# JVBSouza/descriptools

Measured on AMD Instinct MI355X. Metric: Mcells/s full descriptor chain, higher is better.
Workload: dtype f32; 1 GPU; 16384x16384 synthetic tilted-integer-fBm DEM per GPU, full chain (d8, flowacc, river mask, flowhand/HAND with fused GFI + ln(hl/H), fused slope+TI+MTI, downslope), device-resident; global_dem=16384x16384, river_threshold_cells=524288

## Files before the change

### descriptools_amd/csrc/dt_capi.hip

```cpp
#include <cmath>
#include <stdarg.h>
#include <stdlib.h>

#include <sys/mman.h>
#include <atomic>
#include <chrono>
#include <mutex>
#include <system_error>
#include <thread>
#include <utility>
#include <vector>

#include "dt_common.h"
#include "dt_kernels.h"

static thread_local char g_err[512] = "";
void dt_set_error(const char *fmt, ...) {
  va_list ap;
  va_start(ap, fmt);
  vsnprintf(g_err, sizeof(g_err), fmt, ap);
  va_end(ap);
}
extern "C" const char *dt_last_error(void) { return g_err; }
extern "C" const char *dt_version(void) { return "descriptools_hip 0.1 (gfx950)"; }
// ... 941 lines not shown
}
extern "C" int dt_dev_downslope_queue(dt_ctx *c, const float *dem, const uint8_t *fdr, int64_t H, int64_t W, double px,
                                      double dz, int raw, float *out, void *qwork, int64_t qbytes) {
  return dev_downslope_phase(c, 1, dem, fdr, H, W, px, dz, raw, out, qwork, qbytes, nullptr, 0);
}
extern "C" int dt_dev_downslope_queued(dt_ctx *c, const void *qwork, int64_t *count) {
  DT_CTX(c);
  DT_REQUIRE(qwork && count, "NULL pointer");
  uint32_t n = 0;
  DT_HIP(hipMemcpyAsync(&n, qwork, sizeof(n), hipMemcpyDeviceToHost, c->stream));
  DT_HIP(hipStreamSynchronize(c->stream));
  *count = (int64_t)n;
  return DT_OK;
}
extern "C" int dt_dev_downslope_finish(dt_ctx *c, const float *dem, const uint8_t *fdr, int64_t H, int64_t W, double px,
                                       double dz, int raw, float *out, void *qwork, int64_t qbytes, void *twork,
                                       int64_t tbytes) {
  return dev_downslope_phase(c, 2, dem, fdr, H, W, px, dz, raw, out, qwork, qbytes, twork, tbytes);
}

extern "C" int dt_dev_confusion_multi(dt_ctx *c, const double *desc, const int8_t *flood, int64_t N,
                                      double nodata_value, const double *th_host, int nth, int under,
                                      int64_t *counts4_dev) {
  DT_DEV(d, c);
  DT_REQUIRE(th_host && counts4_dev, "NULL thresholds / counts");
  DT_REQUIRE((desc && flood) || N == 0, "NULL raster");
  return d.done(dt_launch_confusion(c->stream, desc, flood, N, nodata_value, th_host, nth, under,
                                    (unsigned long long *)counts4_dev));
}

extern "C" int dt_dev_unique_extremes_f32(dt_ctx *c, const float *x, int64_t N, float *out3_dev) {
  DT_DEV(d, c);
  DT_REQUIRE(x && out3_dev && N >= 0, "bad arguments");
  uint32_t *work = (uint32_t *)d.scratch(64, 256);
  DT_TRY(d.rc);
  return d.done(dt_launch_unique_extremes(c->stream, x, N, work, out3_dev));
}

extern "C" int dt_dev_minmax_scale_f32(dt_ctx *c, const float *x, int64_t N, float mn, float mx, float nodata,
                                       double *desc) {
  DT_DEV(d, c);
  DT_REQUIRE((x && desc) || N == 0, "NULL raster");
  return d.done(dt_launch_minmax_scale(c->stream, x, N, mn, mx, nodata, desc));
}

extern "C" int dt_dev_minmax_scale_f32_f64(dt_ctx *c, const float *x, int64_t N, double mn, double mx, double nodata,
                                           double *desc) {
  DT_DEV(d, c);
  DT_REQUIRE((x && desc) || N == 0, "NULL raster");
  return d.done(dt_launch_minmax_scale_f32f64(c->stream, x, N, mn, mx, nodata, desc));
}

extern "C" int dt_dev_classify(dt_ctx *c, const double *desc, int8_t *flood, int64_t N, double nodata_value,
                               double threshold, int under, int remap_flood, uint8_t *binary, int32_t *klass,
                               int64_t *counts4_dev) {
  DT_DEV(d, c);
  DT_REQUIRE(counts4_dev != nullptr, "counts4 is NULL");
  DT_REQUIRE((desc && flood) || N == 0, "NULL raster");
  return d.done(dt_launch_classify_f64(c->stream, desc, nullptr, flood, N, nodata_value, threshold, under, remap_flood,
                                       binary, klass, (unsigned long long *)counts4_dev));
}

extern "C" int dt_dev_membench_copy(dt_ctx *c, const float *a, float *b, int64_t N, int blocks) {
  DT_DEV(d, c);
  DT_REQUIRE(a && b && N >= 0 && blocks != 0, "bad arguments");
  return d.done(dt_launch_membench_copy(c->stream, a, b, N, blocks));
}

extern "C" int dt_dev_membench_mix(dt_ctx *c, const float *r0, const float *r1, float *w0, float *w1, float *w2,
                                   int64_t N, int n_reads, int n_writes, int nontemporal) {
  DT_DEV(d, c);
  DT_REQUIRE((n_reads < 1 || r0) && (n_reads < 2 || r1) && w0 && (n_writes < 2 || w1) && (n_writes < 3 || w2),
             "NULL stream");
  return d.done(dt_launch_membench_mix(c->stream, r0, r1, w0, w1, w2, N, n_reads, n_writes, nontemporal));
}

extern "C" int dt_dev_membench_mix_timed(dt_ctx *c, const float *r0, const float *r1, float *w0, float *w1, float *w2,
                                         int64_t N, int n_reads, int n_writes, int nontemporal, int reps, double *ms) {
  DT_CTX(c);
  DT_REQUIRE(ms && reps >= 1, "bad arguments");
  DT_TRY(dt_dev_membench_mix(c, r0, r1, w0, w1, w2, N, n_reads, n_writes, nontemporal));
  hipEvent_t e0 = nullptr, e1 = nullptr;
  DT_HIP(hipEventCreate(&e0));
  const hipError_t created = hipEventCreate(&e1);
  if (created != hipSuccess) {
    (void)hipEventDestroy(e0);
    DT_HIP(created);
  }
  int rc = DT_OK;
  float t = 0.0f;
  if (hipEventRecord(e0, c->stream) != hipSuccess) rc = DT_EHIP;
  for (int r = 0; r < reps && rc == DT_OK; r++)
    rc = dt_dev_membench_mix(c, r0, r1, w0, w1, w2, N, n_reads, n_writes, nontemporal);
  if (rc == DT_OK && (hipEventRecord(e1, c->stream) != hipSuccess || hipEventSynchronize(e1) != hipSuccess ||
                      hipEventElapsedTime(&t, e0, e1) != hipSuccess)) {
    dt_set_error("event timing failed: %s", hipGetErrorString(hipGetLastError()));
    rc = DT_EHIP;
  }
  (void)hipEventDestroy(e0);
  (void)hipEventDestroy(e1);
  if (rc == DT_OK) *ms = (double)t / reps;
  return rc;
}
extern "C" int dt_dev_mem_info(dt_ctx *c, int64_t *free_bytes, int64_t *total_bytes) {
  DT_CTX(c);
  size_t f = 0, t = 0;
  DT_HIP(hipMemGetInfo(&f, &t));
  if (free_bytes) *free_bytes = (int64_t)f;
  if (total_bytes) *total_bytes = (int64_t)t;
  return DT_OK;
}

extern "C" int dt_dev_i32_to_i64(dt_ctx *c, const int32_t *src, int64_t N, int64_t *dst) {
  DT_DEV(d, c);
  return d.done(dt_launch_i32_to_i64(c->stream, src, N, dst));
}
extern "C" int dt_dev_i64_to_i32(dt_ctx *c, const int64_t *src, int64_t N, int32_t *dst) {
  DT_DEV(d, c);
  return d.done(dt_launch_i64_to_i32(c->stream, src, N, dst));
}

extern "C" int64_t dt_perim_cells(int64_t H, int64_t W) { return dt_perim_count((int)H, (int)W); }

extern "C" int dt_dev_slope_d8_w(dt_ctx *c, const dt_window *win, const float *dem, double px, float *slope,
                                 uint8_t *fdr, float *slope_rad) {
  DT_DEV(d, c, win);
  DT_REQUIRE(dem && (slope || fdr || slope_rad), "NULL raster");
  DT_TRY(dt_side_reserve(c, &c->aux, &c->aux_bytes, dt_stencil_aux_bytes(d.w.H, d.w.W)));
  return d.done(dt_launch_stencil(c->stream, d.w, dem, px, slope, fdr, slope_rad, nullptr, 0, 0.0, nullptr, nullptr,
                                  c->aux));
}

static int dev_slope_twi_w(dt_ctx *c, const dt_window *win, const float *dem, const void *acc, int acc64, double px,
                           double n_top, float *slope, float *slope_rad, float *ti, float *mti) {
  DT_DEV(d, c, win);
  DT_REQUIRE(dem && acc && ti && mti, "NULL raster");
  DT_TRY(dt_side_reserve(c, &c->aux, &c->aux_bytes, dt_stencil_aux_bytes(d.w.H, d.w.W)));
  return d.done(dt_launch_stencil(c->stream, d.w, dem, px, slope, nullptr, slope_rad, acc, acc64, n_top, ti, mti,
                                  c->aux));
}
extern "C" int dt_dev_slope_twi_w(dt_ctx *c, const dt_window *win, const float *dem, const int32_t *acc32,
                                  double px, double n_top, float *slope, float *slope_rad, float *ti,
                                  float *mti) {
  return dev_slope_twi_w(c, win, dem, acc32, 0, px, n_top, slope, slope_rad, ti, mti);
}
extern "C" int dt_dev_slope_twi_w_a64(dt_ctx *c, const dt_window *win, const float *dem, const int64_t *acc64,
                                      double px, double n_top, float *slope, float *slope_rad, float *ti,
                                      float *mti) {
  return dev_slope_twi_w(c, win, dem, acc64, 1, px, n_top, slope, slope_rad, ti, mti);
}

extern "C" int64_t dt_downslope_lift_workspace_w(const dt_window *win) {
  DtWin w;
  if (dt_convert_window(win, &w) != DT_OK) return -1;
  return (int64_t)dt_downslope_lift_bytes_w(w);
}
enum DsForm { DS_PLAIN, DS_LIFT, DS_EMIT };
static int dev_downslope_w(dt_ctx *c, DsForm form, const dt_window *win, const float *dem, const uint8_t *fdr, double px,
                           double dz, int raw, float *out, int32_t *n_unresolved_dev, void *work, int64_t work_bytes,
                           void *walkers, int64_t walkers_bytes) {
  DT_DEV(d, c, win);
  DT_REQUIRE(dem && fdr && out, "NULL raster");
  if (form == DS_LIFT)
    DT_REQUIRE(work != nullptr && work_bytes >= (int64_t)dt_downslope_lift_bytes_w(d.w),
               "downslope workspace missing or too small");
  if (form == DS_EMIT) {
    DT_REQUIRE(work == nullptr || work_bytes >= (int64_t)dt_downslope_lift_bytes_w(d.w), "downslope workspace too small");
    DT_REQUIRE(walkers != nullptr && walkers_bytes >= 256 + 48, "walker buffer missing or too small");
  }
  if (n_unresolved_dev) DT_HIP(hipMemsetAsync(n_unresolved_dev, 0, sizeof(int32_t), c->stream));
  const DtDsLift L = work ? dt_downslope_lift_layout(d.w, work) : DtDsLift{};
  return d.done(dt_launch_downslope(c->stream, d.w, dem, fdr, px, dz, raw, out, (int *)n_unresolved_dev, L.qcount,
                                    L.tab[0], 0, walkers, (size_t)walkers_bytes));
}
extern "C" int dt_dev_downslope_w(dt_ctx *c, const dt_window *win, const float *dem, const uint8_t *fdr,
                                  double px, double dz, int raw, float *out, int32_t *n_unresolved_dev) {
  return dev_downslope_w(c, DS_PLAIN, win, dem, fdr, px, dz, raw, out, n_unresolved_dev, nullptr, 0, nullptr, 0);
}
extern "C" int dt_dev_downslope_lift_w(dt_ctx *c, const dt_window *win, const float *dem, const uint8_t *fdr,
                                       double px, double dz, int raw, float *out, int32_t *n_unresolved_dev,
                                       void *work, int64_t work_bytes) {
  return dev_downslope_w(c, DS_LIFT, win, dem, fdr, px, dz, raw, out, n_unresolved_dev, work, work_bytes, nullptr, 0);
}
extern "C" int dt_dev_downslope_emit_w(dt_ctx *c, const dt_window *win, const float *dem, const uint8_t *fdr,
                                       double px, double dz, int raw, float *out, int32_t *n_unresolved_dev,
                                       void *work, int64_t work_bytes, void *walkers, int64_t walkers_bytes) {
  return dev_downslope_w(c, DS_EMIT, win, dem, fdr, px, dz, raw, out, n_unresolved_dev, work, work_bytes, walkers,
                         walkers_bytes);
}

extern "C" int dt_dev_downslope_walk_w(dt_ctx *c, const dt_window *win, const float *dem, const uint8_t *fdr, double px,
                                       double dz, int64_t n, void *rec, void *work, int64_t work_bytes) {
  DT_DEV(d, c, win);
  DT_REQUIRE(n >= 0, "negative count");
  DT_REQUIRE(n == 0 || (dem && fdr && rec), "NULL pointer");
  DT_REQUIRE(work == nullptr || work_bytes >= (int64_t)dt_downslope_lift_bytes_w(d.w), "downslope workspace too small");
  return d.done(dt_launch_ds_walk(c->stream, d.w, dem, fdr, px, dz, n, rec, work));
}
extern "C" int dt_dev_downslope_walk_route_w(dt_ctx *c, const dt_window *win, const float *dem, const uint8_t *fdr,
                                             double px, double dz, int64_t n, void *rec, void *work, int64_t work_bytes,
                                             float *out, const int32_t *row_starts, int32_t ty,
                                             const int32_t *col_starts, int32_t tx, void *send, int32_t *counts,
                                             int32_t *scratch) {
  DT_DEV(d, c, win);
  DT_REQUIRE(n >= 0, "negative count");
  DT_REQUIRE(ty >= 1 && tx >= 1 && row_starts && col_starts && counts, "layout / counts missing");
  DT_REQUIRE(n == 0 || (dem && fdr && rec && out && send && scratch), "NULL pointer");
  DT_REQUIRE(work == nullptr || work_bytes >= (int64_t)dt_downslope_lift_bytes_w(d.w), "downslope workspace too small");
  DT_TRY(dt_launch_ds_walk(c->stream, d.w, dem, fdr, px, dz, n, rec, work, out));
  return d.done(dt_launch_ds_route(c->stream, n, rec, row_starts, ty, col_starts, tx, send, counts, scratch));
}
template <typename T, typename Launch>
static int dev_downslope_walk_seed_w(dt_ctx *c, const dt_window *win, const T *dem, int64_t n, const int32_t *ys,
                                     const int32_t *xs, void *rec, Launch launch) {
  DT_DEV(d, c, win);
  DT_REQUIRE(n >= 0, "negative count");
  DT_REQUIRE(n == 0 || (dem && ys && xs && rec), "NULL pointer");
  return d.done(launch(c->stream, d.w, dem, n, ys, xs, rec));
}
extern "C" int dt_dev_downslope_walk_seed_w(dt_ctx *c, const dt_window *win, const float *dem, int64_t n,
                                            const int32_t *ys, const int32_t *xs, void *rec) {
  return dev_downslope_walk_seed_w(c, win, dem, n, ys, xs, rec, dt_launch_ds_walk_seed);
}

extern "C" int dt_dev_flowacc_local_w(dt_ctx *c, const dt_window *win, const uint8_t *fdr, int32_t *acc32,
                                      int64_t *A_perim, int32_t *xr_perim, uint8_t *code_perim) {
  DT_DEV(d, c, win);
  DT_REQUIRE(fdr && A_perim && xr_perim && code_perim, "NULL pointer");
  const size_t need = dt_flowacc_tiled_scratch(d.w.H, d.w.W);
  void *scr, *scr2;
  d.scratch(need, dt_flowhand_tiled_scratch(d.w.H, d.w.W), &scr, &scr2);
  DT_TRY(d.rc);
  DT_TRY(dt_launch_fa_local(c->stream, d.w, fdr, scr, need, acc32, 1));
  DT_TRY(d.done(dt_launch_fa_summary(c->stream, d.w, scr, A_perim, xr_perim, code_perim)));
  dt_scratch_claim(c, DT_OWNER_FLOWACC, d.w.H, d.w.W, scr, scr2);
  return DT_OK;
}

static int dev_flowacc_finish_w(dt_ctx *c, const dt_window *win, const uint8_t *fdr, const float *dem,
                                const uint64_t *ext_perim, int64_t threshold, void *acc, int acc64, int8_t *river) {
  DT_DEV(d, c, win);
  DT_REQUIRE(fdr && acc, "NULL raster");
  const DtScratchClaim *k;
  DT_TRY(dt_scratch_claimed(c, DT_OWNER_FLOWACC, &d.w, false,
                            "dt_dev_flowacc_finish_w without a matching dt_dev_flowacc_local_w on this context (another "
                            "call has used the context's scratch in between)", &k));
  return d.done(dt_launch_fa_finish(c->stream, d.w, fdr, dem, k->ptr, (const unsigned long long *)ext_perim, threshold,
                                    acc, acc64, river, c->status));
}
extern "C" int dt_dev_flowacc_finish_w(dt_ctx *c, const dt_window *win, const uint8_t *fdr, const float *dem,
                                       const uint64_t *ext_perim, int64_t threshold, int32_t *acc32,
                                       int8_t *river) {
  return dev_flowacc_finish_w(c, win, fdr, dem, ext_perim, threshold, acc32, 0, river);
}
extern "C" int dt_dev_flowacc_finish_w_a64(dt_ctx *c, const dt_window *win, const uint8_t *fdr, const float *dem,
                                           const uint64_t *ext_perim, int64_t threshold, int64_t *acc64,
                                           int8_t *river) {
  return dev_flowacc_finish_w(c, win, fdr, dem, ext_perim, threshold, acc64, 1, river);
}

static int dev_flowacc_finish_fh_local_w(dt_ctx *c, const dt_window *win, const uint8_t *fdr, const float *dem,
                                         const uint64_t *ext_perim, int64_t threshold, void *acc, int acc64,
                                         int8_t *river, uint8_t *kind, int32_t *ref, int32_t *nc, int32_t *nd,
                                         float *zr, int64_t *ar) {
  DT_DEV(d, c, win);
  DT_REQUIRE(fdr && acc && river && kind && ref && nc && nd && zr && ar, "NULL pointer");
  const DtScratchClaim *k;
  DT_TRY(dt_scratch_claimed(c, DT_OWNER_FLOWACC, &d.w, true,
                            "dt_dev_flowacc_finish_flowhand_local_w without a matching dt_dev_flowacc_local_w on this "
                            "context (another call has used the context's scratch in between)", &k));
  char *fh = k->ptr2;
  DT_TRY(dt_launch_fa_finish_fh_local(c->stream, d.w, fdr, dem, k->ptr, fh, dt_flowhand_tiled_scratch(d.w.H, d.w.W),
                                      (const unsigned long long *)ext_perim, threshold, acc, acc64, river, c->status));
  DT_TRY(d.done(dt_launch_fh_summary(c->stream, d.w, fh, dem, acc, acc64, kind, ref, nc, nd, zr, (long long *)ar)));
  dt_scratch_claim(c, DT_OWNER_HAND, d.w.H, d.w.W, fh);
  return DT_OK;
}
extern "C" int dt_dev_flowacc_finish_flowhand_local_w(dt_ctx *c, const dt_window *win, const uint8_t *fdr,
                                                      const float *dem, const uint64_t *ext_perim, int64_t threshold,
                                                      int32_t *acc32, int8_t *river, uint8_t *kind, int32_t *ref,
                                                      int32_t *nc, int32_t *nd, float *zr, int64_t *ar) {
  return dev_flowacc_finish_fh_local_w(c, win, fdr, dem, ext_perim, threshold, acc32, 0, river, kind, ref, nc, nd, zr, ar);
}
extern "C" int dt_dev_flowacc_finish_flowhand_local_w_a64(dt_ctx *c, const dt_window *win, const uint8_t *fdr,
                                                          const float *dem, const uint64_t *ext_perim,
                                                          int64_t threshold, int64_t *acc64, int8_t *river,
                                                          uint8_t *kind, int32_t *ref, int32_t *nc, int32_t *nd,
                                                          float *zr, int64_t *ar) {
  return dev_flowacc_finish_fh_local_w(c, win, fdr, dem, ext_perim, threshold, acc64, 1, river, kind, ref, nc, nd, zr, ar);
}

static int dev_flowacc_river_flowhand_local(dt_ctx *c, const uint8_t *fdr, const float *dem, const uint8_t *nod4,
                                           int64_t H, int64_t W, int64_t threshold, int32_t *acc32, int8_t *river,
                                           const DtTwiEpilogue *twi = nullptr) {
  DT_DEV(d, c, H, W);
  DT_REQUIRE((fdr && acc32 && river) || H * W == 0, "NULL raster");
  DT_REQUIRE(!twi || H * W == 0 || dt_twi_epilogue_ok(d.w, acc32, river, twi),
             "this raster does not take the TI / MTI epilogue (dt_slope_from_d8_ok): use dt_dev_slope_twi");
  const size_t need = dt_flowacc_tiled_scratch(H, W), need2 = dt_flowhand_tiled_scratch(H, W);
  void *scr, *scr2;
  d.scratch(need, need2, &scr, &scr2);
  DT_TRY(d.rc);
  DT_TRY(dt_launch_fa_local(c->stream, d.w, fdr, scr, need, acc32, 0));
  DT_TRY(d.done(dt_launch_fa_finish_fh_local(c->stream, d.w, fdr, dem, scr, scr2, need2, nullptr, threshold, acc32, 0,
                                             river, c->status, nod4, dt_nodata4_ld(W), twi)));
  dt_scratch_claim(c, DT_OWNER_HAND, H, W, scr2);
  return DT_OK;
}
extern "C" int dt_dev_flowacc_river_flowhand_local(dt_ctx *c, const uint8_t *fdr, const float *dem, int64_t H, int64_t W,
                                                   int64_t threshold, int32_t *acc32, int8_t *river) {
  return dev_flowacc_river_flowhand_local(c, fdr, dem, nullptr, H, W, threshold, acc32, river);
}
extern "C" int dt_dev_flowacc_river_flowhand_local_m(dt_ctx *c, const uint8_t *fdr, const float *dem,
                                                     const uint8_t *nodata4, int64_t H, int64_t W, int64_t threshold,
                                                     int32_t *acc32, int8_t *river) {
  DT_REQUIRE((dem && nodata4) || H * W == 0, "dem and the nodata mask are both required");
  return dev_flowacc_river_flowhand_local(c, fdr, dem, nodata4, H, W, threshold, acc32, river);
}
extern "C" int dt_dev_flowacc_river_flowhand_local_ms(dt_ctx *c, const uint8_t *fdr, const float *dem,
                                                      const uint8_t *nodata4, int64_t H, int64_t W, int64_t threshold,
                                                      int32_t *acc32, int8_t *river, double px, double n_top,
                                                      const float *slope, float *ti, float *mti, void *marks) {
  DT_REQUIRE((dem && nodata4 && slope && ti && mti && marks) || H * W == 0, "NULL raster");
  const DtTwiEpilogue twi{slope, ti, mti, px, n_top, marks};
  return dev_flowacc_river_flowhand_local(c, fdr, dem, nodata4, H, W, threshold, acc32, river, &twi);
}
extern "C" int dt_slope_from_d8_ok(int64_t H, int64_t W) {
  return H > 0 && W > 0 && W % 64 == 0;
}
extern "C" int64_t dt_slope_marks_bytes(int64_t H, int64_t W) {
  return (H < 0 || W < 0) ? -1 : (int64_t)dt_stencil_aux_bytes(H, W);
}
extern "C" int dt_dev_slope_twi_fix(dt_ctx *c, const float *dem, const int32_t *acc32, int64_t H, int64_t W, double px,
                                    double n_top, float *slope, float *ti, float *mti, const void *marks) {
  DT_DEV(d, c, H, W);
  DT_REQUIRE((dem && acc32 && slope && ti && mti && marks) || H * W == 0, "NULL raster");
  return d.done(dt_launch_slope_twi_fix(c->stream, d.w, dem, px, slope, acc32, n_top, ti, mti, (void *)marks));
}
extern "C" int64_t dt_nodata_mask_bytes(int64_t H, int64_t W) {
  return (H < 0 || W < 0) ? -1 : (int64_t)dt_nodata4_bytes(H, W);
}
extern "C" int dt_dev_slope_d8_m(dt_ctx *c, const float *dem, int64_t H, int64_t W, double px, uint8_t *fdr,
                                 uint8_t *nodata4) {
  DT_DEV(d, c, H, W);
  DT_REQUIRE((dem && fdr && nodata4) || H * W == 0, "NULL raster");
  DT_TRY(dt_side_reserve(c, &c->aux, &c->aux_bytes, dt_stencil_aux_bytes(H, W)));
  return d.done(dt_launch_stencil(c->stream, d.w, dem, px, nullptr, fdr, nullptr, nullptr, 0, 0.0, nullptr, nullptr,
                                  c->aux, nodata4, dt_nodata4_ld(W)));
}
extern "C" int dt_dev_slope_d8_ms(dt_ctx *c, const float *dem, int64_t H, int64_t W, double px, uint8_t *fdr,
                                  uint8_t *nodata4, float *slope, void *marks) {
  DT_DEV(d, c, H, W);
  DT_REQUIRE((dem && fdr && nodata4 && (marks || !slope)) || H * W == 0, "NULL raster");
  DT_TRY(dt_side_reserve(c, &c->aux, &c->aux_bytes, dt_stencil_aux_bytes(H, W)));
  return d.done(dt_launch_d8_slope(c->stream, d.w, dem, px, fdr, slope, c->aux, nodata4, dt_nodata4_ld(W), marks));
}
extern "C" int dt_dev_slope_d8_f64(dt_ctx *c, const double *dem, int64_t H, int64_t W, double px, uint8_t *fdr,
                                   float *proxy) {
  DT_DEV(d, c, H, W);
  DT_REQUIRE(dem || H * W == 0, "NULL raster");
  return d.done(dt_launch_d8_f64(c->stream, dem, H, W, px, fdr, nullptr, proxy));
}
extern "C" int dt_dev_slope_twi_f64(dt_ctx *c, const double *dem, const int32_t *acc32, int64_t H, int64_t W,
                                    double px, double n_top, float *slope, float *slope_rad, float *ti, float *mti) {
  DT_DEV(d, c, H, W);
  DT_REQUIRE((dem && acc32 && ti && mti) || H * W == 0, "NULL raster");
  return d.done(dt_launch_slope_twi_f64(c->stream, dem, acc32, H, W, px, n_top, slope, slope_rad, ti, mti));
}
extern "C" int dt_dev_downslope_f64(dt_ctx *c, const double *dem, const uint8_t *fdr, int64_t H, int64_t W, double px,
                                    double dz, int raw, float *out) {
  DT_DEV(d, c, H, W);
  DT_REQUIRE((dem && fdr && out) || H * W == 0, "NULL raster");
  return d.done(dt_launch_downslope_win_f64(c->stream, dem, fdr, H, W, px, dz, raw, out));
}
extern "C" int dt_dev_hand_gfi_f64(dt_ctx *c, const double *dem, const int32_t *idx32, const int32_t *acc32, int64_t H,
                                   int64_t W, double px, double n_gfi, double b, double *hand, float *gfi,
                                   float *lnhlh) {
  DT_DEV(d, c, H, W);
  DT_REQUIRE((dem && idx32 && acc32 && hand) || H * W == 0, "NULL raster");
  return d.done(dt_launch_hand_gfi_f64(c->stream, dem, idx32, acc32, H * W, n_gfi, b, px, hand, gfi, lnhlh));
}

static int dev_flowhand_local_w(dt_ctx *c, const dt_window *win, const float *dem, const uint8_t *fdr,
                                const int8_t *river, const void *acc, int acc64, uint8_t *kind, int32_t *ref,
                                int32_t *nc, int32_t *nd, float *zr, int64_t *ar) {
  DT_DEV(d, c, win);
  DT_REQUIRE(fdr && river && kind && ref && nc && nd && zr && ar, "NULL pointer");
  const size_t need = dt_flowhand_tiled_scratch(d.w.H, d.w.W);
  void *scr = d.scratch(need);
  DT_TRY(d.rc);
  DT_TRY(dt_launch_fh_local(c->stream, d.w, fdr, river, scr, need));
  DT_TRY(d.done(dt_launch_fh_summary(c->stream, d.w, scr, dem, acc, acc64, kind, ref, nc, nd, zr, (long long *)ar)));
  dt_scratch_claim(c, DT_OWNER_HAND, d.w.H, d.w.W, scr);
  return DT_OK;
}
extern "C" int dt_dev_flowhand_local_w(dt_ctx *c, const dt_window *win, const float *dem, const uint8_t *fdr,
                                       const int8_t *river, const int32_t *acc32, uint8_t *kind, int32_t *ref,
                                       int32_t *nc, int32_t *nd, float *zr, int64_t *ar) {
  return dev_flowhand_local_w(c, win, dem, fdr, river, acc32, 0, kind, ref, nc, nd, zr, ar);
}
extern "C" int dt_dev_flowhand_local_w_a64(dt_ctx *c, const dt_window *win, const float *dem, const uint8_t *fdr,
                                           const int8_t *river, const int64_t *acc64, uint8_t *kind, int32_t *ref,
                                           int32_t *nc, int32_t *nd, float *zr, int64_t *ar) {
  return dev_flowhand_local_w(c, win, dem, fdr, river, acc64, 1, kind, ref, nc, nd, zr, ar);
}

static int dev_flowhand_finish_w(dt_ctx *c, const dt_window *win, const float *dem, const uint8_t *fdr,
                                 const int8_t *river, const void *acc, int acc64, double px, double n_gfi, double b,
                                 const uint8_t *res_ok, const int32_t *res_nc, const int32_t *res_nd,
                                 const int64_t *rem_gidx, const float *rem_zr, const int64_t *rem_ar, float *fdist,
                                 int32_t *idx32, int64_t *idx64, float *hand, void *a_river, float *gfi,
                                 float *lnhlh, bool fused) {
  DT_DEV(d, c, win);
  DT_REQUIRE(fdr && river, "NULL raster");
  DT_REQUIRE(!hand || dem, "hand needs dem");
  DT_REQUIRE(!a_river || acc, "a_river needs the accumulation raster");
  DT_REQUIRE(!fused || (dem && acc && gfi && lnhlh), "NULL raster");
  DT_REQUIRE(!res_ok || (res_nc && res_nd && rem_gidx && rem_zr && rem_ar), "incomplete rank-exit results");
  const DtScratchClaim *k;
  DT_TRY(dt_scratch_claimed(c, DT_OWNER_HAND, &d.w, false,
                            "flowhand finish without a matching dt_dev_flowhand_local_w on this context (another call "
                            "has used the context's scratch in between)", &k));
  return d.done(dt_launch_fh_finish(c->stream, d.w, dem, fdr, river, acc, acc64, px, k->ptr, res_ok, res_nc, res_nd,
                                    (const long long *)rem_gidx, rem_zr, (const long long *)rem_ar, fdist, idx32,
                                    (long long *)idx64, hand, a_river, fused ? gfi : nullptr, fused ? lnhlh : nullptr,
                                    n_gfi, b, px));
}
extern "C" int dt_dev_flowhand_finish_w(dt_ctx *c, const dt_window *win, const float *dem, const uint8_t *fdr,
                                        const int8_t *river, const int32_t *acc32, double px,
                                        const uint8_t *res_ok, const int32_t *res_nc, const int32_t *res_nd,
                                        const int64_t *rem_gidx, const float *rem_zr, const int64_t *rem_ar,
                                        float *fdist, int32_t *idx32, int64_t *idx64, float *hand,
                                        int32_t *a_river) {
  return dev_flowhand_finish_w(c, win, dem, fdr, river, acc32, 0, px, 0.0, 1.0, res_ok, res_nc, res_nd, rem_gidx, rem_zr,
                               rem_ar, fdist, idx32, idx64, hand, a_river, nullptr, nullptr, false);
}
extern "C" int dt_dev_flowhand_finish_w_a64(dt_ctx *c, const dt_window *win, const float *dem, const uint8_t *fdr,
                                            const int8_t *river, const int64_t *acc64, double px,
                                            const uint8_t *res_ok, const int32_t *res_nc, const int32_t *res_nd,
                                            const int64_t *rem_gidx, const float *rem_zr, const int64_t *rem_ar,
                                            float *fdist, int32_t *idx32, int64_t *idx64, float *hand,
                                            int64_t *a_river64) {
  return dev_flowhand_finish_w(c, win, dem, fdr, river, acc64, 1, px, 0.0, 1.0, res_ok, res_nc, res_nd, rem_gidx, rem_zr,
                               rem_ar, fdist, idx32, idx64, hand, a_river64, nullptr, nullptr, false);
}
extern "C" int dt_dev_flowhand_gfi_finish_w(dt_ctx *c, const dt_window *win, const float *dem, const uint8_t *fdr,
                                            const int8_t *river, const int32_t *acc32, double px, double n_gfi,
                                            double b, const uint8_t *res_ok, const int32_t *res_nc,
                                            const int32_t *res_nd, const int64_t *rem_gidx, const float *rem_zr,
                                            const int64_t *rem_ar, float *fdist, int32_t *idx32, int64_t *idx64,
                                            float *hand, int32_t *a_river, float *gfi, float *lnhlh) {
  return dev_flowhand_finish_w(c, win, dem, fdr, river, acc32, 0, px, n_gfi, b, res_ok, res_nc, res_nd, rem_gidx, rem_zr,
                               rem_ar, fdist, idx32, idx64, hand, a_river, gfi, lnhlh, true);
}
extern "C" int dt_dev_flowhand_gfi_finish_w_a64(dt_ctx *c, const dt_window *win, const float *dem,
                                                const uint8_t *fdr, const int8_t *river, const int64_t *acc64,
                                                double px, double n_gfi, double b, const uint8_t *res_ok,
                                                const int32_t *res_nc, const int32_t *res_nd,
                                                const int64_t *rem_gidx, const float *rem_zr, const int64_t *rem_ar,
                                                float *fdist, int32_t *idx32, int64_t *idx64, float *hand,
                                                int64_t *a_river64, float *gfi, float *lnhlh) {
  return dev_flowhand_finish_w(c, win, dem, fdr, river, acc64, 1, px, n_gfi, b, res_ok, res_nc, res_nd, rem_gidx, rem_zr,
                               rem_ar, fdist, idx32, idx64, hand, a_river64, gfi, lnhlh, true);
}

static int dt_scratch2_reserve(dt_ctx *c, size_t bytes) {
  return dt_side_reserve(c, &c->scratch2, &c->scratch2_bytes, bytes);
}

extern "C" int dt_dev_rank_solve_flowacc(dt_ctx *c, int ty, int tx, const int64_t *heights, const int64_t *widths,
                                         int64_t Pmax, const void *rows_dev, int64_t rowbytes,
                                         const int64_t *field_offsets3, int rank, int64_t P_rank,
                                         uint64_t *ext_out_dev) {
  DT_DEV(d, c);
  DT_REQUIRE(heights && widths && rows_dev && field_offsets3 && ext_out_dev, "NULL pointer");
  DT_REQUIRE(rank >= 0 && rank < ty * tx && P_rank >= 0 && P_rank <= Pmax, "bad rank / ring size");
  DT_TRY(dt_scratch2_reserve(c, dt_rank_solve_scratch(ty * tx, Pmax)));
  return d.done(dt_launch_rank_solve_flowacc(c->stream, ty, tx, heights, widths, Pmax, rows_dev, rowbytes,
                                             field_offsets3, rank, P_rank, c->scratch2,
                                             (unsigned long long *)ext_out_dev));
}

extern "C" int dt_dev_rank_solve_flowhand(dt_ctx *c, int ty, int tx, const int64_t *heights, const int64_t *widths,
                                          int64_t Pmax, const void *rows_dev, int64_t rowbytes,
                                          const int64_t *field_offsets7, int rank, int64_t P_rank,
                                          uint8_t *res_ok, int32_t *res_nc, int32_t *res_nd, int64_t *rem_gidx,
                                          float *rem_zr, int64_t *rem_ar) {
  DT_DEV(d, c);
  DT_REQUIRE(heights && widths && rows_dev && field_offsets7 && res_ok && res_nc && res_nd && rem_gidx && rem_zr &&
                 rem_ar, "NULL pointer");
  DT_REQUIRE(rank >= 0 && rank < ty * tx && P_rank >= 0 && P_rank <= Pmax, "bad rank / ring size");
  DT_TRY(dt_scratch2_reserve(c, dt_rank_solve_scratch(ty * tx, Pmax)));
  return d.done(dt_launch_rank_solve_flowhand(c->stream, ty, tx, heights, widths, Pmax, rows_dev, rowbytes,
                                              field_offsets7, rank, P_rank, c->scratch2, res_ok, res_nc, res_nd,
                                              (long long *)rem_gidx, rem_zr, (long long *)rem_ar));
}

extern "C" int dt_dev_slope_d8_f64_w(dt_ctx *c, const dt_window *win, const double *dem, double px, uint8_t *fdr,
                                     float *proxy) {
  DT_DEV(d, c, win);
  DT_REQUIRE(dem && (fdr || proxy), "NULL raster");
  return d.done(dt_launch_d8_f64_w(c->stream, d.w, dem, px, fdr, proxy));
}
static int dev_slope_twi_f64_w(dt_ctx *c, const dt_window *win, const double *dem, const void *acc, int acc64,
                               double px, double n_top, float *slope, float *slope_rad, float *ti, float *mti) {
  DT_DEV(d, c, win);
  DT_REQUIRE(dem && acc && ti && mti, "NULL raster");
  return d.done(dt_launch_slope_twi_f64_w(c->stream, d.w, dem, acc, acc64, px, n_top, slope, slope_rad, ti, mti));
}
extern "C" int dt_dev_slope_twi_f64_w(dt_ctx *c, const dt_window *win, const double *dem, const int32_t *acc32,
                                      double px, double n_top, float *slope, float *slope_rad, float *ti, float *mti) {
  return dev_slope_twi_f64_w(c, win, dem, acc32, 0, px, n_top, slope, slope_rad, ti, mti);
}
extern "C" int dt_dev_slope_twi_f64_w_a64(dt_ctx *c, const dt_window *win, const double *dem, const int64_t *acc64,
                                          double px, double n_top, float *slope, float *slope_rad, float *ti,
                                          float *mti) {
  return dev_slope_twi_f64_w(c, win, dem, acc64, 1, px, n_top, slope, slope_rad, ti, mti);
}
extern "C" int dt_dev_downslope_f64_w(dt_ctx *c, const dt_window *win, const double *dem, const uint8_t *fdr,
                                      double px, double dz, int raw, float *out, int32_t *n_unresolved_dev) {
  DT_DEV(d, c, win);
  DT_REQUIRE(dem && fdr && out, "NULL raster");
  if (n_unresolved_dev) DT_HIP(hipMemsetAsync(n_unresolved_dev, 0, sizeof(int32_t), c->stream));
  return d.done(dt_launch_downslope_win_f64_w(c->stream, d.w, dem, fdr, px, dz, raw, out, (int *)n_unresolved_dev));
}
extern "C" int dt_dev_downslope_walk_seed_f64_w(dt_ctx *c, const dt_window *win, const double *dem, int64_t n,
                                                const int32_t *ys, const int32_t *xs, void *rec) {
  return dev_downslope_walk_seed_w(c, win, dem, n, ys, xs, rec, dt_launch_ds_walk_seed_f64);
}
extern "C" int dt_dev_downslope_walk_route_f64_w(dt_ctx *c, const dt_window *win, const double *dem,
                                                 const uint8_t *fdr, double px, double dz, int64_t n, void *rec,
                                                 float *out, const int32_t *row_starts, int32_t ty,
                                                 const int32_t *col_starts, int32_t tx, void *send, int32_t *counts,
                                                 int32_t *scratch) {
  DT_DEV(d, c, win);
  DT_REQUIRE(n >= 0, "negative count");
  DT_REQUIRE(ty >= 1 && tx >= 1 && row_starts && col_starts && counts, "layout / counts missing");
  DT_REQUIRE(n == 0 || (dem && fdr && rec && out && send && scratch), "NULL pointer");
  DT_TRY(dt_launch_ds_walk_f64(c->stream, d.w, dem, fdr, px, dz, n, rec, out));
  return d.done(dt_launch_ds_route(c->stream, n, rec, row_starts, ty, col_starts, tx, send, counts, scratch));
}
extern "C" int dt_dev_flowhand_zr64_w(dt_ctx *c, const dt_window *win, const double *dem, int64_t n,
                                      const uint8_t *kind, const int32_t *ref, double *zr64) {
  DT_DEV(d, c, win);
  DT_REQUIRE(n >= 0 && n <= dt_perim_count(d.w.H, d.w.W), "bad ring size");
  DT_REQUIRE(n == 0 || (dem && kind && ref && zr64), "NULL pointer");
  return d.done(dt_launch_fh_zr64_w(c->stream, d.w, dem, n, kind, ref, zr64));
}
extern "C" int dt_dev_rank_solve_flowhand_f64(dt_ctx *c, int ty, int tx, const int64_t *heights, const int64_t *widths,
                                              int64_t Pmax, const void *rows_dev, int64_t rowbytes,
                                              const int64_t *field_offsets8, int rank, int64_t P_rank,
                                              uint8_t *res_ok, int32_t *res_nc, int32_t *res_nd, int64_t *rem_gidx,
                                              float *rem_zr, int64_t *rem_ar, double *rem_zr64) {
  DT_DEV(d, c);
  DT_REQUIRE(heights && widths && rows_dev && field_offsets8 && res_ok && res_nc && res_nd && rem_gidx && rem_zr &&
                 rem_ar && rem_zr64, "NULL pointer");
  DT_REQUIRE(rank >= 0 && rank < ty * tx && P_rank >= 0 && P_rank <= Pmax, "bad rank / ring size");
  DT_REQUIRE(field_offsets8[7] % 8 == 0 && rowbytes % 8 == 0, "the float64 field must be 8-byte aligned");
  DT_TRY(dt_scratch2_reserve(c, dt_rank_solve_scratch(ty * tx, Pmax)));
  return d.done(dt_launch_rank_solve_flowhand_f64(c->stream, ty, tx, heights, widths, Pmax, rows_dev, rowbytes,
                                                  field_offsets8, rank, P_rank, c->scratch2, res_ok, res_nc, res_nd,
                                                  (long long *)rem_gidx, rem_zr, (long long *)rem_ar, rem_zr64));
}
extern "C" int64_t dt_hand_f64_table_bytes(int64_t n_remote) {
  return n_remote < 0 ? -1 : dt_hand_f64_table_slots(n_remote) * 16;
}
static int dev_hand_gfi_f64_w(dt_ctx *c, const dt_window *win, const double *dem, const int32_t *idx32,
                              const int64_t *idx64, const void *acc, const void *a_river, int acc64, int64_t n_remote,
                              const uint8_t *res_ok, const int64_t *rem_gidx, const double *rem_zr64, void *table,
                              int64_t table_bytes, double px, double n_gfi, double b, double *hand, float *gfi,
                              float *lnhlh) {
  DT_DEV(d, c, win);
  DT_REQUIRE(dem && (idx32 || idx64) && acc && a_river && hand, "NULL raster");
  DT_REQUIRE(n_remote >= 0 && (n_remote == 0 || !res_ok || (rem_gidx && rem_zr64)), "incomplete rank-exit results");
  DT_REQUIRE(table && table_bytes >= dt_hand_f64_table_bytes(n_remote), "river-height table missing or too small");
  return d.done(dt_launch_hand_gfi_f64_w(c->stream, d.w, dem, idx64 ? nullptr : idx32, idx64, acc, a_river, acc64,
                                         n_remote, res_ok, rem_gidx, rem_zr64, table, n_gfi, b, px, hand, gfi, lnhlh));
}
extern "C" int dt_dev_hand_gfi_f64_w(dt_ctx *c, const dt_window *win, const double *dem, const int32_t *idx32,
                                     const int64_t *idx64, const int32_t *acc32, const int32_t *a_river32,
                                     int64_t n_remote, const uint8_t *res_ok, const int64_t *rem_gidx,
                                     const double *rem_zr64, void *table, int64_t table_bytes, double px,
                                     double n_gfi, double b, double *hand, float *gfi, float *lnhlh) {
  return dev_hand_gfi_f64_w(c, win, dem, idx32, idx64, acc32, a_river32, 0, n_remote, res_ok, rem_gidx, rem_zr64,
                            table, table_bytes, px, n_gfi, b, hand, gfi, lnhlh);
}
extern "C" int dt_dev_hand_gfi_f64_w_a64(dt_ctx *c, const dt_window *win, const double *dem, const int32_t *idx32,
                                         const int64_t *idx64, const int64_t *acc64, const int64_t *a_river64,
                                         int64_t n_remote, const uint8_t *res_ok, const int64_t *rem_gidx,
                                         const double *rem_zr64, void *table, int64_t table_bytes, double px,
                                         double n_gfi, double b, double *hand, float *gfi, float *lnhlh) {
  return dev_hand_gfi_f64_w(c, win, dem, idx32, idx64, acc64, a_river64, 1, n_remote, res_ok, rem_gidx, rem_zr64,
                            table, table_bytes, px, n_gfi, b, hand, gfi, lnhlh);
}

static dt_ctx *g_host_ctx = nullptr;
static std::mutex g_host_mu;

static int host_ctx(dt_ctx **out) {
  if (!g_host_ctx) {
    int dev = 0;
    if (hipGetDevice(&dev) != hipSuccess) dev = 0;
    DT_TRY(dt_ctx_create(dev, nullptr, &g_host_ctx));
  }
  *out = g_host_ctx;
  return hipSetDevice(g_host_ctx->device) == hipSuccess ? DT_OK : DT_EHIP;
}

struct HostBlock {
  void *p;
  size_t bytes;
  bool busy;
};
static std::vector<HostBlock> g_blocks;
static void host_blocks_drop_idle(size_t keep_bytes) {
  for (;;) {
    size_t idle = 0;
    int big = -1;
    for (size_t i = 0; i < g_blocks.size(); i++)
      if (!g_blocks[i].busy) {
        idle += g_blocks[i].bytes;
        if (big < 0 || g_blocks[i].bytes > g_blocks[(size_t)big].bytes) big = (int)i;
      }
    if (idle <= keep_bytes || big < 0) return;
    (void)hipFree(g_blocks[(size_t)big].p);
    g_blocks.erase(g_blocks.begin() + big);
  }
}
static void *host_block_take(size_t bytes) {
  int best = -1;
  for (size_t i = 0; i < g_blocks.size(); i++)
    if (!g_blocks[i].busy && g_blocks[i].bytes >= bytes && g_blocks[i].bytes <= bytes + bytes / 4 + 4096 &&
        (best < 0 || g_blocks[i].bytes < g_blocks[(size_t)best].bytes))
      best = (int)i;
  if (best >= 0) {
    g_blocks[(size_t)best].busy = true;
    return g_blocks[(size_t)best].p;
  }
  void *p = nullptr;
  if (hipMalloc(&p, bytes) != hipSuccess) {
    host_blocks_drop_idle(0);
    (void)hipGetLastError();
    if (hipMalloc(&p, bytes) != hipSuccess) return nullptr;
  }
  g_blocks.push_back(HostBlock{p, bytes, true});
  return p;
}
static size_t host_cache_budget() {
  static long long mb = -1;
  if (mb < 0) {
    const char *e = getenv("DT_HOST_CACHE_MB");
    mb = e ? atoll(e) : 4096;
    if (mb < 0) mb = 0;
  }
  return (size_t)mb << 20;
}
static void host_block_release(void *p) {
  for (auto &b : g_blocks)
    if (b.p == p) b.busy = false;
  host_blocks_drop_idle(host_cache_budget());
}
struct HostCall {
  std::lock_guard<std::mutex> lk{g_host_mu};
  dt_ctx *c = nullptr;
  int rc = host_ctx(&c);
  ~HostCall() {
    if (!synced && c) (void)hipStreamSynchronize(c->stream);
    for (void *p : blocks) host_block_release(p);
  }
  void *workspace(size_t bytes) {
    void *p = host_block_take(bytes ? bytes : 16);
    if (p) blocks.push_back(p);
    return p;
  }
  template <typename T>
  T *scratch(size_t count) {
    T *d = rc == DT_OK ? (T *)workspace(count * sizeof(T)) : nullptr;
    if (!d && rc == DT_OK) {
      dt_set_error("hipMalloc of %zu bytes failed", count ? count * sizeof(T) : 16);
      rc = DT_ENOMEM;
    }
    return d;
  }
  template <typename T>
  T *in(const T *src, size_t count) {
    T *d = src ? scratch<T>(count) : nullptr;
    if (d) copy(d, src, count * sizeof(T), hipMemcpyHostToDevice);
    return d;
  }
  template <typename T>
  T *out(T *dst, size_t count) {
    T *d = dst ? scratch<T>(count) : nullptr;
    if (d) downloads.push_back({dst, d, count * sizeof(T)});
    return d;
  }
  template <typename T>
  int download(T *dst, const T *src, size_t count) {
    copy(dst, src, count * sizeof(T), hipMemcpyDeviceToHost);
    return rc;
  }
  int finish() {
    for (const Copy &d : downloads) copy(d.dst, d.src, d.bytes, hipMemcpyDeviceToHost);
    if (rc != DT_OK) return rc;
    synced = true;
    return dt_ctx_sync(c);
  }

 private:
  struct Copy {
    void *dst;
    const void *src;
    size_t bytes;
  };
  std::vector<void *> blocks;
  std::vector<Copy> downloads;
  bool synced = false;
  void copy(void *dst, const void *src, size_t bytes, hipMemcpyKind kind) {
    if (rc != DT_OK || bytes == 0) return;
    const hipError_t e = hipMemcpyAsync(dst, src, bytes, kind, c->stream);
    if (e != hipSuccess) {
      dt_set_error("hipMemcpyAsync of %zu bytes failed: %s", bytes, hipGetErrorString(e));
      rc = e == hipErrorOutOfMemory ? DT_ENOMEM : DT_EHIP;
    }
  }
};
extern "C" int dt_host_trim(void) {
  std::lock_guard<std::mutex> lk(g_host_mu);
  if (g_host_ctx) DT_HIP(hipStreamSynchronize(g_host_ctx->stream));
  for (size_t i = 0; i < g_blocks.size();) {
// ... 908 lines not shown
```

### descriptools_amd/csrc/dt_common.h

```cpp
#pragma once
#include <hip/hip_runtime.h>
#include <stdint.h>
#include <stdio.h>
#include <string.h>

#include "../../include/descriptools_hip.h"

#define DT_NODATA (-100.0f)

void dt_set_error(const char *fmt, ...);

#define DT_HIP(call)                                                                   \
  do {                                                                                 \
    hipError_t e__ = (call);                                                           \
    if (e__ != hipSuccess) {                                                           \
      dt_set_error("%s failed: %s (%s:%d)", #call, hipGetErrorString(e__), __FILE__,   \
                   __LINE__);                                                          \
      return e__ == hipErrorOutOfMemory ? DT_ENOMEM : DT_EHIP;                         \
    }                                                                                  \
  } while (0)

#define DT_REQUIRE(cond, msg)                      \
  do {                                             \
    if (!(cond)) {                                 \
      dt_set_error("invalid argument: %s", msg);   \
      return DT_EINVAL;                            \
    }                                              \
  } while (0)

#define DT_TRY(expr)          \
  do {                        \
    int rc__ = (expr);        \
    if (rc__ != DT_OK) return rc__; \
  } while (0)

enum {
  DT_DBG_TWI_FLAG_ALL = 0,
  DT_DBG_RETIRED_FIRST = 1, DT_DBG_RETIRED_LAST = 7,
  DT_DBG_HY_COLOUR_MIN = 8,
  DT_DBG_FA_SCATTER = 9,
  DT_DBG_RC_SLOTS = 10,
  DT_DBG_DINF_STACK = 11,
  DT_DBG_COUNT = 12
};
int dt_debug_get(int key);

enum DtScratchOwner { DT_OWNER_NONE = 0, DT_OWNER_FLOWACC, DT_OWNER_HAND, DT_OWNER_DINF, DT_OWNER_MFD };
struct DtScratchClaim {
  DtScratchOwner owner;
  int64_t h, w;
  char *ptr;
  char *ptr2;
  const void *in[2];
  int frac_bits;
};
struct dt_ctx {
  int device;
  hipStream_t stream;
  bool own_stream;
  char *scratch;
  size_t scratch_bytes;
  size_t scratch_used;
  DtScratchClaim claim;
  char *scratch2;
  size_t scratch2_bytes;
  hipEvent_t ev;
  int *status;
  char *aux;
  size_t aux_bytes;
  uint64_t ws_gen;
};

int dt_scratch_reset(dt_ctx *ctx, size_t total_bytes);
void *dt_scratch_take(dt_ctx *ctx, size_t bytes);
static inline size_t dt_align256(size_t b) { return (b + 255) & ~(size_t)255; }

struct DtCarver {
  char *base;
  size_t off = 0;
  explicit DtCarver(void *p) : base((char *)p) {}
  void *raw(size_t nbytes) {
    char *q = base ? base + off : nullptr;
    off += dt_align256(nbytes);
    return q;
  }
  template <typename T> T *take(size_t count) { return (T *)raw(count * sizeof(T)); }
  size_t bytes() const { return off; }
};
static inline int dt_doubling_rounds(int64_t N) {
  int r = 0;
  while (r < 62 && (1ll << r) < N) r++;
  return r + 1;
}
static inline unsigned dt_capped_grid(int64_t n, int64_t cap) {
  const int64_t want = (n + 255) / 256;
  return (unsigned)(want < cap ? want : cap);
}

__device__ __forceinline__ uint32_t dt_block_scan_256(uint32_t v, uint32_t *s_w, uint32_t *total) {
  const int lane = (int)(threadIdx.x & 63u), wv = (int)(threadIdx.x >> 6);
  uint32_t x = v;
#pragma unroll
  for (int o = 1; o < 64; o <<= 1) {
    const uint32_t t = (uint32_t)__shfl_up((int)x, o);
    if (lane >= o) x += t;
  }
  if (lane == 63) s_w[wv] = x;
  __syncthreads();
  uint32_t before = 0, all = 0;
#pragma unroll
  for (int k = 0; k < 4; k++) {
    const uint32_t t = s_w[k];
    before += k < wv ? t : 0u;
    all += t;
  }
  __syncthreads();
  *total = all;
  return before + x - v;
}

__device__ __forceinline__ bool dt_d8_valid(uint32_t code) {
  return code != 0u && (code & (code - 1u)) == 0u;
}
#define DT_PK8(a, b, c, d, e, f, g, h)                                                 \
  ((uint32_t)((a) + 1) | (uint32_t)((b) + 1) << 2 | (uint32_t)((c) + 1) << 4 |          \
   (uint32_t)((d) + 1) << 6 | (uint32_t)((e) + 1) << 8 | (uint32_t)((f) + 1) << 10 |    \
   (uint32_t)((g) + 1) << 12 | (uint32_t)((h) + 1) << 14)
#define DT_DX_PACK DT_PK8(1, 1, 0, -1, -1, -1, 0, 1)
#define DT_DY_PACK DT_PK8(0, 1, 1, 1, 0, -1, -1, -1)
__device__ __forceinline__ void dt_nb_delta(int i, int &dy, int &dx) {
  dx = (int)((DT_DX_PACK >> (2 * i)) & 3u) - 1;
  dy = (int)((DT_DY_PACK >> (2 * i)) & 3u) - 1;
}
__device__ __forceinline__ uint32_t dt_nb_back_code(int i) { return 1u << ((i + 4) & 7); }
__device__ __forceinline__ void dt_d8_delta(uint32_t code, int &dy, int &dx) {
  dt_nb_delta(__ffs((int)code) - 1, dy, dx);
}

struct DtWin {
  int H, W;
  long long ld;
  int gy0, gx0, Hg, Wg;
  int halo;
};
static inline DtWin dt_full_window(int64_t H, int64_t W) {
  DtWin w;
  w.H = (int)H; w.W = (int)W; w.ld = W; w.gy0 = 0; w.gx0 = 0; w.Hg = (int)H; w.Wg = (int)W; w.halo = 0;
  return w;
}
__host__ __device__ __forceinline__ bool dt_in_core(const DtWin &w, int y, int x) {
  return y >= 0 && y < w.H && x >= 0 && x < w.W;
}
__host__ __device__ __forceinline__ bool dt_readable(const DtWin &w, int y, int x) {
  int gy = w.gy0 + y, gx = w.gx0 + x;
  return gy >= 0 && gy < w.Hg && gx >= 0 && gx < w.Wg && y >= -w.halo && y < w.H + w.halo && x >= -w.halo &&
         x < w.W + w.halo;
}
__host__ __device__ __forceinline__ bool dt_has_code(const DtWin &w, int y, int x) {
  if (!dt_readable(w, y, x)) return false;
  const int gy = w.gy0 + y, gx = w.gx0 + x;
  return (y > -w.halo || gy == 0) && (y < w.H + w.halo - 1 || gy == w.Hg - 1) && (x > -w.halo || gx == 0) &&
         (x < w.W + w.halo - 1 || gx == w.Wg - 1);
}
__host__ __device__ __forceinline__ bool dt_in_global(const DtWin &w, int y, int x) {
  int gy = w.gy0 + y, gx = w.gx0 + x;
  return gy >= 0 && gy < w.Hg && gx >= 0 && gx < w.Wg;
}
__host__ __device__ __forceinline__ long long dt_perim_count(int H, int W) {
  if (H <= 0 || W <= 0) return 0;
  if (H == 1) return W;
  if (W == 1) return H;
  return 2ll * W + 2ll * (H - 2);
}
__host__ __device__ __forceinline__ long long dt_perim_index(int H, int W, int y, int x) {
  if (H == 1) return x;
  if (W == 1) return y;
  if (y == 0) return x;
  if (y == H - 1) return (long long)W + x;
  if (x == 0) return 2ll * W + (y - 1);
  if (x == W - 1) return 2ll * W + (H - 2) + (y - 1);
  return -1;
}
__host__ __device__ __forceinline__ void dt_perim_cell(int H, int W, long long i, int &y, int &x) {
  if (H == 1) { y = 0; x = (int)i; return; }
  if (W == 1) { y = (int)i; x = 0; return; }
  if (i < W) { y = 0; x = (int)i; }
  else if (i < 2ll * W) { y = H - 1; x = (int)(i - W); }
  else if (i < 2ll * W + (H - 2)) { y = (int)(i - 2ll * W) + 1; x = 0; }
  else { y = (int)(i - 2ll * W - (H - 2)) + 1; x = W - 1; }
}
```

### descriptools_amd/csrc/dt_fa3fh1_kernel.inc

```
#if FA3_TWI
__global__ __launch_bounds__(256, 6) void k_fa3fh1_twi(const uint8_t *__restrict__ fdr, const float *__restrict__ dem,
#else
template <int ND>
__global__ __launch_bounds__(256, 6) void k_fa3fh1(const uint8_t *__restrict__ fdr, const float *__restrict__ dem,
#endif
                                                  const uint8_t *__restrict__ nod4, int ldm, DtWin w, int tiles_x,
                                                  const unsigned long long *__restrict__ rec,
                                                  const unsigned long long *__restrict__ state,
                                                  const unsigned long long *__restrict__ ext,
                                                  const uint16_t *__restrict__ loc16, int32_t *__restrict__ acc32,
                                                  int32_t river_thr, int8_t *__restrict__ river,
                                                  int *__restrict__ status, uint32_t nnodes,
                                                  unsigned long long *__restrict__ nodes,
                                                  unsigned long long *__restrict__ cache,
#if FA3_TWI
                                                  uint8_t *__restrict__ cache_wide, TwiOut tw) {
  constexpr int ND = 2;
#else
                                                  uint8_t *__restrict__ cache_wide) {
#endif
#define P3(c) ((uint32_t)(c) + (((uint32_t)(c) >> 6) << 2))
#define NT3 (TH * (TW + 4))
  __shared__ __attribute__((aligned(16))) unsigned char smem[NT3 * 6];
  __shared__ unsigned long long s_in;
  __shared__ int s_ovf;
  uint32_t *s_delta = reinterpret_cast<uint32_t *>(smem);
  uint16_t *s_nxt = reinterpret_cast<uint16_t *>(smem + NT3 * 4);
  const int tile = dt_tile_of_block((int)blockIdx.x, (int)gridDim.x);
  const int ty = tile / tiles_x, tx = tile - ty * tiles_x;
  const int y0 = ty * TH, x0 = tx * TW;
  const uint4 v_fdr = dt_tile_fetch16(fdr, w, y0, x0);
  uint32_t c2[8] = {0u, 0u, 0u, 0u, 0u, 0u, 0u, 0u};
  if (rec) fa_nbr_codes(fdr, w, y0, x0, threadIdx.x, c2);
  unsigned long long e = 0ull;
  if (threadIdx.x < PS && ext) e = ext[(size_t)tile * PS + threadIdx.x];
  constexpr int VPT = NT / 4 / 256;
  uint2 l4[VPT];
  float4 z4[VPT];
#if FA3_TWI
  fa_v4f s4[VPT];
#endif
#pragma unroll
  for (int u = 0; u < VPT; u++) {
    int c = 4 * (threadIdx.x + 256 * u);
    int y = y0 + c / TW;
    l4[u] = *reinterpret_cast<const uint2 *>(loc16 + (size_t)tile * NT + c);
    z4[u] = make_float4(0.f, 0.f, 0.f, 0.f);
#if FA3_TWI
    s4[u] = (fa_v4f){0.f, 0.f, 0.f, 0.f};
    if (y < w.H)
      s4[u] = __builtin_nontemporal_load(reinterpret_cast<const fa_v4f *>(tw.slope + (long long)y * w.ld + x0 + c % TW));
#endif
    if (ND == 1 && y < w.H) z4[u] = *reinterpret_cast<const float4 *>(dem + (long long)y * w.ld + x0 + c % TW);
    if (ND == 2 && y < w.H) {
      const uint32_t m = (uint32_t)reinterpret_cast<const uint16_t *>(nod4)[(long long)(y >> 2) * ldm + ((x0 + c % TW) >> 2)] >>
                         (4 * (y & 3));
      z4[u] = make_float4((m & 1u) ? DT_NODATA : 0.f, (m & 2u) ? DT_NODATA : 0.f, (m & 4u) ? DT_NODATA : 0.f,
                          (m & 8u) ? DT_NODATA : 0.f);
    }
  }
  {
    const int ly = (int)threadIdx.x >> 2, lxb = ((int)threadIdx.x & 3) * 16;
    const uint32_t cv[4] = {v_fdr.x, v_fdr.y, v_fdr.z, v_fdr.w};
    const bool interior = dt_tile_interior(w, y0, x0);
    const int pbase = ly * (TW + 4) + lxb;
#pragma unroll
    for (int q = 0; q < 4; q++) {
      uint32_t nn[4];
#pragma unroll
      for (int k = 0; k < 4; k++) {
        const uint32_t code = (cv[q] >> (8 * k)) & 0xFFu;
        const int lx = lxb + 4 * q + k;
        const uint32_t n = interior ? dt_tile_next_interior(code, ly, lx) : dt_tile_next(code, ly, lx, y0, x0, w);
        nn[k] = n < NT ? P3(n) : n;
      }
      *reinterpret_cast<uint2 *>(&s_nxt[pbase + 4 * q]) = make_uint2(nn[0] | (nn[1] << 16), nn[2] | (nn[3] << 16));
      *reinterpret_cast<uint4 *>(&s_delta[pbase + 4 * q]) = make_uint4(0, 0, 0, 0);
    }
  }
  if (rec) e = fa_inflow(fa_gather(c2, y0, x0, threadIdx.x, tiles_x, rec, state), e);
  if (threadIdx.x == 0) s_ovf = 0;
  if (__syncthreads_or(!(e & FA_CYCLE) && FA_VALUE(e) >= (1ull << 22))) {
    if (threadIdx.x == 0) s_in = 0ull;
    __syncthreads();
    if (e != 0ull && !(e & FA_CYCLE)) atomicAdd(&s_in, FA_VALUE(e));
    __syncthreads();
    if (threadIdx.x == 0 && s_in >= (1ull << 31) - (unsigned long long)NT && status) atomicOr(status, DT_STATUS_ACC_OVERFLOW);
  }
  if (e != 0ull) {
    int ly, lx;
    dt_cell_of_slot(threadIdx.x, ly, lx);
    uint32_t c = P3(ly * TW + lx);
    if (e & FA_CYCLE) {
      for (int it = 0; it < NT && c < NT3; it++) {
        atomicOr(&s_delta[c], 0x80000000u);
        c = s_nxt[c];
      }
    } else {
      const uint32_t add = (uint32_t)e;
      for (int it = 0; it < NT && c < NT3; it++) {
        atomicAdd(&s_delta[c], add);
        c = s_nxt[c];
      }
    }
  }
  __syncthreads();
  auto finish = [&](uint32_t l16, uint32_t d, float z) -> int32_t {
    int32_t v = l16 == 0xFFFFu ? -100 : (int32_t)l16;
    if (v != -100) v += (int32_t)(d & 0x7FFFFFFFu);
    if (d & 0x80000000u) v = -100;
    if (ND != 0 && z <= DT_NODATA) v = -100;
    return v;
  };
  uint32_t riv4[VPT];
#pragma unroll
  for (int u = 0; u < VPT; u++) {
    int c = 4 * (threadIdx.x + 256 * u);
    int y = y0 + c / TW;
    riv4[u] = 0u;
    if (y >= w.H) continue;
    long long o = (long long)y * w.ld + x0 + c % TW;
    uint4 d = *reinterpret_cast<const uint4 *>(&s_delta[P3(c)]);
    int4 v = make_int4(finish(l4[u].x & 0xFFFFu, d.x, z4[u].x), finish(l4[u].x >> 16, d.y, z4[u].y),
                       finish(l4[u].y & 0xFFFFu, d.z, z4[u].z), finish(l4[u].y >> 16, d.w, z4[u].w));
    *reinterpret_cast<int4 *>(acc32 + o) = v;
    riv4[u] = (v.x > river_thr ? 1u : 0u) | (v.y > river_thr ? 0x100u : 0u) | (v.z > river_thr ? 0x10000u : 0u) |
              (v.w > river_thr ? 0x1000000u : 0u);
    *reinterpret_cast<uint32_t *>(river + o) = riv4[u];
#if FA3_TWI
    {
      const int32_t fv[4] = {v.x, v.y, v.z, v.w};
      const double nlnpx2 = tw.n_top * tw.lnpx2;
      fa_v4f tio, mtio;
      uint32_t rej = 0u;
#pragma unroll
      for (int k = 0; k < 4; k++) {
        const float q = dt_pct_to_tan(s4[u][k]);
        const bool tnod = fv[k] <= -100;
        float tv, mv;
        rej |= ((sd_twi_fast(fv[k], q, tw.n_top, tw.lnpx2, nlnpx2, tv, mv) && !tnod) ? 1u : 0u) << k;
        tio[k] = tnod ? DT_NODATA : tv;
        mtio[k] = tnod ? DT_NODATA : mv;
      }
      __builtin_nontemporal_store(tio, reinterpret_cast<fa_v4f *>(tw.ti + o));
      __builtin_nontemporal_store(mtio, reinterpret_cast<fa_v4f *>(tw.mti + o));
      if (rej) {
        const int x = x0 + c % TW;
        const int stile = (y >> 4) * tw.stiles_x + (x >> 8);
        const size_t lane = (size_t)stile * 256 + (size_t)(((y & 15) >> 2) * 64 + ((x & 255) >> 2));
        atomicOr(&tw.lane_mask[lane >> 1], rej << (16 * (int)(lane & 1) + 4 * (y & 3)));
        tw.tile_mark[stile] = (uint8_t)1;
      }
    }
#endif
  }
  __syncthreads();
#undef P3
#undef NT3
  uint32_t *s_w = reinterpret_cast<uint32_t *>(smem);
  uint8_t *s_fdr = smem + NT * 4;
  uint8_t *s_kind = smem + NT * 5;
  uint32_t *s_lut = reinterpret_cast<uint32_t *>(smem + NT * 6);
  s_lut[threadIdx.x] = fh_lut_entry(threadIdx.x);
  dt_tile_put16(s_fdr, v_fdr);
  __syncthreads();
  fh_tile1n_body(s_fdr, s_w, s_kind, &s_ovf, s_lut, riv4, w, tile, tiles_x, y0, x0, nnodes, nodes, cache, cache_wide);
}
```

### descriptools_amd/csrc/dt_kernels.h

```cpp
#pragma once
#include "dt_common.h"

int dt_launch_synth_dem(hipStream_t s, uint32_t seed, int O, int64_t Hg, int64_t y0, int64_t x0,
                        int64_t h, int64_t w, int nodata_pct, float *out);
int dt_launch_stencil(hipStream_t s, const DtWin &w, const float *dem, double px, float *slope,
                      uint8_t *fdr, float *slope_rad, const void *acc, int acc64, double n_top, float *ti,
                      float *mti, void *aux = nullptr, uint8_t *nod4 = nullptr, int ldm = 0);
static inline int dt_nodata4_ld(int64_t W) { return (int)((((W + 3) / 4) + 7) & ~(int64_t)7); }
static inline size_t dt_nodata4_bytes(int64_t H, int64_t W) { return (size_t)((H + 3) / 4) * (size_t)dt_nodata4_ld(W) * 2; }
struct DtStencilAux {
  uint8_t *mark;
  uint16_t *lmask;
  size_t bytes;
};
static inline DtStencilAux dt_stencil_aux_layout(int64_t ntiles, void *aux) {
  DtStencilAux a;
  DtCarver c(aux);
  a.mark = c.take<uint8_t>((size_t)ntiles);
  a.lmask = c.take<uint16_t>((size_t)ntiles * 256);
  a.bytes = c.bytes();
  return a;
}
size_t dt_stencil_aux_bytes(int64_t H, int64_t W);
int dt_launch_d8_slope(hipStream_t s, const DtWin &w, const float *dem, double px, uint8_t *fdr, float *slope,
                       void *aux, uint8_t *nod4, int ldm, void *smarks);
int dt_launch_slope_twi_fix(hipStream_t s, const DtWin &w, const float *dem, double px, float *slope,
                            const int32_t *acc, double n_top, float *ti, float *mti, void *smarks);
int dt_launch_flowacc(hipStream_t s, const uint8_t *fdr, const float *dem, int64_t H, int64_t W,
                      unsigned long long *state, int32_t *acc32);
int dt_launch_river_mask(hipStream_t s, const int32_t *acc32, int64_t n, int64_t thr, int8_t *river);
int dt_launch_flowhand(hipStream_t s, const float *dem, const uint8_t *fdr, const int8_t *river,
                       const int32_t *acc32, int64_t H, int64_t W, double px,
                       unsigned long long *state, float *fdist, int32_t *idx32, float *hand,
                       int32_t *a_river);
int dt_launch_twi(hipStream_t s, const int32_t *acc32, const float *srad, int64_t n, double px,
                  double n_top, float *ti, float *mti);
int dt_launch_twi_i64(hipStream_t s, const int64_t *fac, const float *srad, int64_t n, double px,
                      double n_top, float *ti, float *mti);
int dt_launch_gfi(hipStream_t s, const float *hand, const int32_t *area, int64_t n, double expo,
                  double b, double size, float *out, int own_cell);
int dt_launch_gfi_i64(hipStream_t s, const float *hand, const int64_t *area, int64_t n, double expo,
                      double b, double size, float *out, int own_cell);
int dt_launch_river_acc_i64(hipStream_t s, const int64_t *fac, const int64_t *idx, int64_t n,
                            int64_t *out);
struct DtDsLift {
  uint32_t *qcount;
  uint4 *qentries;
  uint32_t qcapacity;
  uint2 *tab[3];
  uint8_t *dom;
  size_t queue_bytes, tables_bytes, bytes;
};
DtDsLift dt_downslope_lift_layout(const DtWin &w, void *work);
size_t dt_downslope_lift_bytes(int64_t H, int64_t W);
size_t dt_downslope_queue_bytes(int64_t H, int64_t W);
size_t dt_downslope_tables_bytes(int64_t H, int64_t W);
uint32_t dt_downslope_lift_min(int64_t H, int64_t W);
size_t dt_downslope_tables_bytes_w(const DtWin &w);
size_t dt_downslope_lift_bytes_w(const DtWin &w);
int dt_launch_downslope(hipStream_t s, const DtWin &w, const float *dem, const uint8_t *fdr, double px,
                        double dz, int raw, float *out, int *n_unresolved, void *qwork = nullptr,
                        void *twork = nullptr, int phase = 0, void *walkers = nullptr, size_t walkers_bytes = 0);
int dt_launch_ds_walk(hipStream_t s, const DtWin &w, const float *dem, const uint8_t *fdr, double px, double dz,
                      int64_t n, void *rec, void *work, float *out = nullptr);
int dt_launch_ds_route(hipStream_t s, int64_t n, const void *rec, const int32_t *row_starts, int ty,
                       const int32_t *col_starts, int tx, void *send, int32_t *counts, int32_t *scratch);
int dt_launch_ds_walk_seed(hipStream_t s, const DtWin &w, const float *dem, int64_t n, const int32_t *ys,
                           const int32_t *xs, void *rec);
int dt_launch_downslope_v1(hipStream_t s, const float *dem, const uint8_t *fdr, int64_t H, int64_t W,
                           double px, double dz, int raw, float *out);
int dt_launch_hand_i64(hipStream_t s, const float *dem, const int64_t *idx, int64_t n, float *hand);
int dt_launch_slope_f64(hipStream_t s, const double *dem, int64_t H, int64_t W, double px, float *slope);
int dt_launch_hand_f64(hipStream_t s, const double *dem, const int64_t *idx, int64_t n, double *hand);
int dt_launch_downslope_f64(hipStream_t s, const double *dem, const uint8_t *fdr, int64_t H, int64_t W, double px,
                            double dz, int raw, float *out);
int dt_launch_gfi_f64h(hipStream_t s, const double *hand, const int64_t *fac, const int64_t *idx, int64_t n,
                       double expo, double b, double size, int own_area, float *out);
int dt_launch_d8_f64(hipStream_t s, const double *dem, int64_t H, int64_t W, double px, uint8_t *fdr, float *slope,
                     float *proxy);
int dt_launch_slope_twi_f64(hipStream_t s, const double *dem, const int32_t *acc32, int64_t H, int64_t W, double px,
                            double n_top, float *slope, float *slope_rad, float *ti, float *mti);
int dt_launch_downslope_win_f64(hipStream_t s, const double *dem, const uint8_t *fdr, int64_t H, int64_t W, double px,
                                double dz, int raw, float *out);
int dt_launch_hand_gfi_f64(hipStream_t s, const double *dem, const int32_t *idx32, const int32_t *acc32, int64_t n,
                           double expo, double b, double size, double *hand, float *gfi, float *lnhlh);
int dt_launch_d8_f64_w(hipStream_t s, const DtWin &w, const double *dem, double px, uint8_t *fdr, float *proxy);
int dt_launch_slope_twi_f64_w(hipStream_t s, const DtWin &w, const double *dem, const void *acc, int acc64, double px,
                              double n_top, float *slope, float *slope_rad, float *ti, float *mti);
int dt_launch_downslope_win_f64_w(hipStream_t s, const DtWin &w, const double *dem, const uint8_t *fdr, double px,
                                  double dz, int raw, float *out, int *n_unresolved);
int dt_launch_fh_zr64_w(hipStream_t s, const DtWin &w, const double *dem, int64_t n, const uint8_t *kind,
                        const int32_t *ref, double *zr64);
int64_t dt_hand_f64_table_slots(int64_t n_remote);
int dt_launch_hand_gfi_f64_w(hipStream_t s, const DtWin &w, const double *dem, const int32_t *idx32,
                             const int64_t *idx64, const void *fac, const void *a_river, int acc64, int64_t n_remote,
                             const uint8_t *res_ok, const int64_t *rem_gidx, const double *rem_zr64, void *table,
                             double expo, double b, double size, double *hand, float *gfi, float *lnhlh);
int dt_launch_ds_walk_f64(hipStream_t s, const DtWin &w, const double *dem, const uint8_t *fdr, double px, double dz,
                          int64_t n, void *rec, float *out);
int dt_launch_ds_walk_seed_f64(hipStream_t s, const DtWin &w, const double *dem, int64_t n, const int32_t *ys,
                               const int32_t *xs, void *rec);
int dt_launch_confusion(hipStream_t s, const double *desc, const int8_t *flood, int64_t n,
                        double nodata, const double *th_host, int nth, int under,
                        unsigned long long *counts4);
int dt_launch_i32_to_i64(hipStream_t s, const int32_t *a, int64_t n, int64_t *b);
int dt_launch_i64_to_i32(hipStream_t s, const int64_t *a, int64_t n, int32_t *b);

size_t dt_flowacc_tiled_scratch(int64_t H, int64_t W);
int dt_launch_fa_local(hipStream_t s, const DtWin &w, const uint8_t *fdr, void *scratch, size_t scratch_bytes,
                       int32_t *acc32, int rank_level);
int dt_launch_fa_summary(hipStream_t s, const DtWin &w, void *scratch, int64_t *A, int32_t *xr, uint8_t *code);
int dt_launch_fa_finish(hipStream_t s, const DtWin &w, const uint8_t *fdr, const float *dem, void *scratch,
                        const unsigned long long *ext_perim, int64_t river_thr, void *acc, int acc64,
                        int8_t *river, int *status = nullptr);
size_t dt_flowacc_weighted_scratch(int64_t H, int64_t W);
int dt_launch_flowacc_weighted(hipStream_t s, const DtWin &w, const uint8_t *fdr, const float *dem, const double *wt,
                               int frac_bits, void *scratch, size_t scratch_bytes, double *acc, int *status);
size_t dt_flowhand_tiled_scratch(int64_t H, int64_t W);
struct DtTwiEpilogue {
  const float *slope;
  float *ti, *mti;
  double px, n_top;
  void *marks;
};
int dt_launch_fa_finish_fh_local(hipStream_t s, const DtWin &w, const uint8_t *fdr, const float *dem, void *fa_scratch,
                                 void *fh_scratch, size_t fh_bytes, const unsigned long long *ext_perim,
                                 int64_t river_thr, void *acc, int acc64, int8_t *river, int *status,
                                 const uint8_t *nod4 = nullptr, int ldm = 0, const DtTwiEpilogue *twi = nullptr);
bool dt_twi_epilogue_ok(const DtWin &w, const void *acc, const int8_t *river, const DtTwiEpilogue *twi);
int dt_launch_fh_local(hipStream_t s, const DtWin &w, const uint8_t *fdr, const int8_t *river, void *scratch,
                       size_t scratch_bytes);
int dt_launch_fh_summary(hipStream_t s, const DtWin &w, void *scratch, const float *dem, const void *acc, int acc64,
                         uint8_t *kind, int32_t *ref, int32_t *nc, int32_t *nd, float *zr, long long *ar);
int dt_launch_fh_finish(hipStream_t s, const DtWin &w, const float *dem, const uint8_t *fdr,
                        const int8_t *river, const void *acc, int acc64, double px, void *scratch,
                        const uint8_t *res_ok, const int32_t *res_nc, const int32_t *res_nd,
                        const long long *rem_gidx, const float *rem_zr, const long long *rem_ar, float *fdist,
                        int32_t *idx32, long long *idx64, float *hand, void *a_river, float *gfi = nullptr,
                        float *lnhlh = nullptr, double n_gfi = 0.0, double b_gfi = 1.0, double size = 1.0);
int dt_launch_gfi_both(hipStream_t s, const float *hand, const void *a_river, const void *fac, int acc64,
                       int64_t n, double expo, double b, double size, float *gfi, float *lnhlh);
int dt_launch_unique_extremes(hipStream_t s, const float *x, int64_t n, uint32_t *work4, float *out3);
int dt_launch_minmax_scale(hipStream_t s, const float *x, int64_t n, float mn, float mx, float nodata,
                           double *out);
int dt_launch_minmax_scale_f32f64(hipStream_t s, const float *x, int64_t n, double mn, double mx, double nodata,
                                  double *out);
int dt_launch_minmax_scale_den_f32(hipStream_t s, const float *x, int64_t n, float mn, float den, float nodata,
                                   float *out);
int dt_launch_minmax_scale_den_f64(hipStream_t s, const double *x, int64_t n, double mn, double den, double nodata,
                                   double *out);
int dt_launch_minmax_scale_f16(hipStream_t s, const void *x, int64_t n, float mn, float den, float nodata, void *out);
int dt_launch_classify_f64(hipStream_t s, const double *desc, const int32_t *bin_in, int8_t *flood, int64_t n,
                           double nodata, double th, int under, int remap, uint8_t *binary, int32_t *klass,
                           unsigned long long *counts4);
int dt_launch_classify_f32(hipStream_t s, const float *desc, const int32_t *bin_in, int8_t *flood, int64_t n,
                           float nodata, float th, int under, int remap, uint8_t *binary, int32_t *klass,
                           unsigned long long *counts4);
int dt_launch_membench_copy(hipStream_t s, const float *a, float *b, int64_t n, int blocks);
int dt_launch_membench_mix(hipStream_t s, const float *r0, const float *r1, float *w0, float *w1, float *w2, int64_t n,
                           int nr, int nw, int nt);
size_t dt_rank_solve_scratch(int nranks, int64_t Pmax);
int dt_launch_rank_solve_flowacc(hipStream_t s, int ty, int tx, const int64_t *heights, const int64_t *widths,
                                 int64_t Pmax, const void *rows, int64_t rowbytes, const int64_t *offs, int rank,
                                 int64_t P_rank, void *scratch, unsigned long long *ext_out);
int dt_launch_rank_solve_flowhand(hipStream_t s, int ty, int tx, const int64_t *heights, const int64_t *widths,
                                  int64_t Pmax, const void *rows, int64_t rowbytes, const int64_t *offs, int rank,
                                  int64_t P_rank, void *scratch, uint8_t *res_ok, int32_t *res_nc,
                                  int32_t *res_nd, long long *gidx, float *zr, long long *ar);
int dt_launch_rank_solve_flowhand_f64(hipStream_t s, int ty, int tx, const int64_t *heights, const int64_t *widths,
                                      int64_t Pmax, const void *rows, int64_t rowbytes, const int64_t *offs8, int rank,
                                      int64_t P_rank, void *scratch, uint8_t *res_ok, int32_t *res_nc,
                                      int32_t *res_nd, long long *gidx, float *zr, long long *ar, double *zr64);

size_t dt_hydro_scratch(int64_t H, int64_t W);
int dt_launch_condition(hipStream_t s, const float *dem, int64_t H, int64_t W, double px, float *filled, uint8_t *fdr,
                        void *scratch, int *unresolved_host, int *rounds_host);
int dt_launch_condition_stage(hipStream_t s, const DtWin &w, int stage, int rounds, const float *dem, float *filled,
                              uint8_t *fdr, uint32_t *dist, int *flag_dev, uint8_t *nsame = nullptr);
int dt_launch_condition_async(hipStream_t s, const float *dem, int64_t H, int64_t W, double px, float *filled,
                              uint8_t *fdr, void *scratch, int rounds, int *status);
int dt_launch_condition_f64(hipStream_t s, const double *dem, int64_t H, int64_t W, double px, double *filled,
                            uint8_t *fdr, void *scratch, int *unresolved_host, int *rounds_host);
int dt_launch_condition_async_f64(hipStream_t s, const double *dem, int64_t H, int64_t W, double px, double *filled,
                                  uint8_t *fdr, void *scratch, int rounds, int *status);

int dt_flow_impl();

size_t dt_stream_order_scratch(int64_t H, int64_t W);
#define DT_SCAN_CPT 8
#define DT_SCAN_CHUNK (256 * DT_SCAN_CPT)
static inline int64_t dt_scan_blocks(int64_t n) { return (n + DT_SCAN_CHUNK - 1) / DT_SCAN_CHUNK; }
struct DtCountScan {
  int64_t nblk, ng;
  uint32_t *bcount, *gsum;
  int64_t *offsets, *goff, *meta;
};
DtCountScan dt_count_scan_carve(DtCarver &c, int64_t n, int64_t *meta);
int dt_launch_count_scan(hipStream_t s, const DtCountScan &cs, int64_t nblk);
int dt_launch_stream_order(hipStream_t s, const uint8_t *fdr, const int8_t *river, int64_t H, int64_t W, void *scratch,
                           size_t scratch_bytes, int8_t *strahler, int64_t *shreve, int64_t *link, int64_t *m_host);

size_t dt_drainage_scratch(int64_t H, int64_t W);
size_t dt_upslope_length_scratch(int64_t H, int64_t W);
int dt_launch_drainage(hipStream_t s, const uint8_t *fdr, const float *dem, const int64_t *pour, int64_t H, int64_t W,
                       double px, void *scratch, size_t scratch_bytes, int64_t *target, double *length,
                       int64_t *label);
int dt_launch_upslope_length(hipStream_t s, const uint8_t *fdr, const float *dem, int64_t H, int64_t W, double px,
                             void *scratch, size_t scratch_bytes, double *length);

size_t dt_reach_catchments_scratch(int64_t N, int own_reach);
int dt_launch_reach_catchments(hipStream_t s, const int64_t *link, const void *idx, int idx_bytes, int64_t N,
                               void *scratch, size_t scratch_bytes, int32_t *reach, int32_t *catch_, int64_t *heads,
                               int64_t cap, int64_t *n_reaches_dev);
int dt_launch_reach_channels(hipStream_t s, const uint8_t *fdr, const int32_t *reach, int64_t H, int64_t W, int64_t R,
                             int64_t *end, int64_t *down, int64_t *n_cells, int64_t *n_card, int64_t *n_diag);
size_t dt_reach_tables_scratch(int K);
int dt_launch_reach_tables(hipStream_t s, const int32_t *catch_, const void *hand, int hand_bytes, const float *slope,
                           int64_t H, int64_t W, const double *stages_host, int K, int64_t R, int frac_bits,
                           void *scratch, size_t scratch_bytes, int64_t *cells, int64_t *Hq, int64_t *Bq, int *status,
                           int slots);
int dt_launch_inundate(hipStream_t s, const int32_t *catch_, const void *hand, int hand_bytes, const double *stage,
                       int64_t N, int64_t R, float *depth);

int dt_launch_dinf_direction(hipStream_t s, const float *dem, const uint8_t *fdr, int64_t H, int64_t W, double px,
                             float *angle, float *slope);
#define DI_STACK 8
size_t dt_dinf_accumulate_scratch(int64_t H, int64_t W);
int dt_launch_dinf_accumulate(hipStream_t s, const float *angle, const double *wt, int64_t H, int64_t W, int frac_bits,
                              int start, int rounds, int finish, int stack_cap, void *scratch, size_t scratch_bytes,
                              double *out, int *status);
const uint32_t *dt_dinf_accumulate_ctl(void *scratch, int64_t H, int64_t W);

#define DT_DINF_DIST_BATCH_MAX 64
size_t dt_dinf_distance_scratch(int64_t H, int64_t W);
int dt_launch_dinf_distance(hipStream_t s, const float *angle, const int8_t *river, const float *dem, int64_t H,
                            int64_t W, double px, int stat, int check_edges, int visit_limit, int start, int rounds,
                            int finish, void *scratch, size_t scratch_bytes, double *h, double *v, double *sf,
                            int *status);
const uint32_t *dt_dinf_distance_ctl(void *scratch, int64_t H, int64_t W);

int dt_launch_mfd_shares(hipStream_t s, const float *dem, const uint8_t *fdr, int64_t H, int64_t W, double exponent,
                         int contour, uint16_t *shares);
size_t dt_mfd_accumulate_scratch(int64_t H, int64_t W);
int dt_launch_mfd_accumulate(hipStream_t s, const uint16_t *shares, const double *wt, int64_t H, int64_t W,
                             int frac_bits, int start, int rounds, int finish, int stack_cap, void *scratch,
                             size_t scratch_bytes, double *out, int *status);
const uint32_t *dt_mfd_accumulate_ctl(void *scratch, int64_t H, int64_t W);

#define DT_TERRAIN_OUTPUTS 8
#define DT_TERRAIN_RADIUS_MAX 32
int dt_launch_terrain(hipStream_t s, const float *dem, int64_t H, int64_t W, double px, int radius, double sx,
                      double sy, double sz, float *const out[DT_TERRAIN_OUTPUTS]);

#define DT_HORIZON_RADIUS_MAX 64
int dt_launch_horizon(hipStream_t s, const float *dem, int64_t H, int64_t W, double px, int radius, int skip,
                      double flat_tan, uint8_t *landform, uint16_t *pattern, float *positive, float *negative,
                      float *sky_view);

size_t dt_proximity_scratch(int64_t H, int64_t W);
int dt_launch_proximity(hipStream_t s, const int8_t *river, const float *nod, int64_t H, int64_t W, double px,
                        void *scratch, size_t scratch_bytes, float *distance, int64_t *indices);

size_t dt_regions_scratch(int64_t H, int64_t W);
size_t dt_inundate_connected_scratch(int64_t H, int64_t W);
int dt_launch_regions(hipStream_t s, const uint8_t *mask, const uint8_t *seeds, int64_t H, int64_t W, int connectivity,
                      int64_t min_cells, void *scratch, size_t scratch_bytes, int64_t *label, int64_t *size,
                      uint8_t *keep);
int dt_launch_inundate_connected(hipStream_t s, const int32_t *catch_, const void *hand, int hand_bytes,
                                 const double *stage, const int8_t *river, int64_t H, int64_t W, int64_t R,
                                 int connectivity, void *scratch, size_t scratch_bytes, float *depth);
```

### descriptools_amd/csrc/dt_tiles.hip

```cpp
#include "dt_common.h"
#include "dt_kernels.h"
#include "dt_math.h"

#define TW 64
#define TH 64
#define NT (TW * TH)
#define PS (2 * TW + 2 * (TH - 2))
#define CPT (NT / 256)

#define NX_SINK 0xFFFFu
#define NX_EXIT 0xFFFEu
#define NX_REXIT 0xFFFDu
#define X_NONE 0xFFFFu

__device__ __forceinline__ int dt_slot_of(int ly, int lx) {
  if (ly == 0) return lx;
  if (ly == TH - 1) return TW + lx;
  if (lx == 0) return 2 * TW + (ly - 1);
  if (lx == TW - 1) return 2 * TW + (TH - 2) + (ly - 1);
  return -1;
}
__device__ __forceinline__ void dt_cell_of_slot(int s, int &ly, int &lx) {
  if (s < TW) { ly = 0; lx = s; }
  else if (s < 2 * TW) { ly = TH - 1; lx = s - TW; }
// ... 900 lines not shown
#pragma unroll
    for (int o = 32; o > 0; o >>= 1) s += __shfl_xor(s, o);
    const uint32_t km = (uint32_t)__popcll(__ballot(mine));
    if (lane == lead) {
      led = true;
      k = km;
      S = (unsigned long long)s;
      rp = rec[pl];
      pp = parent[pl];
      old = atomicAdd(&state[pl], S - ((unsigned long long)km << FA2_SH));
    }
    todo = todo && !mine;
  }
  if (!led || (old >> FA2_SH) != (unsigned long long)k) return;
  unsigned long long T = FAW_W(rp) + (old & FA2_MASK) + S;
  p = pp;
  for (int64_t it = 0; it < nnodes && p != FA_NONE; it++) {
    rp = rec[p];
    pp = parent[p];
    old = atomicAdd(&state[p], T - (1ull << FA2_SH));
    if ((old >> FA2_SH) != 1ull) break;
    T = FAW_W(rp) + (old & FA2_MASK) + T;
    p = pp;
  }
}

#define P3(c) ((uint32_t)(c) + (((uint32_t)(c) >> 6) << 2))
#define NT3 (TH * (TW + 4))
template <bool HAS_DEM>
__global__ __launch_bounds__(256, 3) void k_faw_tile3(const uint8_t *__restrict__ fdr, const float *__restrict__ dem,
                                                     DtWin w, int tiles_x, const unsigned long long *__restrict__ rec,
                                                     const unsigned long long *__restrict__ state,
                                                     const unsigned long long *__restrict__ loc, int sbits,
                                                     double *__restrict__ acc) {
  __shared__ uint16_t s_nxt[NT3];
  __shared__ __attribute__((aligned(16))) unsigned long long s_delta[NT3];
  uint8_t *s_fdr = reinterpret_cast<uint8_t *>(s_delta);
  const int tile = dt_tile_of_block((int)blockIdx.x, (int)gridDim.x);
  const int ty = tile / tiles_x, tx = tile - ty * tiles_x;
  const int y0 = ty * TH, x0 = tx * TW;
  const uint4 v_fdr = dt_tile_fetch16(fdr, w, y0, x0);
  uint32_t c2[8];
  fa_nbr_codes(fdr, w, y0, x0, threadIdx.x, c2);
  unsigned long long lv[CPT];
  float zv[CPT];
#pragma unroll
  for (int j = 0; j < CPT; j++) {
    const int c = threadIdx.x + 256 * j;
    const int y = y0 + c / TW, x = x0 + c % TW;
    lv[j] = loc[(size_t)tile * NT + c];
    zv[j] = (HAS_DEM && y < w.H && x < w.W) ? dem[(long long)y * w.ld + x] : 0.0f;
  }
  unsigned long long e = 0ull;
  {
    int ly = 0, lx = 0;
    if (threadIdx.x < PS) dt_cell_of_slot(threadIdx.x, ly, lx);
    unsigned long long pend = 0ull;
#pragma unroll
    for (int k = 0; k < 8; k++)
      if (c2[k] == fa_back(k)) {
        const uint32_t f = dt_node_of(y0 + ly + FA_QDY(k), x0 + lx + FA_QDX(k), tiles_x);
        const unsigned long long st = state[f];
        e += FAW_W(rec[f]) + (st & FA2_MASK);
        pend |= st >> FA2_SH;
      }
    if (pend) e = FAW_CYC;
  }
  dt_tile_put16(s_fdr, v_fdr);
  __syncthreads();
  uint32_t nx[CPT];
#pragma unroll
  for (int j = 0; j < CPT; j++) {
    const int c = threadIdx.x + 256 * j;
    nx[j] = dt_tile_next(s_fdr[c], c / TW, c % TW, y0, x0, w);
  }
  __syncthreads();
#pragma unroll
  for (int j = 0; j < CPT; j++) {
    const int c = threadIdx.x + 256 * j;
    s_nxt[P3(c)] = (uint16_t)(nx[j] < NT ? P3(nx[j]) : nx[j]);
    s_delta[P3(c)] = 0ull;
  }
  __syncthreads();
  if (e != 0ull) {
    int ly, lx;
    dt_cell_of_slot(threadIdx.x, ly, lx);
    uint32_t c = P3(ly * TW + lx);
    if (e & FAW_CYC) {
      for (int it = 0; it < NT && c < NT3; it++) {
        atomicOr(&s_delta[c], FAW_CYC);
        c = s_nxt[c];
      }
    } else {
      for (int it = 0; it < NT && c < NT3; it++) {
        atomicAdd(&s_delta[c], e);
        c = s_nxt[c];
      }
    }
  }
  __syncthreads();
#pragma unroll
  for (int j = 0; j < CPT; j++) {
    const int c = threadIdx.x + 256 * j;
    const int y = y0 + c / TW, x = x0 + c % TW;
    if (y >= w.H || x >= w.W) continue;
    const unsigned long long d = s_delta[P3(c)];
    const bool dead = lv[j] == FAW_LOC_CYC || (d & FAW_CYC) || (HAS_DEM && zv[j] <= DT_NODATA);
    acc[(long long)y * w.ld + x] = dead ? -100.0 : ldexp((double)(lv[j] + d), -sbits);
  }
}
#undef P3
#undef NT3

struct FawScratch {
  unsigned long long *rec, *state, *loc;
  uint32_t *parent;
  int64_t nnodes, ntiles;
  int tiles_x;
  size_t bytes;
};
static FawScratch faw_layout(const DtWin &w, void *scratch) {
  FawScratch f;
  f.tiles_x = (w.W + TW - 1) / TW;
  f.ntiles = (int64_t)f.tiles_x * ((w.H + TH - 1) / TH);
  f.nnodes = f.ntiles * PS;
  DtCarver c(scratch);
  f.rec = c.take<unsigned long long>((size_t)f.nnodes);
  f.state = c.take<unsigned long long>((size_t)f.nnodes);
  f.parent = c.take<uint32_t>((size_t)f.nnodes);
  f.loc = c.take<unsigned long long>((size_t)f.ntiles * NT);
  f.bytes = c.bytes();
  return f;
}
size_t dt_flowacc_weighted_scratch(int64_t H, int64_t W) { return faw_layout(dt_full_window(H, W), nullptr).bytes; }

int dt_launch_flowacc_weighted(hipStream_t s, const DtWin &w, const uint8_t *fdr, const float *dem, const double *wt,
                               int frac_bits, void *scratch, size_t scratch_bytes, double *acc, int *status) {
  if (w.H == 0 || w.W == 0) return DT_OK;
  FawScratch f = faw_layout(w, scratch);
  DT_REQUIRE(scratch_bytes >= f.bytes, "scratch too small");
  DT_REQUIRE(f.nnodes < 0x7FFFFFF0ll, "raster too large for one device tile");
  const unsigned long long qmax = (1ull << 52) / (unsigned long long)((int64_t)w.H * w.W);
  dim3 gt((unsigned)f.ntiles), b(256), gn((unsigned)((f.nnodes + 255) / 256));
  hipLaunchKernelGGL(k_faw_tile1, gt, b, 0, s, fdr, wt, w, f.tiles_x, frac_bits, qmax, f.rec, f.state, f.parent,
                     f.loc, status);
  hipLaunchKernelGGL(k_faw_reduce, gn, b, 0, s, f.rec, f.nnodes, f.parent, f.state);
  if (dem) hipLaunchKernelGGL(k_faw_tile3<true>, gt, b, 0, s, fdr, dem, w, f.tiles_x, f.rec, f.state, f.loc, frac_bits, acc);
  else hipLaunchKernelGGL(k_faw_tile3<false>, gt, b, 0, s, fdr, dem, w, f.tiles_x, f.rec, f.state, f.loc, frac_bits, acc);
  return DT_OK;
}

#define FHT_DEAD 0xFFFFFFFFu
#define FHT_REMOTE 0x80000000u
#define FHT_DONE 0x8000u
#define FHT_CAP 20000u
#define K_RIVER 1u
#define K_DEAD 2u
#define K_EXIT 3u
#define K_REXIT 4u

__device__ __forceinline__ unsigned long long fht_pack(uint32_t ptr, uint32_t nd, uint32_t ncf) {
  return ((unsigned long long)ptr << 32) | ((unsigned long long)nd << 16) | (unsigned long long)ncf;
}

struct FhTile {
  uint8_t *s_fdr;
  uint8_t *s_halo;
  unsigned long long *s_st;
};

__device__ __forceinline__ uint32_t fht_fdr_at(const FhTile &T, int ly, int lx) {
  if (ly >= 0 && ly < TH && lx >= 0 && lx < TW) return T.s_fdr[ly * TW + lx];
  if (ly < 0) return T.s_halo[lx + 1];
  if (ly >= TH) return T.s_halo[(TW + 2) + lx + 1];
  if (lx < 0) return T.s_halo[2 * (TW + 2) + ly];
  return T.s_halo[2 * (TW + 2) + TH + ly];
}

__device__ __forceinline__ void fht_solve_tile(const FhTile &T, const uint8_t *__restrict__ fdr,
                                               const int8_t *__restrict__ river, const DtWin &w, int y0,
                                               int x0) {
  dt_tile_load_fdr(fdr, w, y0, x0, T.s_fdr);
  for (int i = threadIdx.x; i < 2 * (TW + 2) + 2 * TH; i += 256) {
    int y, x;
    if (i < TW + 2) { y = y0 - 1; x = x0 - 1 + i; }
    else if (i < 2 * (TW + 2)) { y = y0 + TH; x = x0 - 1 + (i - (TW + 2)); }
    else if (i < 2 * (TW + 2) + TH) { y = y0 + (i - 2 * (TW + 2)); x = x0 - 1; }
    else { y = y0 + (i - 2 * (TW + 2) - TH); x = x0 + TW; }
    uint8_t v = 0;
    if (dt_readable(w, y, x)) v = fdr[(long long)y * w.ld + x];
    T.s_halo[i] = v;
  }
  uint8_t *s_riv = reinterpret_cast<uint8_t *>(T.s_st);
  dt_tile_load_fdr(reinterpret_cast<const uint8_t *>(river), w, y0, x0, s_riv);
  __syncthreads();
  uint32_t riv = 0;
  for (int j = 0; j < CPT; j++) {
    int c = threadIdx.x + 256 * j;
    if (s_riv[c] == 1) riv |= 1u << j;
  }
  __syncthreads();
  if (dt_tile_interior(w, y0, x0)) {
#pragma unroll
    for (int j = 0; j < CPT; j++) {
      int c = threadIdx.x + 256 * j;
      int ly = c / TW, lx = c % TW;
      uint32_t code = T.s_fdr[c];
      uint32_t ptr = (uint32_t)c | (K_DEAD << 12), lo = FHT_DONE;
      if (code != 0u && ((riv >> j) & 1u)) {
        ptr = (uint32_t)c | (K_RIVER << 12);
      } else if (dt_d8_valid(code)) {
        int dy, dx;
        dt_d8_delta(code, dy, dx);
        uint32_t ny = (uint32_t)(ly + dy), nx = (uint32_t)(lx + dx);
        bool in_tile = ny < (uint32_t)TH && nx < (uint32_t)TW;
        uint32_t tcode = in_tile ? (uint32_t)T.s_fdr[ny * TW + nx] : fht_fdr_at(T, ly + dy, lx + dx);
        if (tcode != 0u) {
          if (in_tile) {
            bool diag = dy != 0 && dx != 0;
            ptr = ny * TW + nx;
            lo = diag ? (1u << 16) : 1u;
          } else {
            ptr = (uint32_t)c | (K_EXIT << 12);
          }
        }
      }
      T.s_st[c] = ((unsigned long long)ptr << 32) | (unsigned long long)lo;
    }
  } else {
    for (int j = 0; j < CPT; j++) {
      int c = threadIdx.x + 256 * j;
      int ly = c / TW, lx = c % TW;
      int y = y0 + ly, x = x0 + lx;
      uint32_t code = T.s_fdr[c];
      unsigned long long s;
      if (y >= w.H || x >= w.W || code == 0u) {
        s = fht_pack((uint32_t)c | (K_DEAD << 12), 0, FHT_DONE);
      } else if ((riv >> j) & 1u) {
        s = fht_pack((uint32_t)c | (K_RIVER << 12), 0, FHT_DONE);
      } else if (!dt_d8_valid(code)) {
        s = fht_pack((uint32_t)c | (K_DEAD << 12), 0, FHT_DONE);
      } else {
        int dy, dx;
        dt_d8_delta(code, dy, dx);
        int ty = y + dy, tx = x + dx;
        if (!dt_in_global(w, ty, tx) || fht_fdr_at(T, ly + dy, lx + dx) == 0u) {
          s = fht_pack((uint32_t)c | (K_DEAD << 12), 0, FHT_DONE);
        } else if (!dt_in_core(w, ty, tx)) {
          s = fht_pack((uint32_t)c | (K_REXIT << 12), 0, FHT_DONE);
        } else if (ly + dy < 0 || ly + dy >= TH || lx + dx < 0 || lx + dx >= TW) {
          s = fht_pack((uint32_t)c | (K_EXIT << 12), 0, FHT_DONE);
        } else {
          bool diag = dy != 0 && dx != 0;
          s = fht_pack((uint32_t)((ly + dy) * TW + lx + dx), diag ? 1u : 0u, diag ? 0u : 1u);
        }
      }
      T.s_st[c] = s;
    }
  }
  __syncthreads();
  ulonglong2 *s_st2 = reinterpret_cast<ulonglong2 *>(T.s_st);
  for (int round = 0; round < 13; round++) {
    int changed = 0;
#pragma unroll
    for (int j = 0; j < CPT / 2; j++) {
      int c2 = threadIdx.x + 256 * j;
      ulonglong2 s = s_st2[c2];
      bool dx = ((uint32_t)s.x & FHT_DONE) != 0u, dy = ((uint32_t)s.y & FHT_DONE) != 0u;
      if (dx && dy) continue;
      if (!dx) {
        unsigned long long t = T.s_st[(uint32_t)(s.x >> 32) & 0xFFFu];
        s.x = (t & 0xFFFFFFFF00000000ull) | (unsigned long long)((uint32_t)s.x + (uint32_t)t);
      }
      if (!dy) {
        unsigned long long t = T.s_st[(uint32_t)(s.y >> 32) & 0xFFFu];
        s.y = (t & 0xFFFFFFFF00000000ull) | (unsigned long long)((uint32_t)s.y + (uint32_t)t);
      }
      s_st2[c2] = s;
      changed |= (((uint32_t)s.x & (uint32_t)s.y & FHT_DONE) == 0u) ? 1 : 0;
    }
    if (!__syncthreads_or(changed)) break;
  }
#pragma unroll
  for (int j = 0; j < CPT; j++) {
    int c = threadIdx.x + 256 * j;
    if (!((uint32_t)T.s_st[c] & FHT_DONE)) T.s_st[c] = fht_pack((uint32_t)c | (K_DEAD << 12), 0, FHT_DONE);
  }
  __syncthreads();
}

__device__ __forceinline__ uint32_t fh_cache_pack(unsigned long long s) {
  uint32_t ptr = (uint32_t)(s >> 32);
  return (ptr & 0x7FFFu) | ((uint32_t)((s >> 16) & 0xFFu) << 15) | ((uint32_t)(s & 0xFFu) << 23);
}
__device__ __forceinline__ unsigned long long fh_cache_unpack(uint32_t v) {
  return fht_pack(v & 0x7FFFu, (v >> 15) & 0xFFu, ((v >> 23) & 0xFFu) | FHT_DONE);
}
__device__ __forceinline__ unsigned long long fh_cache_get(const unsigned long long *__restrict__ cache, bool wide,
                                                            int tile, int c) {
  if (wide) return cache[(size_t)tile * NT + c];
  return fh_cache_unpack(reinterpret_cast<const uint32_t *>(cache + (size_t)tile * NT)[c]);
}

__global__ __launch_bounds__(256) void k_fh_tile1(const uint8_t *__restrict__ fdr,
                                                 const int8_t *__restrict__ river, DtWin w, int tiles_x,
                                                 uint32_t nnodes, unsigned long long *__restrict__ nodes,
                                                 unsigned long long *__restrict__ cache,
                                                 uint8_t *__restrict__ cache_wide, int only_marked, int ntiles) {
  __shared__ __attribute__((aligned(16))) uint8_t s_fdr[NT];
  __shared__ uint8_t s_halo[2 * (TW + 2) + 2 * TH];
  __shared__ __attribute__((aligned(16))) unsigned long long s_st[NT];
  for (int tile = (int)blockIdx.x; tile < ntiles; tile += (int)gridDim.x) {
  if (only_marked && cache_wide[tile] != 2) continue;
  const int ty = tile / tiles_x, tx = tile - ty * tiles_x;
  const int y0 = ty * TH, x0 = tx * TW;
  FhTile T{s_fdr, s_halo, s_st};
  fht_solve_tile(T, fdr, river, w, y0, x0);
  if (threadIdx.x < PS) {
    int ly, lx;
    dt_cell_of_slot(threadIdx.x, ly, lx);
    unsigned long long s = s_st[ly * TW + lx];
    uint32_t ptr = (uint32_t)(s >> 32), nd = (uint32_t)((s >> 16) & 0xFFFFu);
    uint32_t ncf = (uint32_t)(s & 0xFFFFu), nc = ncf & 0x7FFFu;
    uint32_t kind = (ptr >> 12) & 7u, f = ptr & 0xFFFu;
    int fy = (int)f / TW, fx = (int)f % TW;
    unsigned long long o = fht_pack(FHT_DEAD, 0, FHT_DONE);
    if (!(ncf & FHT_DONE)) {
    } else if (kind == K_RIVER) {
      o = fht_pack((uint32_t)((y0 + fy) * w.W + x0 + fx), nd, nc | FHT_DONE);
    } else if (kind == K_EXIT || kind == K_REXIT) {
      int dy, dx;
      dt_d8_delta(s_fdr[f], dy, dx);
      bool diag = dy != 0 && dx != 0;
      uint32_t node = kind == K_EXIT ? dt_node_of(y0 + fy + dy, x0 + fx + dx, tiles_x)
                                     : nnodes + (uint32_t)dt_perim_index(w.H, w.W, y0 + fy, x0 + fx);
      o = fht_pack(node, nd + (diag ? 1u : 0u), nc + (diag ? 0u : 1u));
    }
    nodes[(size_t)tile * PS + threadIdx.x] = o;
  }
  unsigned long long wv[CPT];
  int wide = 0;
#pragma unroll
  for (int j = 0; j < CPT; j++) {
    wv[j] = s_st[threadIdx.x + 256 * j];
    wide |= (((uint32_t)wv[j] & 0x7FFFu) > 255u || ((uint32_t)(wv[j] >> 16) & 0xFFFFu) > 255u) ? 1 : 0;
  }
  wide = __syncthreads_or(wide);
  if (threadIdx.x == 0) cache_wide[tile] = (uint8_t)wide;
  if (wide) {
#pragma unroll
    for (int j = 0; j < CPT; j++) cache[(size_t)tile * NT + threadIdx.x + 256 * j] = wv[j];
  } else {
    uint32_t *c32 = reinterpret_cast<uint32_t *>(cache + (size_t)tile * NT);
#pragma unroll
    for (int j = 0; j < CPT; j++) c32[threadIdx.x + 256 * j] = fh_cache_pack(wv[j]);
  }
  __syncthreads();
  }
}

#define FN_CNT 0x3FFFFu
#define FN_DONE 0x40000u
#define FN_LOW 0x7FFFFu
#define FN_OVF 0x20100u
#define FN_PTR_SH 19
__device__ __forceinline__ uint32_t fh_lut_entry(uint32_t code) {
  if (!dt_d8_valid(code)) return 0u;
  int dy, dx;
  dt_d8_delta(code, dy, dx);
  return ((uint32_t)(dy * TW + dx) << FN_PTR_SH) + ((dy != 0 && dx != 0) ? (1u << 9) : 1u);
}
__device__ __forceinline__ void fh_tile1n_body(uint8_t *s_fdr, uint32_t *s_w, uint8_t *s_kind, int *s_ovf_p,
                                               const uint32_t *s_lut, const uint32_t (&riv4)[NT / 4 / 256],
                                               const DtWin &w, int tile, int tiles_x, int y0, int x0, uint32_t nnodes,
                                               unsigned long long *__restrict__ nodes,
                                               unsigned long long *__restrict__ cache,
                                               uint8_t *__restrict__ cache_wide) {
#define s_ovf (*s_ovf_p)
  const bool interior = dt_tile_interior(w, y0, x0);
  const uint32_t lx0 = (4u * threadIdx.x) & 63u;
#pragma unroll
  for (int u = 0; u < NT / 4 / 256; u++) {
    const int c0 = 4 * (threadIdx.x + 256 * u);
    const uint32_t codes = *reinterpret_cast<const uint32_t *>(&s_fdr[c0]);
    uint32_t wd[4], kinds = 0;
#pragma unroll
    for (int k = 0; k < 4; k++) {
      const int c = c0 + k;
      const uint32_t code = (codes >> (8 * k)) & 0xFFu, cw = (uint32_t)c << FN_PTR_SH;
      const bool is_river = ((riv4[u] >> (8 * k)) & 0xFFu) == 1u;
      uint32_t word = cw | FN_DONE, kind = K_DEAD;
      if (interior) {
        const uint32_t wn = cw + s_lut[code];
        if (code != 0u) {
          if (is_river) {
            kind = K_RIVER;
          } else if (wn & FN_CNT) {
            const bool out = (int32_t)wn < 0 || (((wn >> FN_PTR_SH) & 63u) - (lx0 + (uint32_t)k - 1u)) > 2u;
            if (out) kind = K_EXIT;
            else word = wn;
          }
        }
      } else {
        const int ly = c / TW, lx = c % TW;
        const int y = y0 + ly, x = x0 + lx;
        if (y < w.H && x < w.W && code != 0u) {
          if (is_river) {
            kind = K_RIVER;
          } else if (dt_d8_valid(code)) {
            int dy, dx;
            dt_d8_delta(code, dy, dx);
            uint32_t ny = (uint32_t)(ly + dy), nx = (uint32_t)(lx + dx);
            bool in_tile = ny < (uint32_t)TH && nx < (uint32_t)TW;
            if (dt_in_global(w, y + dy, x + dx)) {
              if (!dt_in_core(w, y + dy, x + dx)) kind = K_REXIT;
              else if (!in_tile) kind = K_EXIT;
              else word = ((ny * TW + nx) << FN_PTR_SH) | ((dy != 0 && dx != 0) ? (1u << 9) : 1u);
            }
          }
        }
      }
      wd[k] = word;
      kinds |= kind << (8 * k);
    }
    *reinterpret_cast<uint4 *>(&s_w[c0]) = make_uint4(wd[0], wd[1], wd[2], wd[3]);
    *reinterpret_cast<uint32_t *>(&s_kind[c0]) = kinds;
  }
  __syncthreads();
  uint2 *s_w2 = reinterpret_cast<uint2 *>(s_w);
  uint2 own[CPT / 2];
#pragma unroll
  for (int j = 0; j < CPT / 2; j++) own[j] = s_w2[threadIdx.x + 256 * j];
  for (int round = 0; round < 13; round++) {
    int changed = 0;
    uint32_t ovf = 0;
#pragma unroll
    for (int j = 0; j < CPT / 2; j++) {
      int c2 = threadIdx.x + 256 * j;
      uint2 v = own[j];
      bool dx = (v.x & FN_DONE) != 0u, dy = (v.y & FN_DONE) != 0u;
      if (dx && dy) continue;
      if (!dx) {
        v.x = s_w[v.x >> FN_PTR_SH] + (v.x & FN_CNT);
        if (!(v.x & (FN_DONE | FN_OVF))) v.x = s_w[v.x >> FN_PTR_SH] + (v.x & FN_CNT);
        ovf |= v.x & FN_OVF;
      }
      if (!dy) {
        v.y = s_w[v.y >> FN_PTR_SH] + (v.y & FN_CNT);
        if (!(v.y & (FN_DONE | FN_OVF))) v.y = s_w[v.y >> FN_PTR_SH] + (v.y & FN_CNT);
        ovf |= v.y & FN_OVF;
      }
      own[j] = v;
      s_w2[c2] = v;
      changed |= ((v.x & v.y & FN_DONE) == 0u) ? 1 : 0;
    }
    if (ovf) s_ovf = 1;
    if (!__syncthreads_or(changed)) break;
    if (s_ovf) break;
  }
  if (s_ovf) {
    if (threadIdx.x == 0) cache_wide[tile] = 2;
    return;
  }
  auto narrow = [&](uint32_t v, uint32_t c) -> uint32_t {
    uint32_t f = v >> FN_PTR_SH, kind = s_kind[f];
    if (!(v & FN_DONE)) { f = c; kind = K_DEAD; v = 0; }
    return f | (kind << 12) | (((v >> 9) & 0xFFu) << 15) | ((v & 0xFFu) << 23);
  };
#pragma unroll
  for (int j = 0; j < CPT / 2; j++) {
    const int c2 = threadIdx.x + 256 * j;
    s_w2[c2] = make_uint2(narrow(own[j].x, 2u * (uint32_t)c2), narrow(own[j].y, 2u * (uint32_t)c2 + 1u));
  }
  if (threadIdx.x == 0) cache_wide[tile] = 0;
  __syncthreads();
  uint32_t *c32 = reinterpret_cast<uint32_t *>(cache + (size_t)tile * NT);
#pragma unroll
  for (int u = 0; u < NT / 4 / 256; u++) {
    int c = 4 * (threadIdx.x + 256 * u);
    *reinterpret_cast<uint4 *>(c32 + c) = *reinterpret_cast<const uint4 *>(&s_w[c]);
  }
  if (threadIdx.x < PS) {
    int ly, lx;
    dt_cell_of_slot(threadIdx.x, ly, lx);
    unsigned long long sw = fh_cache_unpack(s_w[ly * TW + lx]);
    uint32_t ptr = (uint32_t)(sw >> 32), nd = (uint32_t)((sw >> 16) & 0xFFFFu), nc = (uint32_t)sw & 0x7FFFu;
    uint32_t kind = (ptr >> 12) & 7u, f = ptr & 0xFFFu;
    int fy = (int)f / TW, fx = (int)f % TW;
    unsigned long long o = fht_pack(FHT_DEAD, 0, FHT_DONE);
    if (kind == K_RIVER) {
      o = fht_pack((uint32_t)((y0 + fy) * w.W + x0 + fx), nd, nc | FHT_DONE);
    } else if (kind == K_EXIT || kind == K_REXIT) {
      int dy, dx;
      dt_d8_delta(s_fdr[f], dy, dx);
      bool diag = dy != 0 && dx != 0;
      uint32_t node = kind == K_EXIT ? dt_node_of(y0 + fy + dy, x0 + fx + dx, tiles_x)
                                     : nnodes + (uint32_t)dt_perim_index(w.H, w.W, y0 + fy, x0 + fx);
      o = fht_pack(node, nd + (diag ? 1u : 0u), nc + (diag ? 0u : 1u));
    }
    nodes[(size_t)tile * PS + threadIdx.x] = o;
  }
#undef s_ovf
}

__global__ __launch_bounds__(256, 6) void k_fh_tile1n(const uint8_t *__restrict__ fdr,
                                                     const int8_t *__restrict__ river, DtWin w, int tiles_x,
                                                     uint32_t nnodes, unsigned long long *__restrict__ nodes,
                                                     unsigned long long *__restrict__ cache,
                                                     uint8_t *__restrict__ cache_wide) {
  __shared__ __attribute__((aligned(16))) uint8_t s_fdr[NT];
  __shared__ __attribute__((aligned(16))) uint32_t s_w[NT];
  __shared__ __attribute__((aligned(16))) uint8_t s_kind[NT];
  __shared__ uint32_t s_lut[256];
  __shared__ int s_ovf;
  const int tile = dt_tile_of_block((int)blockIdx.x, (int)gridDim.x);
  const int ty = tile / tiles_x, tx = tile - ty * tiles_x;
  const int y0 = ty * TH, x0 = tx * TW;
  const uint4 v_fdr = dt_tile_fetch16(fdr, w, y0, x0);
  const uint4 v_riv = dt_tile_fetch16(reinterpret_cast<const uint8_t *>(river), w, y0, x0);
  dt_tile_put16(s_fdr, v_fdr);
  dt_tile_put16(s_kind, v_riv);
  s_lut[threadIdx.x] = fh_lut_entry(threadIdx.x);
  if (threadIdx.x == 0) s_ovf = 0;
  __syncthreads();
  uint32_t riv4[NT / 4 / 256];
#pragma unroll
  for (int u = 0; u < NT / 4 / 256; u++) riv4[u] = *reinterpret_cast<const uint32_t *>(&s_kind[4 * (threadIdx.x + 256 * u)]);
  fh_tile1n_body(s_fdr, s_w, s_kind, &s_ovf, s_lut, riv4, w, tile, tiles_x, y0, x0, nnodes, nodes, cache, cache_wide);
}


struct TwiOut {
  const float *slope;
  float *ti, *mti;
  double n_top, lnpx2;
  uint8_t *tile_mark;
  uint32_t *lane_mask;
  int stiles_x;
};
typedef float fa_v4f __attribute__((ext_vector_type(4)));
#define FA3_TWI 0
#include "dt_fa3fh1_kernel.inc"
#undef FA3_TWI
#define FA3_TWI 1
#include "dt_fa3fh1_kernel.inc"
#undef FA3_TWI

__global__ __launch_bounds__(256) void k_fh_ghost_init(unsigned long long *__restrict__ nodes, uint32_t nnodes,
                                                      int64_t P) {
  int64_t i = (int64_t)blockIdx.x * 256 + threadIdx.x;
  if (i < P) nodes[nnodes + i] = fht_pack(nnodes + (uint32_t)i, 0, 0);
}

__global__ __launch_bounds__(256) void k_fh_node_jump(unsigned long long *__restrict__ state, int64_t n,
                                                      int *__restrict__ flags, int round, int hops) {
  if (flags && round > 0 && flags[round - 1] == 0) {
    if (blockIdx.x == 0 && threadIdx.x == 0) flags[round] = 0;
    return;
  }
  bool pending = false;
  for (int64_t i = (int64_t)blockIdx.x * 256 + threadIdx.x; i < n; i += (int64_t)gridDim.x * 256) {
    unsigned long long s = __hip_atomic_load(&state[i], __ATOMIC_RELAXED, __HIP_MEMORY_SCOPE_AGENT);
    bool open = false, changed = false;
    for (int h = 0; h < hops; h++) {
      const uint32_t ncf = (uint32_t)(s & 0xFFFFu);
      const uint32_t ptr = (uint32_t)(s >> 32), nd = (uint32_t)((s >> 16) & 0xFFFFu);
      if ((ncf & FHT_DONE) || ptr == (uint32_t)i) break;
      const unsigned long long t = __hip_atomic_load(&state[ptr], __ATOMIC_RELAXED, __HIP_MEMORY_SCOPE_AGENT);
      const uint32_t tptr = (uint32_t)(t >> 32), tnd = (uint32_t)((t >> 16) & 0xFFFFu);
      const uint32_t tncf = (uint32_t)(t & 0xFFFFu);
      const uint32_t nnc = ncf + (tncf & 0x7FFFu), nnd = nd + tnd;
      if (((tncf & FHT_DONE) && tptr == FHT_DEAD) || nnc + nnd > FHT_CAP) s = fht_pack(FHT_DEAD, 0, FHT_DONE);
      else s = fht_pack(tptr, nnd, nnc | (tncf & FHT_DONE));
      changed = true;
      open = !(s & (unsigned long long)FHT_DONE) && tptr != ptr;
      if (!open) break;
    }
    if (changed) __hip_atomic_store(&state[i], s, __ATOMIC_RELAXED, __HIP_MEMORY_SCOPE_AGENT);
    pending = pending || open;
  }
  if (flags && __any(pending) && (threadIdx.x & 63) == 0) flags[round] = 1;
}

template <typename AccT>
__global__ __launch_bounds__(256) void k_fh_rank_summary(DtWin w, int tiles_x, uint32_t nnodes,
                                                        const unsigned long long *__restrict__ nodes,
                                                        const float *__restrict__ dem,
                                                        const AccT *__restrict__ acc32, int64_t P,
                                                        uint8_t *__restrict__ kind, int32_t *__restrict__ ref,
                                                        int32_t *__restrict__ nc, int32_t *__restrict__ nd,
                                                        float *__restrict__ zr, long long *__restrict__ ar) {
  int64_t i = (int64_t)blockIdx.x * 256 + threadIdx.x;
  if (i >= P) return;
  int y, x;
  dt_perim_cell(w.H, w.W, i, y, x);
  const bool has_node = dt_slot_of(y % TH, x % TW) >= 0;
  unsigned long long s = has_node ? nodes[dt_node_of(y, x, tiles_x)] : fht_pack(FHT_DEAD, 0, FHT_DONE);
  uint32_t ptr = (uint32_t)(s >> 32), ncf = (uint32_t)(s & 0xFFFFu);
  uint8_t k = (uint8_t)K_DEAD;
  int32_t r = -1;
  float z = DT_NODATA;
  long long a = 0;
  if (ncf & FHT_DONE) {
    if (ptr != FHT_DEAD) {
      k = (uint8_t)K_RIVER;
      r = (int32_t)ptr;
      long long o = (long long)(ptr / (uint32_t)w.W) * w.ld + (ptr % (uint32_t)w.W);
      if (dem) z = dem[o];
      if (acc32) a = (long long)acc32[o];
    }
  } else if (ptr >= nnodes) {
    k = (uint8_t)K_REXIT;
    r = (int32_t)(ptr - nnodes);
  }
  kind[i] = k;
  ref[i] = r;
  nc[i] = (int32_t)(ncf & 0x7FFFu);
  nd[i] = (int32_t)((s >> 16) & 0xFFFFu);
  zr[i] = z;
  ar[i] = a;
}

__global__ __launch_bounds__(256) void k_fh_ghost_set(unsigned long long *__restrict__ nodes, uint32_t nnodes,
                                                     int64_t P, const uint8_t *__restrict__ res_ok,
                                                     const int32_t *__restrict__ res_nc,
                                                     const int32_t *__restrict__ res_nd) {
  int64_t i = (int64_t)blockIdx.x * 256 + threadIdx.x;
  if (i >= P) return;
  unsigned long long o = fht_pack(FHT_DEAD, 0, FHT_DONE);
  if (res_ok[i]) o = fht_pack(FHT_REMOTE | (uint32_t)i, (uint32_t)res_nd[i], (uint32_t)res_nc[i] | FHT_DONE);
  nodes[nnodes + i] = o;
}

struct FhGfi {
  float *gfi, *lnhlh;
  double expo, c0;
  const DtLogEntry *tab;
};
struct FhRemote {
  const long long *gidx;
  const float *zr;
  const long long *ar;
};
template <typename AccT>
struct FhPay;
template <>
struct FhPay<int32_t> {
  unsigned long long v[PS];
  __device__ __forceinline__ void set(int i, float z, int32_t a) {
    v[i] = ((unsigned long long)(uint32_t)a << 32) | (unsigned long long)__float_as_uint(z);
  }
  __device__ __forceinline__ void get(int i, float &z, int32_t &a) const {
    const unsigned long long p = v[i];
    z = __uint_as_float((uint32_t)p);
    a = (int32_t)(uint32_t)(p >> 32);
  }
};
template <>
struct FhPay<long long> {
  long long av[PS];
  float zv[PS];
  __device__ __forceinline__ void set(int i, float z, long long a) {
    av[i] = a;
    zv[i] = z;
  }
  __device__ __forceinline__ void get(int i, float &z, long long &a) const {
    z = zv[i];
    a = av[i];
  }
};

typedef float fh_v4f __attribute__((ext_vector_type(4)));
typedef int fh_v4i __attribute__((ext_vector_type(4)));
__device__ __forceinline__ void fh_store4(float *p, float a, float b, float c, float d) {
  fh_v4f v = {a, b, c, d};
  __builtin_nontemporal_store(v, reinterpret_cast<fh_v4f *>(p));
}
__device__ __forceinline__ void fh_store4(int32_t *p, int32_t a, int32_t b, int32_t c, int32_t d) {
  fh_v4i v = {a, b, c, d};
  __builtin_nontemporal_store(v, reinterpret_cast<fh_v4i *>(p));
}
typedef long long fh_v2l __attribute__((ext_vector_type(2)));
__device__ __forceinline__ void fh_store4(long long *p, long long a, long long b, long long c, long long d) {
  fh_v2l v0 = {a, b}, v1 = {c, d};
  __builtin_nontemporal_store(v0, reinterpret_cast<fh_v2l *>(p));
  __builtin_nontemporal_store(v1, reinterpret_cast<fh_v2l *>(p + 2));
}

template <bool RANKED, int VH, int MINW, typename AccT>
__global__ __launch_bounds__(256, MINW) void k_fh_tile3(const uint8_t *__restrict__ fdr,
                                                 const float *__restrict__ dem,
                                                 const AccT *__restrict__ acc32, DtWin w, int tiles_x,
                                                 uint32_t nnodes, const unsigned long long *__restrict__ nodes,
                                                 const unsigned long long *__restrict__ cache,
                                                 const uint8_t *__restrict__ cache_wide,
                                                 FhRemote rem, double px, float *__restrict__ fdist,
                                                 int32_t *__restrict__ idx32, long long *__restrict__ idx64,
                                                 float *__restrict__ hand, AccT *__restrict__ a_river,
                                                 FhGfi G) {
  __shared__ unsigned long long s_x[PS];
  __shared__ FhPay<AccT> s_pay;
  __shared__ DtLogEntry s_tab[DT_LOGTAB_N];
  if (G.gfi) dt_math_stage(G.tab, s_tab);
  const int tile = dt_tile_of_block((int)blockIdx.x, (int)gridDim.x);
  const int ty = tile / tiles_x, tx = tile - ty * tiles_x;
  const int y0 = ty * TH, x0 = tx * TW;
  const bool wide = cache_wide[tile] != 0;
  if (threadIdx.x < PS) {
    int ly, lx;
    dt_cell_of_slot(threadIdx.x, ly, lx);
    int f = ly * TW + lx;
    unsigned long long s = fh_cache_get(cache, wide, tile, f);
    uint32_t sp = (uint32_t)(s >> 32);
    unsigned long long o = fht_pack(FHT_DEAD, 0, FHT_DONE);
    float zr = DT_NODATA;
    AccT ar = -100;
    bool ex = sp == ((uint32_t)f | (K_EXIT << 12)), rex = sp == ((uint32_t)f | (K_REXIT << 12));
    if (ex || rex) {
      int dy, dx;
      dt_d8_delta(fdr[(long long)(y0 + ly) * w.ld + x0 + lx], dy, dx);
      size_t node = ex ? (size_t)dt_node_of(y0 + ly + dy, x0 + lx + dx, tiles_x)
                       : (size_t)nnodes + (size_t)dt_perim_index(w.H, w.W, y0 + ly, x0 + lx);
      unsigned long long ns = nodes[node];
      uint32_t nptr = (uint32_t)(ns >> 32), nnd = (uint32_t)((ns >> 16) & 0xFFFFu);
      uint32_t nncf = (uint32_t)(ns & 0xFFFFu);
      if (RANKED && !(nncf & FHT_DONE) && nptr >= nnodes && (size_t)nptr != node) {
        unsigned long long gs = nodes[nptr];
        uint32_t gncf = (uint32_t)(gs & 0xFFFFu);
        nnd += (uint32_t)((gs >> 16) & 0xFFFFu);
        const uint32_t cnt = (nncf & 0x7FFFu) + (gncf & 0x7FFFu);
        nptr = (uint32_t)(gs >> 32);
        if ((gncf & FHT_DONE) && nptr != FHT_DEAD && cnt + nnd <= FHT_CAP) nncf = cnt | FHT_DONE;
        else nptr = FHT_DEAD;
      }
      bool diag = dy != 0 && dx != 0;
      if ((nncf & FHT_DONE) && nptr != FHT_DEAD) {
        o = fht_pack(nptr, nnd + (diag ? 1u : 0u), ((nncf & 0x7FFFu) + (diag ? 0u : 1u)) | FHT_DONE);
        if (RANKED && (nptr & FHT_REMOTE)) {
          zr = rem.zr[nptr & ~FHT_REMOTE];
          ar = (AccT)rem.ar[nptr & ~FHT_REMOTE];
        } else {
          long long ro = (long long)(nptr / (uint32_t)w.W) * w.ld + (nptr % (uint32_t)w.W);
          if (dem) zr = dem[ro];
          if (acc32) ar = acc32[ro];
        }
      }
    }
    s_x[threadIdx.x] = o;
    s_pay.set((int)threadIdx.x, zr, ar);
  }
  const bool vec = x0 + TW <= w.W && (w.ld & 3) == 0 && (!dem || ((uintptr_t)dem & 15) == 0) &&
                   (!fdist || ((uintptr_t)fdist & 15) == 0) && (!idx32 || ((uintptr_t)idx32 & 15) == 0) &&
                   (!idx64 || ((uintptr_t)idx64 & 15) == 0) && (!hand || ((uintptr_t)hand & 15) == 0) &&
                   (!a_river || ((uintptr_t)a_river & 15) == 0) &&
                   (!G.gfi || ((((uintptr_t)G.gfi | (uintptr_t)G.lnhlh | (uintptr_t)acc32) & 15) == 0));
  const double dcard = px, ddiag = px * sqrt(2.0);
  struct CellOut {
    float fd, h;
    int32_t i32;
    AccT ar;
    long long i64;
  };
  auto solve = [&](unsigned long long s, float z) -> CellOut {
    uint32_t ptr = (uint32_t)(s >> 32), nd = (uint32_t)((s >> 16) & 0xFFFFu);
    uint32_t ncf = (uint32_t)(s & 0xFFFFu), nc = ncf & 0x7FFFu;
    uint32_t kind = (ptr >> 12) & 7u, f = ptr & 0xFFFu;
    bool ok = false;
    uint32_t ridx = 0;
    float pz = 0.0f;
    AccT pa = 0;
    if (ncf & FHT_DONE) {
      if (kind == K_RIVER) {
        ok = true;
        ridx = (uint32_t)((y0 + (int)f / TW) * w.W + x0 + (int)f % TW);
        long long ro = (long long)(y0 + (int)f / TW) * w.ld + x0 + (int)f % TW;
        pz = dem ? dem[ro] : DT_NODATA;
        pa = acc32 ? acc32[ro] : (AccT)-100;
      } else if (kind == K_EXIT || kind == K_REXIT) {
        int slot = dt_slot_of((int)f / TW, (int)f % TW);
        unsigned long long xs = s_x[slot];
        uint32_t xptr = (uint32_t)(xs >> 32);
        if (xptr != FHT_DEAD) {
          nc += (uint32_t)(xs & 0x7FFFu);
          nd += (uint32_t)((xs >> 16) & 0xFFFFu);
          ok = nc + nd <= FHT_CAP;
          ridx = xptr;
          s_pay.get(slot, pz, pa);
        }
      }
    }
    const bool remote = RANKED && ok && (ridx & FHT_REMOTE) != 0u;
    CellOut o;
    o.fd = ok ? (float)(dcard * (double)nc + ddiag * (double)nd) : DT_NODATA;
    o.i32 = (ok && !remote) ? (int32_t)ridx : -100;
    o.i64 = -100;
    if (RANKED && ok) {
      o.i64 = remote ? rem.gidx[ridx & ~FHT_REMOTE]
                     : (long long)(w.gy0 + (int)(ridx / (uint32_t)w.W)) * w.Wg + w.gx0 + (int)(ridx % (uint32_t)w.W);
      o.i32 = (int32_t)o.i64;
    }
    o.h = DT_NODATA;
    if (z != DT_NODATA && ok) {
      o.h = z - pz;
      if (o.h < 0.0f && o.h != DT_NODATA) o.h = 0.0f;
    }
    o.ar = ok ? pa : (AccT)-100;
    return o;
  };
  if (vec) {
    constexpr int VPT = NT / 4 / 256;
#pragma unroll 1
    for (int h = 0; h < VPT / VH; h++) {
      uint4 wa[VH], wb[VH];
      float4 z4[VH];
#pragma unroll
      for (int u = 0; u < VH; u++) {
        int c = 4 * (threadIdx.x + 256 * (h * VH + u));
        if (wide) {
          const uint4 *cp = reinterpret_cast<const uint4 *>(cache + (size_t)tile * NT + c);
          wa[u] = cp[0];
          wb[u] = cp[1];
        } else {
          uint4 v = *reinterpret_cast<const uint4 *>(reinterpret_cast<const uint32_t *>(cache + (size_t)tile * NT) + c);
          unsigned long long a = fh_cache_unpack(v.x), b2 = fh_cache_unpack(v.y), c2 = fh_cache_unpack(v.z),
                             d2 = fh_cache_unpack(v.w);
          wa[u] = make_uint4((uint32_t)a, (uint32_t)(a >> 32), (uint32_t)b2, (uint32_t)(b2 >> 32));
          wb[u] = make_uint4((uint32_t)c2, (uint32_t)(c2 >> 32), (uint32_t)d2, (uint32_t)(d2 >> 32));
        }
        int y = y0 + c / TW;
        z4[u] = make_float4(DT_NODATA, DT_NODATA, DT_NODATA, DT_NODATA);
        if (dem && y < w.H) z4[u] = *reinterpret_cast<const float4 *>(dem + (long long)y * w.ld + x0 + c % TW);
      }
      if (h == 0) __syncthreads();
#pragma unroll
      for (int u = 0; u < VH; u++) {
        int c = 4 * (threadIdx.x + 256 * (h * VH + u));
        int y = y0 + c / TW;
        if (y >= w.H) continue;
        long long o = (long long)y * w.ld + x0 + c % TW;
        CellOut r0 = solve(((unsigned long long)wa[u].y << 32) | wa[u].x, z4[u].x);
        CellOut r1 = solve(((unsigned long long)wa[u].w << 32) | wa[u].z, z4[u].y);
        CellOut r2 = solve(((unsigned long long)wb[u].y << 32) | wb[u].x, z4[u].z);
        CellOut r3 = solve(((unsigned long long)wb[u].w << 32) | wb[u].z, z4[u].w);
        if (fdist) fh_store4(fdist + o, r0.fd, r1.fd, r2.fd, r3.fd);
        if (idx32) fh_store4(idx32 + o, r0.i32, r1.i32, r2.i32, r3.i32);
        if (RANKED && idx64) {
          *reinterpret_cast<longlong2 *>(idx64 + o) = make_longlong2(r0.i64, r1.i64);
          *reinterpret_cast<longlong2 *>(idx64 + o + 2) = make_longlong2(r2.i64, r3.i64);
        }
        if (hand) fh_store4(hand + o, r0.h, r1.h, r2.h, r3.h);
        if (a_river) fh_store4(a_river + o, r0.ar, r1.ar, r2.ar, r3.ar);
        if (G.gfi) {
          AccT fx, fy, fz, fw;
          if (sizeof(AccT) == 8) {
            const longlong2 fa = *reinterpret_cast<const longlong2 *>(acc32 + o);
            const longlong2 fb = *reinterpret_cast<const longlong2 *>(acc32 + o + 2);
            fx = (AccT)fa.x; fy = (AccT)fa.y; fz = (AccT)fb.x; fw = (AccT)fb.y;
          } else {
            const int4 f = *reinterpret_cast<const int4 *>(acc32 + o);
            fx = (AccT)f.x; fy = (AccT)f.y; fz = (AccT)f.z; fw = (AccT)f.w;
          }
          float4 g, l;
          dt_gfi_both_cell(r0.h, r0.ar, fx, G.expo, G.c0, s_tab, g.x, l.x);
          __builtin_amdgcn_sched_barrier(0);
          dt_gfi_both_cell(r1.h, r1.ar, fy, G.expo, G.c0, s_tab, g.y, l.y);
          __builtin_amdgcn_sched_barrier(0);
          dt_gfi_both_cell(r2.h, r2.ar, fz, G.expo, G.c0, s_tab, g.z, l.z);
          __builtin_amdgcn_sched_barrier(0);
          dt_gfi_both_cell(r3.h, r3.ar, fw, G.expo, G.c0, s_tab, g.w, l.w);
          fh_store4(G.gfi + o, g.x, g.y, g.z, g.w);
          fh_store4(G.lnhlh + o, l.x, l.y, l.z, l.w);
        }
        __builtin_amdgcn_sched_barrier(0);
      }
    }
    return;
  }
  __syncthreads();
#pragma unroll 1
  for (int j = 0; j < CPT; j++) {
    int c = threadIdx.x + 256 * j;
    int y = y0 + c / TW, x = x0 + c % TW;
    if (y >= w.H || x >= w.W) continue;
    long long o = (long long)y * w.ld + x;
    CellOut r = solve(fh_cache_get(cache, wide, tile, c), dem ? dem[o] : DT_NODATA);
    if (fdist) fdist[o] = r.fd;
    if (idx32) idx32[o] = r.i32;
    if (RANKED && idx64) idx64[o] = r.i64;
    if (hand) hand[o] = r.h;
    if (a_river) a_river[o] = r.ar;
    if (G.gfi) {
      float g, l;
      dt_gfi_both_cell(r.h, r.ar, acc32[o], G.expo, G.c0, s_tab, g, l);
      G.gfi[o] = g;
      G.lnhlh[o] = l;
    }
  }
}

struct FhScratch {
  unsigned long long *nodes, *cache;
  int *flags;
  uint8_t *cache_wide;
  int64_t nnodes, ntiles, P;
  int tiles_x;
  size_t bytes;
};
static FhScratch fh_layout(const DtWin &w, void *scratch) {
  FhScratch f;
  f.tiles_x = (w.W + TW - 1) / TW;
  f.ntiles = (int64_t)f.tiles_x * ((w.H + TH - 1) / TH);
  f.nnodes = f.ntiles * PS;
  f.P = dt_perim_count(w.H, w.W);
  DtCarver c(scratch);
  f.nodes = c.take<unsigned long long>((size_t)f.nnodes + (size_t)f.P);
  f.cache = c.take<unsigned long long>((size_t)f.ntiles * NT);
  f.flags = (int *)c.raw(256);
  f.cache_wide = c.take<uint8_t>((size_t)f.ntiles);
  f.bytes = c.bytes();
  return f;
}
size_t dt_flowhand_tiled_scratch(int64_t H, int64_t W) { return fh_layout(dt_full_window(H, W), nullptr).bytes; }

static int fh_local_tail(hipStream_t s, const DtWin &w, const uint8_t *fdr, const int8_t *river, const FhScratch &f) {
  dim3 gt((unsigned)f.ntiles), b(256);
  hipLaunchKernelGGL(k_fh_tile1, dim3(gt.x < 2048u ? gt.x : 2048u), b, 0, s, fdr, river, w, f.tiles_x,
                     (uint32_t)f.nnodes, f.nodes, f.cache, f.cache_wide, 1, (int)f.ntiles);
  hipLaunchKernelGGL(k_fh_ghost_init, dim3((unsigned)((f.P + 255) / 256)), b, 0, s, f.nodes, (uint32_t)f.nnodes, f.P);
  DT_HIP(hipMemsetAsync(f.flags, 0, 64, s));
  dim3 gj(dt_capped_grid(f.nnodes + f.P, 4096));
  for (int r = 0; r < 8; r++)
    hipLaunchKernelGGL(k_fh_node_jump, gj, b, 0, s, f.nodes, f.nnodes + f.P, f.flags, r, 3);
  return DT_OK;
}

int dt_launch_fh_local(hipStream_t s, const DtWin &w, const uint8_t *fdr, const int8_t *river, void *scratch,
                       size_t scratch_bytes) {
  if (w.H == 0 || w.W == 0) return DT_OK;
  FhScratch f = fh_layout(w, scratch);
  DT_REQUIRE(scratch_bytes >= f.bytes, "scratch too small");
  DT_REQUIRE(f.nnodes + f.P < 0x7FFFFFF0ll, "raster too large for one device tile");
  hipLaunchKernelGGL(k_fh_tile1n, dim3((unsigned)f.ntiles), dim3(256), 0, s, fdr, river, w, f.tiles_x,
                     (uint32_t)f.nnodes, f.nodes, f.cache, f.cache_wide);
  return fh_local_tail(s, w, fdr, river, f);
}

bool dt_twi_epilogue_ok(const DtWin &w, const void *acc, const int8_t *river, const DtTwiEpilogue *twi) {
  return w.W % TW == 0 && (w.ld & 3) == 0 && w.halo == 0 && w.gx0 == 0 &&
         w.gy0 == 0 && w.ld == w.W && ((uintptr_t)acc & 15) == 0 && ((uintptr_t)river & 3) == 0 && twi->marks &&
         twi->slope && twi->ti && twi->mti &&
         (((uintptr_t)twi->slope | (uintptr_t)twi->ti | (uintptr_t)twi->mti | (uintptr_t)twi->marks) & 15) == 0;
}

int dt_launch_fa_finish_fh_local(hipStream_t s, const DtWin &w, const uint8_t *fdr, const float *dem, void *fa_scratch,
                                 void *fh_scratch, size_t fh_bytes, const unsigned long long *ext_perim,
                                 int64_t river_thr, void *acc, int acc64, int8_t *river, int *status,
                                 const uint8_t *nod4, int ldm, const DtTwiEpilogue *twi) {
  if (w.H == 0 || w.W == 0) return DT_OK;
  DT_REQUIRE(river != nullptr, "HAND needs the river mask");
  FaScratch f = fa_layout(w, fa_scratch);
  FhScratch h = fh_layout(w, fh_scratch);
  DT_REQUIRE(fh_bytes >= h.bytes, "scratch too small");
  DT_REQUIRE(h.nnodes + h.P < 0x7FFFFFF0ll, "raster too large for one device tile");
  dim3 gt((unsigned)f.ntiles), b(256), gn((unsigned)((f.nnodes + 255) / 256));
  if (ext_perim) {
    int64_t P = dt_perim_count(w.H, w.W);
    hipLaunchKernelGGL(k_fa_propagate, dim3((unsigned)((P + 255) / 256)), b, 0, s, w, f.tiles_x, f.nnodes, f.nxt,
                       ext_perim, P, f.ext);
  }
  if (dt_debug_get(DT_DBG_FA_SCATTER)) hipLaunchKernelGGL(k_fa_poison, gn, b, 0, s, f.rec, f.nnodes, f.entry_of, f.state, f.ext);
  const bool fused = !acc64 && w.W % TW == 0 && (w.ld & 3) == 0 &&
                     (((uintptr_t)acc | (uintptr_t)dem) & 15) == 0 && ((uintptr_t)river & 3) == 0;
  if (fused) {
    const FaIn in = fa_inputs(f, ext_perim);
    int32_t thr = river_thr > 2147483647ll ? 2147483647 : (river_thr < -2147483647ll ? -2147483647 : (int32_t)river_thr);
    const bool use_mask = nod4 != nullptr && w.halo == 0 && w.gx0 == 0 && w.gy0 == 0;
    if (twi) {
      DT_REQUIRE(dt_twi_epilogue_ok(w, acc, river, twi) && use_mask && !ext_perim,
                 "the TI / MTI epilogue takes a single raster with its nodata mask (dt_twi_epilogue_ok)");
      const int64_t stx = (w.W + 255) / 256, sntiles = stx * ((w.H + 15) / 16);
      const DtStencilAux S = dt_stencil_aux_layout(sntiles, twi->marks);
      TwiOut tw{twi->slope, twi->ti, twi->mti, twi->n_top, log(twi->px * twi->px), S.mark, (uint32_t *)S.lmask, (int)stx};
      hipLaunchKernelGGL(k_fa3fh1_twi, gt, b, 0, s, fdr, dem, nod4, ldm, w, f.tiles_x, in.rec, in.state, in.ext, f.loc16,
                         (int32_t *)acc, thr, river, status, (uint32_t)h.nnodes, h.nodes, h.cache, h.cache_wide, tw);
    } else if (use_mask)
      hipLaunchKernelGGL(k_fa3fh1<2>, gt, b, 0, s, fdr, dem, nod4, ldm, w, f.tiles_x, in.rec, in.state, in.ext, f.loc16, (int32_t *)acc, thr,
                         river, status, (uint32_t)h.nnodes, h.nodes, h.cache, h.cache_wide);
    else if (dem)
      hipLaunchKernelGGL(k_fa3fh1<1>, gt, b, 0, s, fdr, dem, nod4, ldm, w, f.tiles_x, in.rec, in.state, in.ext, f.loc16, (int32_t *)acc, thr,
                         river, status, (uint32_t)h.nnodes, h.nodes, h.cache, h.cache_wide);
    else
      hipLaunchKernelGGL(k_fa3fh1<0>, gt, b, 0, s, fdr, dem, nod4, ldm, w, f.tiles_x, in.rec, in.state, in.ext, f.loc16, (int32_t *)acc, thr,
                         river, status, (uint32_t)h.nnodes, h.nodes, h.cache, h.cache_wide);
  } else {
    DT_REQUIRE(!twi, "the TI / MTI epilogue needs the fused form of the tile passes (dt_twi_epilogue_ok)");
    if (acc64) {
      fa_launch_tile3<long long>(s, gt, w, fdr, dem, f, ext_perim, (long long *)acc, (long long)river_thr, river, status);
    } else {
      int32_t thr = river_thr > 2147483647ll ? 2147483647 : (river_thr < -2147483647ll ? -2147483647 : (int32_t)river_thr);
      fa_launch_tile3<int32_t>(s, gt, w, fdr, dem, f, ext_perim, (int32_t *)acc, thr, river, status);
    }
    hipLaunchKernelGGL(k_fh_tile1n, gt, b, 0, s, fdr, river, w, h.tiles_x, (uint32_t)h.nnodes, h.nodes, h.cache,
                       h.cache_wide);
  }
  return fh_local_tail(s, w, fdr, river, h);
}

int dt_launch_fh_summary(hipStream_t s, const DtWin &w, void *scratch, const float *dem, const void *acc, int acc64,
                         uint8_t *kind, int32_t *ref, int32_t *nc, int32_t *nd, float *zr, long long *ar) {
  FhScratch f = fh_layout(w, scratch);
  if (f.P == 0) return DT_OK;
  dim3 g((unsigned)((f.P + 255) / 256)), b(256);
  if (acc64)
    hipLaunchKernelGGL(k_fh_rank_summary<long long>, g, b, 0, s, w, f.tiles_x, (uint32_t)f.nnodes, f.nodes, dem,
                       (const long long *)acc, f.P, kind, ref, nc, nd, zr, ar);
  else
    hipLaunchKernelGGL(k_fh_rank_summary<int32_t>, g, b, 0, s, w, f.tiles_x, (uint32_t)f.nnodes, f.nodes, dem,
                       (const int32_t *)acc, f.P, kind, ref, nc, nd, zr, ar);
  return DT_OK;
}

int dt_launch_fh_finish(hipStream_t s, const DtWin &w, const float *dem, const uint8_t *fdr,
                        const int8_t *river, const void *acc, int acc64, double px, void *scratch,
                        const uint8_t *res_ok, const int32_t *res_nc, const int32_t *res_nd,
                        const long long *rem_gidx, const float *rem_zr, const long long *rem_ar, float *fdist,
                        int32_t *idx32, long long *idx64, float *hand, void *a_river, float *gfi,
                        float *lnhlh, double n_gfi, double b_gfi, double size) {
  if (w.H == 0 || w.W == 0) return DT_OK;
  FhScratch f = fh_layout(w, scratch);
  dim3 gt((unsigned)f.ntiles), b(256), gn((unsigned)((f.nnodes + f.P + 255) / 256));
  if (res_ok) {
    hipLaunchKernelGGL(k_fh_ghost_set, dim3((unsigned)((f.P + 255) / 256)), b, 0, s, f.nodes, (uint32_t)f.nnodes,
                       f.P, res_ok, res_nc, res_nd);
  }
  FhRemote rem{rem_gidx, rem_zr, rem_ar};
  FhGfi G{nullptr, nullptr, 0.0, 0.0, nullptr};
  if (gfi && lnhlh) {
    DT_REQUIRE(dem && acc, "fused GFI needs dem and the accumulation raster");
    G = FhGfi{gfi, lnhlh, n_gfi, log(b_gfi) + n_gfi * log(size * size), dt_math_device_table(s)};
  }
  (void)river;
  const bool ranked = res_ok || idx64;
#define FH_GO(R, MW, T)                                                                                                \
  hipLaunchKernelGGL((k_fh_tile3<R, 1, MW, T>), gt, b, 0, s, fdr, dem, (const T *)acc, w, f.tiles_x, (uint32_t)f.nnodes, \
                     f.nodes, f.cache, f.cache_wide, rem, px, fdist, idx32, idx64, hand, (T *)a_river, G)
  if (acc64) {
    if (ranked) FH_GO(true, 4, long long);
    else FH_GO(false, 4, long long);
  } else {
    if (ranked) FH_GO(true, 5, int32_t);
    else FH_GO(false, 5, int32_t);
  }
#undef FH_GO
  return DT_OK;
}

#define RK_MAX 64
struct RkLayout {
  int ty, tx, nranks;
  long long Pmax;
  int ys[RK_MAX + 1], xs[RK_MAX + 1];
  int Hg, Wg;
};
__device__ __forceinline__ void rk_rank_geom(const RkLayout &L, int r, int &y0, int &x0, int &H, int &W) {
  int ry = r / L.tx, rx = r - ry * L.tx;
  y0 = L.ys[ry];
  x0 = L.xs[rx];
  H = L.ys[ry + 1] - y0;
  W = L.xs[rx + 1] - x0;
}
__device__ __forceinline__ long long rk_step_target(const RkLayout &L, int r, long long i, uint32_t code) {
  if (!dt_d8_valid(code)) return -1;
  int y0, x0, H, W;
  rk_rank_geom(L, r, y0, x0, H, W);
  if (i >= dt_perim_count(H, W)) return -1;
  int y, x, dy, dx;
  dt_perim_cell(H, W, i, y, x);
  dt_d8_delta(code, dy, dx);
  int ty = y + dy, tx = x + dx;
  if (ty >= 0 && ty < H && tx >= 0 && tx < W) return -1;
  int gy = y0 + ty, gx = x0 + tx;
  if (gy < 0 || gy >= L.Hg || gx < 0 || gx >= L.Wg) return -1;
  int ry = 0, rx = 0;
  while (gy >= L.ys[ry + 1]) ry++;
  while (gx >= L.xs[rx + 1]) rx++;
  int r2 = ry * L.tx + rx, y2, x2, H2, W2;
  rk_rank_geom(L, r2, y2, x2, H2, W2);
  return (long long)r2 * L.Pmax + dt_perim_index(H2, W2, gy - y2, gx - x2);
}

struct RkRows {
  const unsigned char *buf;
  long long rowbytes;
  long long off[8];
};
template <typename T>
__device__ __forceinline__ T rk_get(const RkRows &R, int field, int r, long long i) {
  return reinterpret_cast<const T *>(R.buf + (long long)r * R.rowbytes + R.off[field])[i];
}

__global__ __launch_bounds__(256) void k_rk_fa_link(RkLayout L, RkRows R, int32_t *__restrict__ entry_of,
                                                   int32_t *__restrict__ parent, uint32_t *__restrict__ pending) {
  long long n = (long long)blockIdx.x * 256 + threadIdx.x;
  if (n >= (long long)L.nranks * L.Pmax) return;
  int r = (int)(n / L.Pmax);
  long long i = n - (long long)r * L.Pmax;
  long long e = rk_step_target(L, r, i, rk_get<uint8_t>(R, 2, r, i));
  int32_t par = -1;
  if (e >= 0) {
    int r2 = (int)(e / L.Pmax);
    int32_t xr = rk_get<int32_t>(R, 1, r2, e - (long long)r2 * L.Pmax);
    if (xr >= 0) {
      par = (int32_t)((long long)r2 * L.Pmax + xr);
      atomicAdd(&pending[par], 1u);
    }
  }
  entry_of[n] = (int32_t)e;
  parent[n] = par;
}
__global__ __launch_bounds__(256) void k_rk_fa_sources(long long nn, const int32_t *__restrict__ entry_of,
                                                      const uint32_t *__restrict__ pending,
                                                      uint8_t *__restrict__ is_src) {
  long long n = (long long)blockIdx.x * 256 + threadIdx.x;
  if (n >= nn) return;
  is_src[n] = (entry_of[n] >= 0 && pending[n] == 0u) ? 1 : 0;
}
__global__ __launch_bounds__(256) void k_rk_fa_reduce(RkLayout L, RkRows R, const int32_t *__restrict__ entry_of,
                                                     const int32_t *__restrict__ parent,
                                                     const uint8_t *__restrict__ is_src,
                                                     uint32_t *__restrict__ pending,
                                                     unsigned long long *__restrict__ sum,
                                                     unsigned long long *__restrict__ ext) {
  long long n = (long long)blockIdx.x * 256 + threadIdx.x;
  long long nn = (long long)L.nranks * L.Pmax;
  if (n >= nn) return;
  if (!is_src[n]) return;
  long long q = n;
  int rq = (int)(q / L.Pmax);
  unsigned long long A = (unsigned long long)rk_get<long long>(R, 0, rq, q - (long long)rq * L.Pmax);
  for (long long it = 0; it < nn; it++) {
    atomicAdd(&ext[entry_of[q]], A);
    int32_t p = parent[q];
    if (p < 0) break;
    atomicAdd(&sum[p], A);
    __threadfence();
    if (atomicSub(&pending[p], 1u) != 1u) break;
    __threadfence();
    int rp = (int)(p / L.Pmax);
    A = (unsigned long long)rk_get<long long>(R, 0, rp, p - (long long)rp * L.Pmax) +
        __hip_atomic_load(&sum[p], __ATOMIC_RELAXED, __HIP_MEMORY_SCOPE_AGENT);
    q = p;
  }
}
__global__ __launch_bounds__(256) void k_rk_fa_poison(RkLayout L, const int32_t *__restrict__ entry_of,
                                                     const uint32_t *__restrict__ pending,
                                                     unsigned long long *__restrict__ ext) {
  long long n = (long long)blockIdx.x * 256 + threadIdx.x;
  if (n >= (long long)L.nranks * L.Pmax) return;
  if (entry_of[n] >= 0 && pending[n] != 0u) atomicOr(&ext[entry_of[n]], FA_CYCLE);
}

static int rk_make_layout(int ty, int tx, const int64_t *heights, const int64_t *widths, int64_t Pmax,
                          RkLayout *L) {
  DT_REQUIRE(ty >= 1 && tx >= 1 && ty <= RK_MAX && tx <= RK_MAX, "rank grid too large");
  L->ty = ty;
  L->tx = tx;
  L->nranks = ty * tx;
  L->Pmax = Pmax;
  L->ys[0] = L->xs[0] = 0;
  for (int i = 0; i < ty; i++) L->ys[i + 1] = L->ys[i] + (int)heights[i];
  for (int i = 0; i < tx; i++) L->xs[i + 1] = L->xs[i] + (int)widths[i];
  L->Hg = L->ys[ty];
  L->Wg = L->xs[tx];
  return DT_OK;
}

struct RkScratch {
  unsigned long long *sum, *ext;
  uint32_t *pending;
  int32_t *entry_of, *parent;
  uint8_t *is_src;
  void *pad;
  size_t bytes;
};
static RkScratch rk_scratch_layout(size_t nn, void *scratch) {
  RkScratch ws;
  DtCarver c(scratch);
  ws.sum = c.take<unsigned long long>(nn);
  ws.ext = c.take<unsigned long long>(nn);
  ws.pending = c.take<uint32_t>(nn);
  ws.entry_of = c.take<int32_t>(nn);
  ws.parent = c.take<int32_t>(nn);
  ws.is_src = c.take<uint8_t>(nn);
  ws.pad = c.raw(256);
  ws.bytes = c.bytes();
  return ws;
}
size_t dt_rank_solve_scratch(int nranks, int64_t Pmax) {
  return rk_scratch_layout((size_t)nranks * (size_t)Pmax, nullptr).bytes;
}

int dt_launch_rank_solve_flowacc(hipStream_t s, int ty, int tx, const int64_t *heights, const int64_t *widths,
                                 int64_t Pmax, const void *rows, int64_t rowbytes, const int64_t *offs, int rank,
                                 int64_t P_rank, void *scratch, unsigned long long *ext_out) {
  RkLayout L;
  DT_TRY(rk_make_layout(ty, tx, heights, widths, Pmax, &L));
  RkRows R;
  R.buf = (const unsigned char *)rows;
  R.rowbytes = rowbytes;
  for (int k = 0; k < 8; k++) R.off[k] = k < 3 ? offs[k] : 0;
  size_t nn = (size_t)L.nranks * (size_t)Pmax;
  if (nn == 0) return DT_OK;
  const RkScratch ws = rk_scratch_layout(nn, scratch);
  DT_HIP(hipMemsetAsync(ws.sum, 0, (size_t)((char *)ws.entry_of - (char *)ws.sum), s));
  dim3 g((unsigned)((nn + 255) / 256)), b(256);
  hipLaunchKernelGGL(k_rk_fa_link, g, b, 0, s, L, R, ws.entry_of, ws.parent, ws.pending);
  hipLaunchKernelGGL(k_rk_fa_sources, g, b, 0, s, (long long)nn, ws.entry_of, ws.pending, ws.is_src);
  hipLaunchKernelGGL(k_rk_fa_reduce, g, b, 0, s, L, R, ws.entry_of, ws.parent, ws.is_src, ws.pending, ws.sum, ws.ext);
  hipLaunchKernelGGL(k_rk_fa_poison, g, b, 0, s, L, ws.entry_of, ws.pending, ws.ext);
  DT_HIP(hipMemcpyAsync(ext_out, ws.ext + (size_t)rank * Pmax, (size_t)P_rank * 8, hipMemcpyDeviceToDevice, s));
  return DT_OK;
}

__global__ __launch_bounds__(256) void k_rk_fh_build(RkLayout L, RkRows R, unsigned long long *__restrict__ nodes) {
  long long n = (long long)blockIdx.x * 256 + threadIdx.x;
  if (n >= (long long)L.nranks * L.Pmax) return;
  int r = (int)(n / L.Pmax);
  long long i = n - (long long)r * L.Pmax;
  uint32_t kind = rk_get<uint8_t>(R, 5, r, i);
  unsigned long long o = fht_pack(FHT_DEAD, 0, FHT_DONE);
  if (kind == K_RIVER) {
    o = fht_pack((uint32_t)n, (uint32_t)rk_get<int32_t>(R, 2, r, i), (uint32_t)rk_get<int32_t>(R, 1, r, i) | FHT_DONE);
  } else if (kind == K_REXIT) {
    long long ex = rk_get<int32_t>(R, 0, r, i);
    long long e = rk_step_target(L, r, ex, rk_get<uint8_t>(R, 6, r, ex));
    if (e >= 0) o = fht_pack((uint32_t)e, (uint32_t)rk_get<int32_t>(R, 2, r, i), (uint32_t)rk_get<int32_t>(R, 1, r, i));
  }
  nodes[n] = o;
}
__global__ __launch_bounds__(256) void k_rk_fh_result(RkLayout L, RkRows R, const unsigned long long *__restrict__ nodes,
                                                     int rank, long long P_rank, uint8_t *__restrict__ res_ok,
                                                     int32_t *__restrict__ res_nc, int32_t *__restrict__ res_nd,
                                                     long long *__restrict__ gidx, float *__restrict__ zr,
                                                     long long *__restrict__ ar) {
  long long i = (long long)blockIdx.x * 256 + threadIdx.x;
  if (i >= P_rank) return;
  uint8_t ok = 0;
  int32_t c = 0, d = 0;
  long long g = -100, a = 0;
  float z = DT_NODATA;
  long long e = rk_step_target(L, rank, i, rk_get<uint8_t>(R, 6, rank, i));
  if (e >= 0) {
    unsigned long long wd = nodes[e];
    uint32_t ptr = (uint32_t)(wd >> 32), ncf = (uint32_t)(wd & 0xFFFFu);
    if ((ncf & FHT_DONE) && ptr != FHT_DEAD) {
      ok = 1;
      c = (int32_t)(ncf & 0x7FFFu);
      d = (int32_t)((wd >> 16) & 0xFFFFu);
      int rt = (int)(ptr / (uint32_t)L.Pmax);
      long long it = (long long)ptr - (long long)rt * L.Pmax;
      int y0, x0, H, W;
      rk_rank_geom(L, rt, y0, x0, H, W);
      int ref = rk_get<int32_t>(R, 0, rt, it);
      g = (long long)(y0 + ref / W) * L.Wg + x0 + ref % W;
      z = rk_get<float>(R, 3, rt, it);
      a = rk_get<long long>(R, 4, rt, it);
    }
  }
  res_ok[i] = ok;
  res_nc[i] = c;
  res_nd[i] = d;
  gidx[i] = g;
  zr[i] = z;
  ar[i] = a;
}

int dt_launch_rank_solve_flowhand(hipStream_t s, int ty, int tx, const int64_t *heights, const int64_t *widths,
                                  int64_t Pmax, const void *rows, int64_t rowbytes, const int64_t *offs, int rank,
                                  int64_t P_rank, void *scratch, uint8_t *res_ok, int32_t *res_nc,
                                  int32_t *res_nd, long long *gidx, float *zr, long long *ar) {
  RkLayout L;
  DT_TRY(rk_make_layout(ty, tx, heights, widths, Pmax, &L));
  RkRows R;
  R.buf = (const unsigned char *)rows;
  R.rowbytes = rowbytes;
  for (int k = 0; k < 8; k++) R.off[k] = k < 7 ? offs[k] : 0;
  size_t nn = (size_t)L.nranks * (size_t)Pmax;
  if (nn == 0 || P_rank == 0) return DT_OK;
  DT_REQUIRE(nn < 0x7FFFFFF0ull, "too many ring cells");
  unsigned long long *nodes = rk_scratch_layout(nn, scratch).sum;
  dim3 g((unsigned)((nn + 255) / 256)), b(256);
  hipLaunchKernelGGL(k_rk_fh_build, g, b, 0, s, L, R, nodes);
  for (int r = 0; r < 8; r++) hipLaunchKernelGGL(k_fh_node_jump, g, b, 0, s, nodes, (int64_t)nn, (int *)nullptr, r, 3);
  hipLaunchKernelGGL(k_rk_fh_result, dim3((unsigned)((P_rank + 255) / 256)), b, 0, s, L, R, nodes, rank,
                     (long long)P_rank, res_ok, res_nc, res_nd, gidx, zr, ar);
  return DT_OK;
}

__global__ __launch_bounds__(256) void k_rk_fh_zr64(RkLayout L, RkRows R, const unsigned long long *__restrict__ nodes,
                                                   int rank, long long P_rank, double *__restrict__ zr64) {
  long long i = (long long)blockIdx.x * 256 + threadIdx.x;
  if (i >= P_rank) return;
  double z = -100.0;
  long long e = rk_step_target(L, rank, i, rk_get<uint8_t>(R, 6, rank, i));
  if (e >= 0) {
    unsigned long long wd = nodes[e];
    uint32_t ptr = (uint32_t)(wd >> 32), ncf = (uint32_t)(wd & 0xFFFFu);
    if ((ncf & FHT_DONE) && ptr != FHT_DEAD) {
      int rt = (int)(ptr / (uint32_t)L.Pmax);
      z = rk_get<double>(R, 7, rt, (long long)ptr - (long long)rt * L.Pmax);
    }
  }
  zr64[i] = z;
}
int dt_launch_rank_solve_flowhand_f64(hipStream_t s, int ty, int tx, const int64_t *heights, const int64_t *widths,
                                      int64_t Pmax, const void *rows, int64_t rowbytes, const int64_t *offs8, int rank,
                                      int64_t P_rank, void *scratch, uint8_t *res_ok, int32_t *res_nc,
                                      int32_t *res_nd, long long *gidx, float *zr, long long *ar, double *zr64) {
  DT_TRY(dt_launch_rank_solve_flowhand(s, ty, tx, heights, widths, Pmax, rows, rowbytes, offs8, rank, P_rank, scratch,
                                       res_ok, res_nc, res_nd, gidx, zr, ar));
  RkLayout L;
  DT_TRY(rk_make_layout(ty, tx, heights, widths, Pmax, &L));
  RkRows R;
  R.buf = (const unsigned char *)rows;
  R.rowbytes = rowbytes;
  for (int k = 0; k < 8; k++) R.off[k] = offs8[k];
  const size_t nn = (size_t)L.nranks * (size_t)Pmax;
  if (nn == 0 || P_rank == 0) return DT_OK;
  hipLaunchKernelGGL(k_rk_fh_zr64, dim3((unsigned)((P_rank + 255) / 256)), dim3(256), 0, s, L, R,
                     (const unsigned long long *)rk_scratch_layout(nn, scratch).sum, rank, (long long)P_rank, zr64);
  return DT_OK;
}
```

Baseline: 36000 Mcells/s.

## Defer HAND tile solve: walk boundary paths in fused flowacc kernel, solve in finish

In the fused flowacc+flowhand local kernel, the full per-tile HAND solve is replaced by a cheap pointer walk, run only for the fed perimeter slots, that produces node summaries. The whole-tile solve moves into the finish stage, where one kernel solves each tile and writes HAND/GFI outputs in the same pass. Marked-tile fallback kernels compact their work by scanning flags per block. This removes a redundant tile solve and moves work out of the heavier fused kernel. The cost is more kernels, new scratch-owner bookkeeping, and serial per-thread walks whose length depends on the data.

```diff
diff --git a/descriptools_amd/csrc/dt_capi.hip b/descriptools_amd/csrc/dt_capi.hip
--- a/descriptools_amd/csrc/dt_capi.hip
+++ b/descriptools_amd/csrc/dt_capi.hip
@@ -1267,9 +1267,10 @@
   d.scratch(need, need2, &scr, &scr2);
   DT_TRY(d.rc);
   DT_TRY(dt_launch_fa_local(c->stream, d.w, fdr, scr, need, acc32, 0));
+  int walked = 0;
   DT_TRY(d.done(dt_launch_fa_finish_fh_local(c->stream, d.w, fdr, dem, scr, scr2, need2, nullptr, threshold, acc32, 0,
-                                             river, c->status, nod4, dt_nodata4_ld(W), twi)));
-  dt_scratch_claim(c, DT_OWNER_HAND, H, W, scr2);
+                                             river, c->status, nod4, dt_nodata4_ld(W), twi, &walked)));
+  dt_scratch_claim(c, walked ? DT_OWNER_HAND_WALK : DT_OWNER_HAND, H, W, scr2);
   return DT_OK;
 }
 extern "C" int dt_dev_flowacc_river_flowhand_local(dt_ctx *c, const uint8_t *fdr, const float *dem, int64_t H, int64_t W,
@@ -1383,13 +1384,15 @@
   DT_REQUIRE(!fused || (dem && acc && gfi && lnhlh), "NULL raster");
   DT_REQUIRE(!res_ok || (res_nc && res_nd && rem_gidx && rem_zr && rem_ar), "incomplete rank-exit results");
   const DtScratchClaim *k;
-  DT_TRY(dt_scratch_claimed(c, DT_OWNER_HAND, &d.w, false,
+  const bool walked = c->claim.owner == DT_OWNER_HAND_WALK && d.w.halo == 0 && d.w.gy0 == 0 && d.w.gx0 == 0 &&
+                      d.w.H == d.w.Hg && d.w.W == d.w.Wg;
+  DT_TRY(dt_scratch_claimed(c, walked ? DT_OWNER_HAND_WALK : DT_OWNER_HAND, &d.w, false,
                             "flowhand finish without a matching dt_dev_flowhand_local_w on this context (another call "
                             "has used the context's scratch in between)", &k));
   return d.done(dt_launch_fh_finish(c->stream, d.w, dem, fdr, river, acc, acc64, px, k->ptr, res_ok, res_nc, res_nd,
                                     (const long long *)rem_gidx, rem_zr, (const long long *)rem_ar, fdist, idx32,
                                     (long long *)idx64, hand, a_river, fused ? gfi : nullptr, fused ? lnhlh : nullptr,
-                                    n_gfi, b, px));
+                                    n_gfi, b, px, walked ? 1 : 0));
 }
 extern "C" int dt_dev_flowhand_finish_w(dt_ctx *c, const dt_window *win, const float *dem, const uint8_t *fdr,
                                         const int8_t *river, const int32_t *acc32, double px,
diff --git a/descriptools_amd/csrc/dt_common.h b/descriptools_amd/csrc/dt_common.h
--- a/descriptools_amd/csrc/dt_common.h
+++ b/descriptools_amd/csrc/dt_common.h
@@ -45,7 +45,7 @@
 };
 int dt_debug_get(int key);
 
-enum DtScratchOwner { DT_OWNER_NONE = 0, DT_OWNER_FLOWACC, DT_OWNER_HAND, DT_OWNER_DINF, DT_OWNER_MFD };
+enum DtScratchOwner { DT_OWNER_NONE = 0, DT_OWNER_FLOWACC, DT_OWNER_HAND, DT_OWNER_DINF, DT_OWNER_MFD, DT_OWNER_HAND_WALK };
 struct DtScratchClaim {
   DtScratchOwner owner;
   int64_t h, w;
diff --git a/descriptools_amd/csrc/dt_fa3fh1_kernel.inc b/descriptools_amd/csrc/dt_fa3fh1_kernel.inc
--- a/descriptools_amd/csrc/dt_fa3fh1_kernel.inc
+++ b/descriptools_amd/csrc/dt_fa3fh1_kernel.inc
@@ -1,8 +1,15 @@
-#if FA3_TWI
-__global__ __launch_bounds__(256, 6) void k_fa3fh1_twi(const uint8_t *__restrict__ fdr, const float *__restrict__ dem,
+#if FA3_WALK
+#define FA3_NAME(n) n##w
+#define FA3_NAME_TWI(n) n##w_twi
+#else
+#define FA3_NAME(n) n
+#define FA3_NAME_TWI(n) n##_twi
+#endif
+#if FA3_TWI
+__global__ __launch_bounds__(256, 6) void FA3_NAME_TWI(k_fa3fh1)(const uint8_t *__restrict__ fdr, const float *__restrict__ dem,
 #else
 template <int ND>
-__global__ __launch_bounds__(256, 6) void k_fa3fh1(const uint8_t *__restrict__ fdr, const float *__restrict__ dem,
+__global__ __launch_bounds__(256, 6) void FA3_NAME(k_fa3fh1)(const uint8_t *__restrict__ fdr, const float *__restrict__ dem,
 #endif
                                                   const uint8_t *__restrict__ nod4, int ldm, DtWin w, int tiles_x,
                                                   const unsigned long long *__restrict__ rec,
@@ -19,11 +26,15 @@
 #else
                                                   uint8_t *__restrict__ cache_wide) {
 #endif
+#undef FA3_NAME
+#undef FA3_NAME_TWI
 #define P3(c) ((uint32_t)(c) + (((uint32_t)(c) >> 6) << 2))
 #define NT3 (TH * (TW + 4))
   __shared__ __attribute__((aligned(16))) unsigned char smem[NT3 * 6];
   __shared__ unsigned long long s_in;
+#if !FA3_WALK
   __shared__ int s_ovf;
+#endif
   uint32_t *s_delta = reinterpret_cast<uint32_t *>(smem);
   uint16_t *s_nxt = reinterpret_cast<uint16_t *>(smem + NT3 * 4);
   const int tile = dt_tile_of_block((int)blockIdx.x, (int)gridDim.x);
@@ -79,7 +90,15 @@
     }
   }
   if (rec) e = fa_inflow(fa_gather(c2, y0, x0, threadIdx.x, tiles_x, rec, state), e);
+#if FA3_WALK
+  bool fed_now = false;
+#pragma unroll
+  for (int q = 0; q < 8; q++) fed_now = fed_now || c2[q] == fa_back(q);
+  const unsigned long long fed_mask = __ballot(fed_now);
+#endif
+#if !FA3_WALK
   if (threadIdx.x == 0) s_ovf = 0;
+#endif
   if (__syncthreads_or(!(e & FA_CYCLE) && FA_VALUE(e) >= (1ull << 22))) {
     if (threadIdx.x == 0) s_in = 0ull;
     __syncthreads();
@@ -154,7 +173,26 @@
     }
 #endif
   }
+#if FA3_WALK
+#pragma unroll
+  for (int u = 0; u < VPT; u++) {
+    if (!riv4[u]) continue;
+    const uint32_t pc = P3(4 * (threadIdx.x + 256 * u));
+    uint2 nx = *reinterpret_cast<const uint2 *>(&s_nxt[pc]);
+    if (riv4[u] & 0x1u) nx.x = (nx.x & 0xFFFF0000u) | NX_RIVER;
+    if (riv4[u] & 0x100u) nx.x = (nx.x & 0xFFFFu) | (NX_RIVER << 16);
+    if (riv4[u] & 0x10000u) nx.y = (nx.y & 0xFFFF0000u) | NX_RIVER;
+    if (riv4[u] & 0x1000000u) nx.y = (nx.y & 0xFFFFu) | (NX_RIVER << 16);
+    *reinterpret_cast<uint2 *>(&s_nxt[pc]) = nx;
+  }
+#endif
   __syncthreads();
+#if FA3_WALK
+  fh_walk_body(s_nxt, fdr, ((fed_mask >> (threadIdx.x & 63u)) & 1ull) != 0ull, w, tile, tiles_x, y0, x0, nodes, cache_wide);
+#undef P3
+#undef NT3
+}
+#else
 #undef P3
 #undef NT3
   uint32_t *s_w = reinterpret_cast<uint32_t *>(smem);
@@ -166,3 +204,4 @@
   __syncthreads();
   fh_tile1n_body(s_fdr, s_w, s_kind, &s_ovf, s_lut, riv4, w, tile, tiles_x, y0, x0, nnodes, nodes, cache, cache_wide);
 }
+#endif
diff --git a/descriptools_amd/csrc/dt_kernels.h b/descriptools_amd/csrc/dt_kernels.h
--- a/descriptools_amd/csrc/dt_kernels.h
+++ b/descriptools_amd/csrc/dt_kernels.h
@@ -126,7 +126,8 @@
 int dt_launch_fa_finish_fh_local(hipStream_t s, const DtWin &w, const uint8_t *fdr, const float *dem, void *fa_scratch,
                                  void *fh_scratch, size_t fh_bytes, const unsigned long long *ext_perim,
                                  int64_t river_thr, void *acc, int acc64, int8_t *river, int *status,
-                                 const uint8_t *nod4 = nullptr, int ldm = 0, const DtTwiEpilogue *twi = nullptr);
+                                 const uint8_t *nod4 = nullptr, int ldm = 0, const DtTwiEpilogue *twi = nullptr,
+                                 int *walked = nullptr);
 bool dt_twi_epilogue_ok(const DtWin &w, const void *acc, const int8_t *river, const DtTwiEpilogue *twi);
 int dt_launch_fh_local(hipStream_t s, const DtWin &w, const uint8_t *fdr, const int8_t *river, void *scratch,
                        size_t scratch_bytes);
@@ -137,7 +138,8 @@
                         const uint8_t *res_ok, const int32_t *res_nc, const int32_t *res_nd,
                         const long long *rem_gidx, const float *rem_zr, const long long *rem_ar, float *fdist,
                         int32_t *idx32, long long *idx64, float *hand, void *a_river, float *gfi = nullptr,
-                        float *lnhlh = nullptr, double n_gfi = 0.0, double b_gfi = 1.0, double size = 1.0);
+                        float *lnhlh = nullptr, double n_gfi = 0.0, double b_gfi = 1.0, double size = 1.0,
+                        int walked = 0);
 int dt_launch_gfi_both(hipStream_t s, const float *hand, const void *a_river, const void *fac, int acc64,
                        int64_t n, double expo, double b, double size, float *gfi, float *lnhlh);
 int dt_launch_unique_extremes(hipStream_t s, const float *x, int64_t n, uint32_t *work4, float *out3);
diff --git a/descriptools_amd/csrc/dt_tiles.hip b/descriptools_amd/csrc/dt_tiles.hip
--- a/descriptools_amd/csrc/dt_tiles.hip
+++ b/descriptools_amd/csrc/dt_tiles.hip
@@ -1226,21 +1226,18 @@
   return fh_cache_unpack(reinterpret_cast<const uint32_t *>(cache + (size_t)tile * NT)[c]);
 }
 
-__global__ __launch_bounds__(256) void k_fh_tile1(const uint8_t *__restrict__ fdr,
-                                                 const int8_t *__restrict__ river, DtWin w, int tiles_x,
-                                                 uint32_t nnodes, unsigned long long *__restrict__ nodes,
-                                                 unsigned long long *__restrict__ cache,
-                                                 uint8_t *__restrict__ cache_wide, int only_marked, int ntiles) {
-  __shared__ __attribute__((aligned(16))) uint8_t s_fdr[NT];
-  __shared__ uint8_t s_halo[2 * (TW + 2) + 2 * TH];
-  __shared__ __attribute__((aligned(16))) unsigned long long s_st[NT];
-  for (int tile = (int)blockIdx.x; tile < ntiles; tile += (int)gridDim.x) {
-  if (only_marked && cache_wide[tile] != 2) continue;
+template <bool NODES>
+__device__ __forceinline__ void fh_tile1_tile(uint8_t *s_fdr, uint8_t *s_halo, unsigned long long *s_st, int tile,
+                                              const uint8_t *__restrict__ fdr, const int8_t *__restrict__ river,
+                                              const DtWin &w, int tiles_x, uint32_t nnodes,
+                                              unsigned long long *__restrict__ nodes,
+                                              unsigned long long *__restrict__ cache,
+                                              uint8_t *__restrict__ cache_wide) {
   const int ty = tile / tiles_x, tx = tile - ty * tiles_x;
   const int y0 = ty * TH, x0 = tx * TW;
   FhTile T{s_fdr, s_halo, s_st};
   fht_solve_tile(T, fdr, river, w, y0, x0);
-  if (threadIdx.x < PS) {
+  if (NODES && threadIdx.x < PS) {
     int ly, lx;
     dt_cell_of_slot(threadIdx.x, ly, lx);
     unsigned long long s = s_st[ly * TW + lx];
@@ -1280,7 +1277,36 @@
     for (int j = 0; j < CPT; j++) c32[threadIdx.x + 256 * j] = fh_cache_pack(wv[j]);
   }
   __syncthreads();
-  }
+}
+__global__ __launch_bounds__(256) void k_fh_tile1(const uint8_t *__restrict__ fdr,
+                                                 const int8_t *__restrict__ river, DtWin w, int tiles_x,
+                                                 uint32_t nnodes, unsigned long long *__restrict__ nodes,
+                                                 unsigned long long *__restrict__ cache,
+                                                 uint8_t *__restrict__ cache_wide, int only_marked, int ntiles) {
+  __shared__ __attribute__((aligned(16))) uint8_t s_fdr[NT];
+  __shared__ uint8_t s_halo[2 * (TW + 2) + 2 * TH];
+  __shared__ __attribute__((aligned(16))) unsigned long long s_st[NT];
+  for (int tile = (int)blockIdx.x; tile < ntiles; tile += (int)gridDim.x) {
+    if (only_marked && cache_wide[tile] != 2) continue;
+    fh_tile1_tile<true>(s_fdr, s_halo, s_st, tile, fdr, river, w, tiles_x, nnodes, nodes, cache, cache_wide);
+  }
+}
+__global__ __launch_bounds__(256) void k_fh_tile1_marked(const uint8_t *__restrict__ fdr,
+                                                        const int8_t *__restrict__ river, DtWin w, int tiles_x,
+                                                        uint32_t nnodes, unsigned long long *__restrict__ nodes,
+                                                        unsigned long long *__restrict__ cache,
+                                                        uint8_t *cache_wide, int ntiles) {
+  __shared__ __attribute__((aligned(16))) uint8_t s_fdr[NT];
+  __shared__ uint8_t s_halo[2 * (TW + 2) + 2 * TH];
+  __shared__ __attribute__((aligned(16))) unsigned long long s_st[NT];
+  __shared__ uint8_t s_flag[256];
+  const int base = (int)blockIdx.x * 256, mine = base + (int)threadIdx.x;
+  const uint8_t flag = mine < ntiles ? cache_wide[mine] : (uint8_t)0;
+  s_flag[threadIdx.x] = flag;
+  if (!__syncthreads_or(flag == 2)) return;
+  for (int i = 0; i < 256; i++)
+    if (s_flag[i] == 2)
+      fh_tile1_tile<false>(s_fdr, s_halo, s_st, base + i, fdr, river, w, tiles_x, nnodes, nodes, cache, cache_wide);
 }
 
 #define FN_CNT 0x3FFFFu
@@ -1294,12 +1320,9 @@
   dt_d8_delta(code, dy, dx);
   return ((uint32_t)(dy * TW + dx) << FN_PTR_SH) + ((dy != 0 && dx != 0) ? (1u << 9) : 1u);
 }
-__device__ __forceinline__ void fh_tile1n_body(uint8_t *s_fdr, uint32_t *s_w, uint8_t *s_kind, int *s_ovf_p,
-                                               const uint32_t *s_lut, const uint32_t (&riv4)[NT / 4 / 256],
-                                               const DtWin &w, int tile, int tiles_x, int y0, int x0, uint32_t nnodes,
-                                               unsigned long long *__restrict__ nodes,
-                                               unsigned long long *__restrict__ cache,
-                                               uint8_t *__restrict__ cache_wide) {
+__device__ __forceinline__ bool fh_tile1n_solve(uint8_t *s_fdr, uint32_t *s_w, uint8_t *s_kind, int *s_ovf_p,
+                                                const uint32_t *s_lut, const uint32_t (&riv4)[NT / 4 / 256],
+                                                const DtWin &w, int y0, int x0, uint2 (&own)[CPT / 2]) {
 #define s_ovf (*s_ovf_p)
   const bool interior = dt_tile_interior(w, y0, x0);
   const uint32_t lx0 = (4u * threadIdx.x) & 63u;
@@ -1352,7 +1375,6 @@
   }
   __syncthreads();
   uint2 *s_w2 = reinterpret_cast<uint2 *>(s_w);
-  uint2 own[CPT / 2];
 #pragma unroll
   for (int j = 0; j < CPT / 2; j++) own[j] = s_w2[threadIdx.x + 256 * j];
   for (int round = 0; round < 13; round++) {
@@ -1382,15 +1404,27 @@
     if (!__syncthreads_or(changed)) break;
     if (s_ovf) break;
   }
-  if (s_ovf) {
+  return !s_ovf;
+#undef s_ovf
+}
+__device__ __forceinline__ uint32_t fh_narrow_word(uint32_t v, uint32_t c, const uint8_t *s_kind) {
+  uint32_t f = v >> FN_PTR_SH, kind = s_kind[f];
+  if (!(v & FN_DONE)) { f = c; kind = K_DEAD; v = 0; }
+  return f | (kind << 12) | (((v >> 9) & 0xFFu) << 15) | ((v & 0xFFu) << 23);
+}
+__device__ __forceinline__ void fh_tile1n_body(uint8_t *s_fdr, uint32_t *s_w, uint8_t *s_kind, int *s_ovf_p,
+                                               const uint32_t *s_lut, const uint32_t (&riv4)[NT / 4 / 256],
+                                               const DtWin &w, int tile, int tiles_x, int y0, int x0, uint32_t nnodes,
+                                               unsigned long long *__restrict__ nodes,
+                                               unsigned long long *__restrict__ cache,
+                                               uint8_t *__restrict__ cache_wide) {
+  uint2 own[CPT / 2];
+  if (!fh_tile1n_solve(s_fdr, s_w, s_kind, s_ovf_p, s_lut, riv4, w, y0, x0, own)) {
     if (threadIdx.x == 0) cache_wide[tile] = 2;
     return;
   }
-  auto narrow = [&](uint32_t v, uint32_t c) -> uint32_t {
-    uint32_t f = v >> FN_PTR_SH, kind = s_kind[f];
-    if (!(v & FN_DONE)) { f = c; kind = K_DEAD; v = 0; }
-    return f | (kind << 12) | (((v >> 9) & 0xFFu) << 15) | ((v & 0xFFu) << 23);
-  };
+  uint2 *s_w2 = reinterpret_cast<uint2 *>(s_w);
+  auto narrow = [&](uint32_t v, uint32_t c) -> uint32_t { return fh_narrow_word(v, c, s_kind); };
 #pragma unroll
   for (int j = 0; j < CPT / 2; j++) {
     const int c2 = threadIdx.x + 256 * j;
@@ -1424,7 +1458,45 @@
     }
     nodes[(size_t)tile * PS + threadIdx.x] = o;
   }
-#undef s_ovf
+}
+
+#define NX_RIVER 0xFFFCu
+#define FH_SOLVE_LATER 3
+__device__ __forceinline__ void fh_walk_body(const uint16_t *s_nxt, const uint8_t *__restrict__ fdr, bool fed, const DtWin &w,
+                                             int tile, int tiles_x, int y0, int x0,
+                                             unsigned long long *__restrict__ nodes,
+                                             uint8_t *__restrict__ cache_wide) {
+  constexpr uint32_t PW = TW + 4, NTP = TH * PW;
+  if (threadIdx.x == 0) cache_wide[tile] = (uint8_t)FH_SOLVE_LATER;
+  if (threadIdx.x >= PS) return;
+  unsigned long long o = fht_pack(FHT_DEAD, 0, FHT_DONE);
+  if (fed) {
+    int ly, lx;
+    dt_cell_of_slot(threadIdx.x, ly, lx);
+    uint32_t c = (uint32_t)ly * PW + (uint32_t)lx, nc = 0, nd = 0;
+    uint32_t n = 0;
+    for (int it = 0; it < NT; it++) {
+      n = s_nxt[c];
+      if (n >= NTP) break;
+      const uint32_t d = n > c ? n - c : c - n;
+      if (d == 1u || d == PW) nc++;
+      else nd++;
+      c = n;
+    }
+    if (n == NX_RIVER || n == NX_EXIT) {
+      const int fy = (int)(c / PW), fx = (int)(c % PW);
+      const uint32_t code = fdr[(long long)(y0 + fy) * w.ld + x0 + fx];
+      if (n == NX_EXIT) {
+        int dy, dx;
+        dt_d8_delta(code, dy, dx);
+        const bool diag = dy != 0 && dx != 0;
+        o = fht_pack(dt_node_of(y0 + fy + dy, x0 + fx + dx, tiles_x), nd + (diag ? 1u : 0u), nc + (diag ? 0u : 1u));
+      } else if (code != 0u) {
+        o = fht_pack((uint32_t)((y0 + fy) * w.W + x0 + fx), nd, nc | FHT_DONE);
+      }
+    }
+  }
+  nodes[(size_t)tile * PS + threadIdx.x] = o;
 }
 
 __global__ __launch_bounds__(256, 6) void k_fh_tile1n(const uint8_t *__restrict__ fdr,
@@ -1463,12 +1535,22 @@
   int stiles_x;
 };
 typedef float fa_v4f __attribute__((ext_vector_type(4)));
+#define FA3_WALK 0
 #define FA3_TWI 0
 #include "dt_fa3fh1_kernel.inc"
 #undef FA3_TWI
 #define FA3_TWI 1
 #include "dt_fa3fh1_kernel.inc"
 #undef FA3_TWI
+#undef FA3_WALK
+#define FA3_WALK 1
+#define FA3_TWI 0
+#include "dt_fa3fh1_kernel.inc"
+#undef FA3_TWI
+#define FA3_TWI 1
+#include "dt_fa3fh1_kernel.inc"
+#undef FA3_TWI
+#undef FA3_WALK
 
 __global__ __launch_bounds__(256) void k_fh_ghost_init(unsigned long long *__restrict__ nodes, uint32_t nnodes,
                                                       int64_t P) {
@@ -1611,30 +1693,46 @@
   __builtin_nontemporal_store(v1, reinterpret_cast<fh_v2l *>(p + 2));
 }
 
-template <bool RANKED, int VH, int MINW, typename AccT>
-__global__ __launch_bounds__(256, MINW) void k_fh_tile3(const uint8_t *__restrict__ fdr,
-                                                 const float *__restrict__ dem,
-                                                 const AccT *__restrict__ acc32, DtWin w, int tiles_x,
-                                                 uint32_t nnodes, const unsigned long long *__restrict__ nodes,
-                                                 const unsigned long long *__restrict__ cache,
-                                                 const uint8_t *__restrict__ cache_wide,
-                                                 FhRemote rem, double px, float *__restrict__ fdist,
-                                                 int32_t *__restrict__ idx32, long long *__restrict__ idx64,
-                                                 float *__restrict__ hand, AccT *__restrict__ a_river,
-                                                 FhGfi G) {
-  __shared__ unsigned long long s_x[PS];
-  __shared__ FhPay<AccT> s_pay;
-  __shared__ DtLogEntry s_tab[DT_LOGTAB_N];
-  if (G.gfi) dt_math_stage(G.tab, s_tab);
-  const int tile = dt_tile_of_block((int)blockIdx.x, (int)gridDim.x);
+struct FhSolveLds {
+  uint8_t *fdr;
+  uint32_t *w;
+  uint8_t *kind;
+  uint32_t *lut;
+  int *ovf;
+};
+template <bool RANKED, int VH, typename AccT, bool SOLVE>
+__device__ __forceinline__ bool fh_tile3_tile(unsigned long long *s_x, FhPay<AccT> &s_pay, DtLogEntry *s_tab,
+                                              const FhSolveLds &L, const int8_t *__restrict__ river, int tile,
+                                              const uint8_t *__restrict__ fdr, const float *__restrict__ dem,
+                                              const AccT *__restrict__ acc32, const DtWin &w, int tiles_x,
+                                              uint32_t nnodes, const unsigned long long *__restrict__ nodes,
+                                              const unsigned long long *__restrict__ cache, bool wide,
+                                              const FhRemote &rem, double px, float *__restrict__ fdist,
+                                              int32_t *__restrict__ idx32, long long *__restrict__ idx64,
+                                              float *__restrict__ hand, AccT *__restrict__ a_river,
+                                              const FhGfi &G) {
   const int ty = tile / tiles_x, tx = tile - ty * tiles_x;
   const int y0 = ty * TH, x0 = tx * TW;
-  const bool wide = cache_wide[tile] != 0;
+  if (SOLVE) {
+    const uint4 v_fdr = dt_tile_fetch16(fdr, w, y0, x0);
+    const uint4 v_riv = dt_tile_fetch16(reinterpret_cast<const uint8_t *>(river), w, y0, x0);
+    dt_tile_put16(L.fdr, v_fdr);
+    dt_tile_put16(L.kind, v_riv);
+    L.lut[threadIdx.x] = fh_lut_entry(threadIdx.x);
+    if (threadIdx.x == 0) *L.ovf = 0;
+    __syncthreads();
+    uint32_t riv4[NT / 4 / 256];
+#pragma unroll
+    for (int u = 0; u < NT / 4 / 256; u++) riv4[u] = *reinterpret_cast<const uint32_t *>(&L.kind[4 * (threadIdx.x + 256 * u)]);
+    uint2 own[CPT / 2];
+    if (!fh_tile1n_solve(L.fdr, L.w, L.kind, L.ovf, L.lut, riv4, w, y0, x0, own)) return false;
+  }
+  auto solved = [&](uint32_t v, int c) -> uint32_t { return fh_narrow_word(v, (uint32_t)c, L.kind); };
   if (threadIdx.x < PS) {
     int ly, lx;
     dt_cell_of_slot(threadIdx.x, ly, lx);
     int f = ly * TW + lx;
-    unsigned long long s = fh_cache_get(cache, wide, tile, f);
+    unsigned long long s = SOLVE ? fh_cache_unpack(solved(L.w[f], f)) : fh_cache_get(cache, wide, tile, f);
     uint32_t sp = (uint32_t)(s >> 32);
     unsigned long long o = fht_pack(FHT_DEAD, 0, FHT_DONE);
     float zr = DT_NODATA;
@@ -1642,7 +1740,7 @@
     bool ex = sp == ((uint32_t)f | (K_EXIT << 12)), rex = sp == ((uint32_t)f | (K_REXIT << 12));
     if (ex || rex) {
       int dy, dx;
-      dt_d8_delta(fdr[(long long)(y0 + ly) * w.ld + x0 + lx], dy, dx);
+      dt_d8_delta(SOLVE ? (uint32_t)L.fdr[f] : (uint32_t)fdr[(long long)(y0 + ly) * w.ld + x0 + lx], dy, dx);
       size_t node = ex ? (size_t)dt_node_of(y0 + ly + dy, x0 + lx + dx, tiles_x)
                        : (size_t)nnodes + (size_t)dt_perim_index(w.H, w.W, y0 + ly, x0 + lx);
       unsigned long long ns = nodes[node];
@@ -1745,7 +1843,13 @@
           wa[u] = cp[0];
           wb[u] = cp[1];
         } else {
-          uint4 v = *reinterpret_cast<const uint4 *>(reinterpret_cast<const uint32_t *>(cache + (size_t)tile * NT) + c);
+          uint4 v;
+          if (SOLVE) {
+            v = *reinterpret_cast<const uint4 *>(&L.w[c]);
+            v = make_uint4(solved(v.x, c), solved(v.y, c + 1), solved(v.z, c + 2), solved(v.w, c + 3));
+          } else {
+            v = *reinterpret_cast<const uint4 *>(reinterpret_cast<const uint32_t *>(cache + (size_t)tile * NT) + c);
+          }
           unsigned long long a = fh_cache_unpack(v.x), b2 = fh_cache_unpack(v.y), c2 = fh_cache_unpack(v.z),
                              d2 = fh_cache_unpack(v.w);
           wa[u] = make_uint4((uint32_t)a, (uint32_t)(a >> 32), (uint32_t)b2, (uint32_t)(b2 >> 32));
@@ -1798,7 +1902,7 @@
         __builtin_amdgcn_sched_barrier(0);
       }
     }
-    return;
+    return true;
   }
   __syncthreads();
 #pragma unroll 1
@@ -1807,7 +1911,8 @@
     int y = y0 + c / TW, x = x0 + c % TW;
     if (y >= w.H || x >= w.W) continue;
     long long o = (long long)y * w.ld + x;
-    CellOut r = solve(fh_cache_get(cache, wide, tile, c), dem ? dem[o] : DT_NODATA);
+    CellOut r = solve(SOLVE ? fh_cache_unpack(solved(L.w[c], c)) : fh_cache_get(cache, wide, tile, c),
+                      dem ? dem[o] : DT_NODATA);
     if (fdist) fdist[o] = r.fd;
     if (idx32) idx32[o] = r.i32;
     if (RANKED && idx64) idx64[o] = r.i64;
@@ -1820,6 +1925,86 @@
       G.lnhlh[o] = l;
     }
   }
+  return true;
+}
+
+template <bool RANKED, int VH, int MINW, typename AccT>
+__global__ __launch_bounds__(256, MINW) void k_fh_tile3(const uint8_t *__restrict__ fdr,
+                                                 const float *__restrict__ dem,
+                                                 const AccT *__restrict__ acc32, DtWin w, int tiles_x,
+                                                 uint32_t nnodes, const unsigned long long *__restrict__ nodes,
+                                                 const unsigned long long *__restrict__ cache,
+                                                 const uint8_t *__restrict__ cache_wide,
+                                                 FhRemote rem, double px, float *__restrict__ fdist,
+                                                 int32_t *__restrict__ idx32, long long *__restrict__ idx64,
+                                                 float *__restrict__ hand, AccT *__restrict__ a_river,
+                                                 FhGfi G) {
+  __shared__ unsigned long long s_x[PS];
+  __shared__ FhPay<AccT> s_pay;
+  __shared__ DtLogEntry s_tab[DT_LOGTAB_N];
+  if (G.gfi) dt_math_stage(G.tab, s_tab);
+  const int tile = dt_tile_of_block((int)blockIdx.x, (int)gridDim.x);
+  const bool wide = cache_wide[tile] != 0;
+  fh_tile3_tile<RANKED, VH, AccT, false>(s_x, s_pay, s_tab, FhSolveLds{}, nullptr, tile, fdr, dem, acc32, w, tiles_x,
+                                         nnodes, nodes, cache, wide, rem, px, fdist, idx32, idx64, hand, a_river, G);
+}
+
+__global__ __launch_bounds__(256, 5) void k_fh_tile3_solve(const uint8_t *__restrict__ fdr,
+                                                          const int8_t *__restrict__ river,
+                                                          const float *__restrict__ dem,
+                                                          const int32_t *__restrict__ acc32, DtWin w, int tiles_x,
+                                                          uint32_t nnodes,
+                                                          const unsigned long long *__restrict__ nodes,
+                                                          uint8_t *__restrict__ cache_wide, double px,
+                                                          float *__restrict__ fdist, int32_t *__restrict__ idx32,
+                                                          float *__restrict__ hand, int32_t *__restrict__ a_river,
+                                                          FhGfi G) {
+  __shared__ unsigned long long s_x[PS];
+  __shared__ FhPay<int32_t> s_pay;
+  __shared__ DtLogEntry s_tab[DT_LOGTAB_N];
+  __shared__ __attribute__((aligned(16))) uint8_t s_fdr[NT];
+  __shared__ __attribute__((aligned(16))) uint32_t s_w[NT];
+  __shared__ __attribute__((aligned(16))) uint8_t s_kind[NT];
+  __shared__ uint32_t s_lut[256];
+  __shared__ int s_ovf;
+  if (G.gfi) dt_math_stage(G.tab, s_tab);
+  const int tile = dt_tile_of_block((int)blockIdx.x, (int)gridDim.x);
+  const bool ok = fh_tile3_tile<false, 1, int32_t, true>(
+      s_x, s_pay, s_tab, FhSolveLds{s_fdr, s_w, s_kind, s_lut, &s_ovf}, river, tile, fdr, dem, acc32, w, tiles_x, nnodes,
+      nodes, nullptr, false, FhRemote{nullptr, nullptr, nullptr}, px, fdist, idx32, nullptr, hand, a_river, G);
+  if (!ok && threadIdx.x == 0) cache_wide[tile] = 2;
+}
+
+__global__ __launch_bounds__(256) void k_fh_tile3_marked(const uint8_t *__restrict__ fdr,
+                                                           const float *__restrict__ dem,
+                                                           const int32_t *__restrict__ acc32, DtWin w, int tiles_x,
+                                                           uint32_t nnodes,
+                                                           const unsigned long long *__restrict__ nodes,
+                                                           const unsigned long long *__restrict__ cache,
+                                                           const uint8_t *__restrict__ cache_wide, int ntiles,
+                                                           double px, float *__restrict__ fdist,
+                                                           int32_t *__restrict__ idx32, float *__restrict__ hand,
+                                                           int32_t *__restrict__ a_river, FhGfi G) {
+  __shared__ unsigned long long s_x[PS];
+  __shared__ FhPay<int32_t> s_pay;
+  __shared__ DtLogEntry s_tab[DT_LOGTAB_N];
+  __shared__ uint8_t s_flag[256];
+  const int base = (int)blockIdx.x * 256, mine = base + (int)threadIdx.x;
+  const uint8_t flag = mine < ntiles ? cache_wide[mine] : (uint8_t)FH_SOLVE_LATER;
+  s_flag[threadIdx.x] = flag;
+  if (!__syncthreads_or(flag != FH_SOLVE_LATER)) return;
+  if (G.gfi) dt_math_stage(G.tab, s_tab);
+  for (int i = 0; i < 256; i++) {
+    if (s_flag[i] == FH_SOLVE_LATER) continue;
+    fh_tile3_tile<false, 1, int32_t, false>(s_x, s_pay, s_tab, FhSolveLds{}, nullptr, base + i, fdr, dem, acc32, w,
+                                            tiles_x, nnodes, nodes, cache, s_flag[i] != 0, FhRemote{nullptr, nullptr, nullptr},
+                                            px, fdist, idx32, nullptr, hand, a_river, G);
+    __syncthreads();
+  }
+}
+__global__ __launch_bounds__(256) void k_fh_mark_all(uint8_t *__restrict__ cache_wide, int ntiles) {
+  const int t = (int)blockIdx.x * 256 + (int)threadIdx.x;
+  if (t < ntiles && cache_wide[t] == FH_SOLVE_LATER) cache_wide[t] = 2;
 }
 
 struct FhScratch {
@@ -1846,10 +2031,12 @@
 }
 size_t dt_flowhand_tiled_scratch(int64_t H, int64_t W) { return fh_layout(dt_full_window(H, W), nullptr).bytes; }
 
-static int fh_local_tail(hipStream_t s, const DtWin &w, const uint8_t *fdr, const int8_t *river, const FhScratch &f) {
+static int fh_local_tail(hipStream_t s, const DtWin &w, const uint8_t *fdr, const int8_t *river, const FhScratch &f,
+                         bool walked = false) {
   dim3 gt((unsigned)f.ntiles), b(256);
-  hipLaunchKernelGGL(k_fh_tile1, dim3(gt.x < 2048u ? gt.x : 2048u), b, 0, s, fdr, river, w, f.tiles_x,
-                     (uint32_t)f.nnodes, f.nodes, f.cache, f.cache_wide, 1, (int)f.ntiles);
+  if (!walked)
+    hipLaunchKernelGGL(k_fh_tile1, dim3(gt.x < 2048u ? gt.x : 2048u), b, 0, s, fdr, river, w, f.tiles_x,
+                       (uint32_t)f.nnodes, f.nodes, f.cache, f.cache_wide, 1, (int)f.ntiles);
   hipLaunchKernelGGL(k_fh_ghost_init, dim3((unsigned)((f.P + 255) / 256)), b, 0, s, f.nodes, (uint32_t)f.nnodes, f.P);
   DT_HIP(hipMemsetAsync(f.flags, 0, 64, s));
   dim3 gj(dt_capped_grid(f.nnodes + f.P, 4096));
@@ -1879,7 +2066,8 @@
 int dt_launch_fa_finish_fh_local(hipStream_t s, const DtWin &w, const uint8_t *fdr, const float *dem, void *fa_scratch,
                                  void *fh_scratch, size_t fh_bytes, const unsigned long long *ext_perim,
                                  int64_t river_thr, void *acc, int acc64, int8_t *river, int *status,
-                                 const uint8_t *nod4, int ldm, const DtTwiEpilogue *twi) {
+                                 const uint8_t *nod4, int ldm, const DtTwiEpilogue *twi, int *walked) {
+  if (walked) *walked = 0;
   if (w.H == 0 || w.W == 0) return DT_OK;
   DT_REQUIRE(river != nullptr, "HAND needs the river mask");
   FaScratch f = fa_layout(w, fa_scratch);
@@ -1899,6 +2087,27 @@
     const FaIn in = fa_inputs(f, ext_perim);
     int32_t thr = river_thr > 2147483647ll ? 2147483647 : (river_thr < -2147483647ll ? -2147483647 : (int32_t)river_thr);
     const bool use_mask = nod4 != nullptr && w.halo == 0 && w.gx0 == 0 && w.gy0 == 0;
+    const bool walk = walked != nullptr && !ext_perim && in.rec != nullptr && w.halo == 0 && w.gx0 == 0 && w.gy0 == 0 &&
+                      w.H == w.Hg && w.W == w.Wg;
+    if (walk) *walked = 1;
+#define FA3_GO(K)                                                                                                      \
+  hipLaunchKernelGGL(K, gt, b, 0, s, fdr, dem, nod4, ldm, w, f.tiles_x, in.rec, in.state, in.ext, f.loc16, (int32_t *)acc, \
+                     thr, river, status, (uint32_t)h.nnodes, h.nodes, h.cache, h.cache_wide)
+    if (walk) {
+      if (twi) {
+        DT_REQUIRE(dt_twi_epilogue_ok(w, acc, river, twi) && use_mask,
+                   "the TI / MTI epilogue takes a single raster with its nodata mask (dt_twi_epilogue_ok)");
+        const int64_t stx = (w.W + 255) / 256, sntiles = stx * ((w.H + 15) / 16);
+        const DtStencilAux S = dt_stencil_aux_layout(sntiles, twi->marks);
+        TwiOut tw{twi->slope, twi->ti, twi->mti, twi->n_top, log(twi->px * twi->px), S.mark, (uint32_t *)S.lmask, (int)stx};
+        hipLaunchKernelGGL(k_fa3fh1w_twi, gt, b, 0, s, fdr, dem, nod4, ldm, w, f.tiles_x, in.rec, in.state, in.ext, f.loc16,
+                           (int32_t *)acc, thr, river, status, (uint32_t)h.nnodes, h.nodes, h.cache, h.cache_wide, tw);
+      } else if (use_mask) FA3_GO(k_fa3fh1w<2>);
+      else if (dem) FA3_GO(k_fa3fh1w<1>);
+      else FA3_GO(k_fa3fh1w<0>);
+      return fh_local_tail(s, w, fdr, river, h, true);
+    }
+#undef FA3_GO
     if (twi) {
       DT_REQUIRE(dt_twi_epilogue_ok(w, acc, river, twi) && use_mask && !ext_perim,
                  "the TI / MTI epilogue takes a single raster with its nodata mask (dt_twi_epilogue_ok)");
@@ -1949,7 +2158,7 @@
                         const uint8_t *res_ok, const int32_t *res_nc, const int32_t *res_nd,
                         const long long *rem_gidx, const float *rem_zr, const long long *rem_ar, float *fdist,
                         int32_t *idx32, long long *idx64, float *hand, void *a_river, float *gfi,
-                        float *lnhlh, double n_gfi, double b_gfi, double size) {
+                        float *lnhlh, double n_gfi, double b_gfi, double size, int walked) {
   if (w.H == 0 || w.W == 0) return DT_OK;
   FhScratch f = fh_layout(w, scratch);
   dim3 gt((unsigned)f.ntiles), b(256), gn((unsigned)((f.nnodes + f.P + 255) / 256));
@@ -1963,8 +2172,24 @@
     DT_REQUIRE(dem && acc, "fused GFI needs dem and the accumulation raster");
     G = FhGfi{gfi, lnhlh, n_gfi, log(b_gfi) + n_gfi * log(size * size), dt_math_device_table(s)};
   }
-  (void)river;
   const bool ranked = res_ok || idx64;
+  if (walked) {
+    DT_REQUIRE(river != nullptr, "HAND needs the river mask");
+    const dim3 gm((unsigned)((f.ntiles + 255) / 256));
+    const bool solve = !ranked && !acc64;
+    if (solve)
+      hipLaunchKernelGGL(k_fh_tile3_solve, gt, b, 0, s, fdr, river, dem, (const int32_t *)acc, w, f.tiles_x,
+                         (uint32_t)f.nnodes, f.nodes, f.cache_wide, px, fdist, idx32, hand, (int32_t *)a_river, G);
+    else
+      hipLaunchKernelGGL(k_fh_mark_all, gm, b, 0, s, f.cache_wide, (int)f.ntiles);
+    hipLaunchKernelGGL(k_fh_tile1_marked, gm, b, 0, s, fdr, river, w, f.tiles_x, (uint32_t)f.nnodes, f.nodes, f.cache,
+                       f.cache_wide, (int)f.ntiles);
+    if (solve) {
+      hipLaunchKernelGGL(k_fh_tile3_marked, gm, b, 0, s, fdr, dem, (const int32_t *)acc, w, f.tiles_x, (uint32_t)f.nnodes,
+                         f.nodes, f.cache, f.cache_wide, (int)f.ntiles, px, fdist, idx32, hand, (int32_t *)a_river, G);
+      return DT_OK;
+    }
+  }
 #define FH_GO(R, MW, T)                                                                                                \
   hipLaunchKernelGGL((k_fh_tile3<R, 1, MW, T>), gt, b, 0, s, fdr, dem, (const T *)acc, w, f.tiles_x, (uint32_t)f.nnodes, \
                      f.nodes, f.cache, f.cache_wide, rem, px, fdist, idx32, idx64, hand, (T *)a_river, G)
```

New measurement: 36840 Mcells/s (median of 6 runs). +2.3%, better.
